# iMacsimus/Triangles-SDF-CPU-RayTracing

Measured on AMD Instinct MI355X. Metric: Mrays/sec + ms/frame at 1920x1080, bunny tris & SDF grid, 1/2/4/8 MI355X, higher is better.
Workload: dtype f32; 1 GPU; bunny: shipped stanford-bunny.obj (69,451 triangles), 1920x1080, primary rays (Normal shading, no plane) (BASELINE configs[1]); camera=orbit r=2.5 h=0.5 fovy 45, parallelism=1 GPU, 1 thread per pixel, frames_per_launch=16, streams=2

## Files before the change

### triangles-sdf-cpu-raytracing_amd/csrc/rt_device.hip

```cpp
#include <hip/hip_runtime.h>

#include <algorithm>
#include <atomic>
#include <cmath>
#include <cstdio>
#include <limits>
#include <map>
#include <mutex>
#include <string>
#include <type_traits>
#include <utility>

#include "../../include/rtamd.h"
#include "rt_dispatch.h"
#include "rt_error.h"
#include "rt_host.h"
#include "rt_queue.h"
#include "rt_ray_io.h"
#include "rt_scene.h"
#include "rt_shade.h"

using namespace rtd;
using namespace rti;

namespace {

#ifndef RT_PERSIST_BLOCK
#define RT_PERSIST_BLOCK 64
#endif
constexpr int kPBlock = RT_PERSIST_BLOCK;
static_assert(kPBlock % 64 == 0 && kPBlock >= 64 && kPBlock <= 1024, "persistent block: whole waves");
constexpr int kTile = 16;

template <class T>
__device__ __forceinline__ void fb_store(T *p, T v, bool peer) {
  if (peer) {
    __hip_atomic_store(p, v, __ATOMIC_RELAXED, __HIP_MEMORY_SCOPE_SYSTEM);
    return;
  }
  __hip_atomic_store(p, v, __ATOMIC_RELAXED, __HIP_MEMORY_SCOPE_AGENT);
}

#ifndef RT_PEER_RELEASE
#define RT_PEER_RELEASE 1
#endif
constexpr uint32_t kSysStoreFlags = RT_FLAG_TILE_NATURAL;
__device__ __forceinline__ void peer_release(uint32_t flags) {
#if RT_PEER_RELEASE
  if (flags & kSysStoreFlags) __builtin_amdgcn_fence(__ATOMIC_RELEASE, "");
#endif
}

__device__ __forceinline__ int image_row(int yl, const FrameArgs &fa) {
  if (fa.nranks <= 1) return yl;
  const uint32_t br = (uint32_t)fa.band_rows, k = (uint32_t)yl / br, r = (uint32_t)yl - k * br;
  return (int)((k * (uint32_t)fa.nranks + (uint32_t)fa.rank) * br + r);
}

template <int DIAG>
struct CntSel { using T = NoCnt; };
template <>
struct CntSel<1> { using T = LaneCnt; };
template <>
struct CntSel<2> { using T = LaneCnt; };

__device__ __forceinline__ void flush_counts(NoCnt &, unsigned long long *) {}
__device__ __forceinline__ void flush_counts(LaneCnt &c, unsigned long long *out) {
#pragma unroll
  for (int i = 0; i < C_ALL; ++i) {
    unsigned long long v = c.v[i];
#pragma unroll
    for (int off = 32; off > 0; off >>= 1) v += __shfl_xor(v, off, 64);
    if ((threadIdx.x & 63) == 0 && v) atomicAdd(out + i, v);
  }
}


#ifndef RT_DIAG_HOST_NOSTORE
#define RT_DIAG_HOST_NOSTORE 0
#endif

#ifndef RT_PAIR_FLUSH
#define RT_PAIR_FLUSH 1
#endif
constexpr int kPairWords = 2 * 8 * 16;

template <class S, int SLOTS, bool GENERAL, int DIAG, int B = kBlock, class CT>
__device__ __forceinline__ bool render_pixels(const S &sc, const PlaneDev &pl, const FrameArgs &fa,
                                              CT &cnt, uint32_t *stk, int xo, int yl,
                                              uint32_t *defer = nullptr) {
  const bool active = xo < fa.W && yl < fa.rows_local;
  constexpr bool kWaveCoop = DIAG == 0 && !GENERAL && S::kCoop;
  constexpr bool kWaveCount = DIAG == 1 && !GENERAL && S::kCoop;
  if (DIAG == 0 && !kWaveCoop && !active) return false;
  if (active || kWaveCoop || kWaveCount) {
    StackOf<S, B> st{stk + threadIdx.x};
    if constexpr (kWaveCoop) {
      const int yo = image_row(active ? yl : 0, fa);
      const uint32_t cx = fa.cull_x, cy = (uint32_t)fa.P.reserved;
      const uint32_t px = (uint32_t)xo >> 3, py = (uint32_t)yo >> 3;
      const bool inside = active && px >= (cx & 0xFFFFu) && px < (cx >> 16) && py >= (cy & 0xFFFFu) && py < (cy >> 16);
      if (__ballot(inside) == 0) {
        const bool natural = (fa.flags & (kSysStoreFlags | kFlagNatural)) != 0;
        const uint32_t idx = (uint32_t)(natural ? yo : yl) * (uint32_t)fa.W + (uint32_t)xo;
        if (defer) {
          defer[0] = 0u;
          defer[kPairWords] = __float_as_uint(kInf);
        } else if (RT_DIAG_HOST_NOSTORE != 0 && (fa.flags & kFlagHostFrame)) {
        } else if (active && (fa.flags & RT_FLAG_CLEAR) && !(fa.flags & RT_FLAG_HITS_ONLY)) {
          const bool sys = (fa.flags & (kSysStoreFlags | kFlagHostFrame)) != 0;
          fb_store(fa.color + idx, 0u, sys);
          fb_store(fa.t + idx, kInf, sys);
        }
        return false;
      }
      asm volatile("" : "+v"(xo), "+v"(yl));
    }
    const int yo = image_row(active ? yl : 0, fa);
    const int y = fa.H - yo - 1;
    const f3 o{fa.P.camera_pos[0], fa.P.camera_pos[1], fa.P.camera_pos[2]};
    f3 d;
    if (fa.flags & kFlagFastEye)
      d = eye_ray_fast(active ? xo : 0, y, fa.W, fa.H, fa.P.proj_inv, fa.P.view_inv);
    else
      d = eye_ray(active ? xo : 0, y, fa.W, fa.H, fa.P.proj_inv, fa.P.view_inv);
    const bool natural = (fa.flags & (kSysStoreFlags | kFlagNatural)) != 0;
    const bool sys = (fa.flags & (kSysStoreFlags | kFlagHostFrame)) != 0;
    const int yb = natural ? yo : yl;
    const uint32_t idx = active ? (uint32_t)yb * (uint32_t)fa.W + (uint32_t)xo : 0u;
    const bool clear = (fa.flags & RT_FLAG_CLEAR) != 0;
    const bool hits_only = (fa.flags & RT_FLAG_HITS_ONLY) != 0;
    const float tPrev = (clear || !active) ? kInf : fa.t[idx];
    const float tFarEff = std_min(100.0f, tPrev);
    bool hit;
    float t;
    f4 c;
    if (!GENERAL) {
      if (active) cnt.add(C_RAYS, 1);
      Hit h;
      if constexpr (kWaveCoop)
        h = sc.template primary<B>(o, d, 0.01f, tFarEff, active, stk);
      else if constexpr (kWaveCount)
        h = sc.template primary_counted<B>(o, d, 0.01f, tFarEff, active, stk, cnt);
      else
        h = sc.template intersect<B>(o, d, 0.01f, tFarEff, st, cnt);
      hit = h.hit;
      t = h.t;
      f3 n = h.n;
      if (dot(n, d) > 0) n = n * -1.0f;
      c = f4{(n.x + 1.0f) / 2.0f, (n.y + 1.0f) / 2.0f, (n.z + 1.0f) / 2.0f, (1.0f + 1.0f) / 2.0f};
    } else {
      c = shade_one<S, B>(sc, pl, fa.P, o, d, tFarEff, true, hit, t, st, nullptr, cnt);
    }
    const bool store = hit && !__builtin_isinf(t);
    if (defer) {
      defer[0] = store ? pack_rgba(c) : 0u;
      defer[kPairWords] = __float_as_uint(store ? t : kInf);
    } else if (RT_DIAG_HOST_NOSTORE == 1 && (fa.flags & kFlagHostFrame)) {
    } else if (RT_DIAG_HOST_NOSTORE == 2 && (fa.flags & kFlagHostFrame)) {
      if (active && store) fb_store(fa.color + idx, pack_rgba(c), sys);
    } else if (!active) {
    } else if (clear && !hits_only) {
      fb_store(fa.color + idx, store ? pack_rgba(c) : 0u, sys);
      fb_store(fa.t + idx, store ? t : kInf, sys);
    } else if (store) {
      fb_store(fa.color + idx, pack_rgba(c), sys);
      fb_store(fa.t + idx, t, sys);
    }
    return active && store;
  }
  return false;
}

typedef unsigned int u32x4 __attribute__((ext_vector_type(4)));
__device__ __forceinline__ void host_store16(uint32_t *p, u32x4 v) {
  asm volatile("global_store_dwordx4 %0, %1, off sc0 sc1" : : "v"(p), "v"(v) : "memory");
}

template <class S, int SLOTS, bool GENERAL, int DIAG, int BT = kBlock>
__device__ __forceinline__ void render_body(const S &sc, const PlaneDev &pl, const FrameArgs &fa,
                                            unsigned long long *counters, uint32_t *stk,
                                            uint32_t *hf = nullptr) {
  typename CntSel<DIAG>::T cnt{};
  unsigned long long t_start = 0;
  if (DIAG == 2) t_start = __builtin_amdgcn_s_memrealtime();
  const int lane = threadIdx.x & 63, wave = threadIdx.x >> 6;
  uint32_t bx = blockIdx.x, by = blockIdx.y;
  if (DIAG == 0 && fa.order) {
    const uint32_t tl = fa.order[blockIdx.y * gridDim.x + blockIdx.x];
    bx = tl % gridDim.x;
    by = tl / gridDim.x;
  }
  const uint64_t c0 = (DIAG == 0 && fa.cost) ? __builtin_amdgcn_s_memtime() : 0;
  const int xo = BT == 64 ? (int)bx * 8 + (lane & 7) : (int)bx * kTile + (wave & 1) * 8 + (lane & 7);
  const int yl = BT == 64 ? (int)by * 8 + (lane >> 3) : (int)by * kTile + (wave >> 1) * 8 + (lane >> 3);
  const int band = wave >> 1;
  const bool flush = RT_PAIR_FLUSH && DIAG == 0 && BT == kBlock && hf != nullptr &&
                     (fa.flags & kFlagHostFrame) && (fa.flags & RT_FLAG_CLEAR) && (fa.flags & RT_FLAG_HITS_ONLY) &&
                     (fa.W & 3) == 0 && (((uintptr_t)fa.color | (uintptr_t)fa.t) & 15u) == 0 &&
                     (int)bx * kTile + kTile <= fa.W && (int)by * kTile + band * 8 + 8 <= fa.rows_local;
  uint32_t *slot = flush ? hf + band * 128 + (lane >> 3) * 16 + (wave & 1) * 8 + (lane & 7) : nullptr;
  const bool stored = render_pixels<S, SLOTS, GENERAL, DIAG, BT>(sc, pl, fa, cnt, stk, xo, yl, slot);
  if (flush) {
    const uint32_t any = __ballot(stored) != 0 ? 1u : 0u;
    __builtin_amdgcn_fence(__ATOMIC_RELEASE, "workgroup");
    uint32_t old = 0;
    if (lane == 0) old = atomicAdd(hf + 2 * kPairWords + band, 1u | (any << 16));
    old = __builtin_amdgcn_readfirstlane(old);
    if ((old & 0xFFFFu) == 1u && (any | (old >> 16)) != 0u) {
      __builtin_amdgcn_fence(__ATOMIC_ACQUIRE, "workgroup");
      const int b = lane >> 5, r = (lane & 31) >> 2, ch = lane & 3;
      const u32x4 v = *reinterpret_cast<const u32x4 *>(hf + b * kPairWords + band * 128 + r * 16 + ch * 4);
      const int ylr = (int)by * kTile + band * 8 + r;
      const bool natural = (fa.flags & (kSysStoreFlags | kFlagNatural)) != 0;
      const uint32_t row = (uint32_t)(natural ? image_row(ylr, fa) : ylr);
      uint32_t *base = b ? reinterpret_cast<uint32_t *>(fa.t) : fa.color;
      host_store16(base + row * (uint32_t)fa.W + (uint32_t)bx * kTile + (uint32_t)ch * 4u, v);
    }
  }
  if constexpr (DIAG == 0) {
    if (fa.hit_box && !(fa.flags & kFlagRowSpan) && __ballot(stored)) {
      int32_t v[4] = {stored ? xo : INT32_MAX, stored ? -xo : INT32_MAX, stored ? yl : INT32_MAX,
                      stored ? -yl : INT32_MAX};
#pragma unroll
      for (int i = 0; i < 4; ++i)
#pragma unroll
        for (int off = 32; off > 0; off >>= 1) {
          const int32_t o = __shfl_xor(v[i], off, 64);
          v[i] = o < v[i] ? o : v[i];
        }
      if (lane == __ffsll((unsigned long long)__ballot(1)) - 1)
#pragma unroll
        for (int i = 0; i < 4; ++i)
          if (v[i] < __hip_atomic_load(fa.hit_box + i, __ATOMIC_RELAXED, __HIP_MEMORY_SCOPE_AGENT))
            atomicMin(fa.hit_box + i, v[i]);
    }
    if (fa.hit_box && (fa.flags & kFlagRowSpan) && __ballot(stored)) {
      int32_t lo = stored ? xo : INT32_MAX, nhi = stored ? -xo : INT32_MAX;
#pragma unroll
      for (int off = 1; off < 8; off <<= 1) {
        const int32_t a = __shfl_xor(lo, off, 64), b = __shfl_xor(nhi, off, 64);
        lo = a < lo ? a : lo;
        nhi = b < nhi ? b : nhi;
      }
      if ((lane & 7) == 0 && lo != INT32_MAX) {
        int32_t *sp = fa.hit_box + 2 * yl;
        if (lo < __hip_atomic_load(sp, __ATOMIC_RELAXED, __HIP_MEMORY_SCOPE_AGENT)) atomicMin(sp, lo);
        if (nhi < __hip_atomic_load(sp + 1, __ATOMIC_RELAXED, __HIP_MEMORY_SCOPE_AGENT)) atomicMin(sp + 1, nhi);
      }
    }
  }
  if constexpr (DIAG == 0) {
    if (fa.cost) {
      const uint64_t dt = __builtin_amdgcn_s_memtime() - c0;
      if (lane == __ffsll((unsigned long long)__ballot(1)) - 1)
        atomicMax(fa.cost + by * gridDim.x + bx, dt > 0xFFFFFFFFull ? 0xFFFFFFFFu : (uint32_t)dt);
    }
  }
  if constexpr (DIAG == 1) flush_counts(cnt, counters);
  if constexpr (DIAG == 2) {
    const unsigned long long t_end = __builtin_amdgcn_s_memrealtime();
    uint32_t units = 0;
#pragma unroll
    for (int i = 0; i < C_RAYS; ++i) units += cnt.v[i];
    uint32_t mx = units, sm = units;
#pragma unroll
    for (int off = 32; off > 0; off >>= 1) {
      const uint32_t om = __shfl_xor(mx, off, 64), os = __shfl_xor(sm, off, 64);
      mx = mx > om ? mx : om;
      sm += os;
    }
    uint32_t rest = units, u9 = 0;
    for (int r = 0; r < 9; ++r) {
      uint32_t m = rest;
#pragma unroll
      for (int off = 32; off > 0; off >>= 1) {
        const uint32_t om = __shfl_xor(m, off, 64);
        m = m > om ? m : om;
      }
      u9 = m;
      const uint64_t who = __ballot(rest == m);
      if ((threadIdx.x & 63) == (int)__builtin_ctzll(who)) rest = 0;
    }
    if ((threadIdx.x & 63) == 0) {
      const size_t w = ((size_t)blockIdx.y * gridDim.x + blockIdx.x) * (kBlock / 64) + (threadIdx.x >> 6);
      counters[4 * w] = t_start;
      counters[4 * w + 1] = t_end;
      counters[4 * w + 2] = ((unsigned long long)sm << 32) | mx;
      counters[4 * w + 3] = __builtin_amdgcn_s_getreg(0x1814) | ((unsigned long long)u9 << 8);
    }
  }
}

template <class S, int SLOTS, bool GENERAL, int DIAG>
constexpr int min_waves() {
  return (DIAG != 0 || SLOTS > 7) ? 1 : GENERAL ? RT_GENERAL_WAVES : S::kMinWaves;
}

#ifndef RT_FRAME_BLOCK
#define RT_FRAME_BLOCK 256
#endif
constexpr int kFBlock = RT_FRAME_BLOCK;
constexpr int kFTile = kFBlock == 64 ? 8 : kTile;
static_assert(kFBlock == 64 || kFBlock == kBlock, "one-frame workgroup: one wave or the 16x16 tile");
template <int DIAG>
constexpr int frame_block() { return DIAG == 0 ? kFBlock : kBlock; }
template <int DIAG>
constexpr int frame_tile() { return DIAG == 0 ? kFTile : kTile; }

#ifndef RT_FRAME_PRIO
#define RT_FRAME_PRIO 0
#endif
#ifndef RT_FRAME_COOP
#define RT_FRAME_COOP RT_COOP_RAYS
#endif
template <class S, int SLOTS, bool GENERAL, int DIAG>
__global__ __launch_bounds__(frame_block<DIAG>()) __attribute__((amdgpu_waves_per_eu(min_waves<S, SLOTS, GENERAL, DIAG>())))
void render_kernel(S sc_arg, PlaneDev pl, FrameArgs fa,
                                                        unsigned long long *counters) {
  __shared__ uint32_t stk[stack_words<S, SLOTS>() * frame_block<DIAG>()];
  constexpr bool kPair = RT_PAIR_FLUSH && DIAG == 0 && frame_block<DIAG>() == kBlock;
  __shared__ __attribute__((aligned(16))) uint32_t hf[kPair ? 2 * kPairWords + 4 : 4];
  S sc = sc_arg;
  if constexpr (S::kCoop && !GENERAL && DIAG == 0) {
    sc.prio_iters = RT_FRAME_PRIO;
    sc.coop_rays = RT_FRAME_COOP;
  }
  if (kPair && (fa.flags & kFlagHostFrame) && (fa.flags & RT_FLAG_CLEAR) && (fa.flags & RT_FLAG_HITS_ONLY)) {
    if (threadIdx.x < 2) hf[2 * kPairWords + threadIdx.x] = 0u;
    __syncthreads();
  }
  render_body<S, SLOTS, GENERAL, DIAG, frame_block<DIAG>()>(sc, pl, fa, counters, stk, kPair ? hf : nullptr);
  peer_release(fa.flags);
}

#ifndef RT_BATCH_BLOCK
#define RT_BATCH_BLOCK 64
#endif
constexpr int kBBlock = RT_BATCH_BLOCK;
#ifndef RT_BATCH_INTERLEAVE
#define RT_BATCH_INTERLEAVE 1
#endif
constexpr int kBTile = kBBlock == 64 ? 8 : kTile;
static_assert(kBBlock == 64 || kBBlock == kBlock, "batch workgroup: one wave or the 16x16 tile");

template <class S, int SLOTS, bool GENERAL>
__global__ __launch_bounds__(kBBlock) __attribute__((amdgpu_waves_per_eu(min_waves<S, SLOTS, GENERAL, 0>())))
void render_batch_kernel(S sc, PlaneDev pl, FrameBatch fb) {
  __shared__ uint32_t stk[stack_words<S, SLOTS>() * kBBlock];
  if constexpr (kBBlock == kBlock) {
    render_body<S, SLOTS, GENERAL, 0>(sc, pl, fb.f[blockIdx.z], nullptr, stk);
  } else {
    NoCnt cnt{};
    const int lane = threadIdx.x & 63;
#if RT_BATCH_INTERLEAVE
    const uint32_t n = gridDim.z, b = (blockIdx.z * gridDim.y + blockIdx.y) * gridDim.x + blockIdx.x;
    const uint32_t f = b % n, tl = fb.f[0].order ? fb.f[0].order[b / n] : b / n;
    const uint32_t tx = tl % gridDim.x, ty = tl / gridDim.x;
#else
    const uint32_t f = blockIdx.z, tl = blockIdx.y * gridDim.x + blockIdx.x, tx = blockIdx.x, ty = blockIdx.y;
#endif
    const uint64_t c0 = fb.f[0].cost ? __builtin_amdgcn_s_memtime() : 0;
    render_pixels<S, SLOTS, GENERAL, 0, kBBlock>(sc, pl, fb.f[f], cnt, stk, (int)tx * 8 + (lane & 7),
                                                 (int)ty * 8 + (lane >> 3));
    if (fb.f[0].cost && lane == 0) {
      const uint64_t dc = __builtin_amdgcn_s_memtime() - c0;
      atomicMax(fb.f[0].cost + tl, (uint32_t)(dc < 0xFFFFFFFFull ? dc : 0xFFFFFFFFull));
    }
  }
  peer_release(fb.f[0].flags);
}

struct PersistQ {
  uint32_t *heads;
  uint32_t items;
  uint32_t tiles_x, per_frame;
  uint32_t waves;
  uint32_t gx, gy;
  uint32_t stride;
  uint32_t nheads;
  uint32_t cpf, nper;
  unsigned long long *stamps;
  uint32_t ox, oy;
};
template <class S, bool GENERAL>
constexpr bool kQueueOrigin = S::kCoop && !GENERAL;
constexpr int kHeadStride = 1088;
constexpr int kHeadStrideMax = 4096;

__device__ __forceinline__ uint32_t q_claim(uint32_t *head) {
  uint32_t k = 0;
  if ((threadIdx.x & 63) == 0) k = __hip_atomic_fetch_add(head, 1u, __ATOMIC_RELAXED, __HIP_MEMORY_SCOPE_AGENT);
  return __builtin_amdgcn_readfirstlane(k);
}
#ifndef RT_QUEUE_HEADS
#define RT_QUEUE_HEADS 0
#endif
__device__ __forceinline__ uint32_t q_nheads(const PersistQ &q) { return RT_QUEUE_HEADS ? (uint32_t)RT_QUEUE_HEADS : q.nheads; }
__device__ __forceinline__ uint32_t q_home(uint32_t xcc, uint32_t nheads) {
  const uint32_t wave = __builtin_amdgcn_readfirstlane(threadIdx.x >> 6);
  return rtq::home(xcc, (blockIdx.x >> 3) + wave, nheads);
}
__device__ __forceinline__ uint32_t q_scan(const PersistQ &q, uint32_t nh, uint32_t own, int lane) {
  uint32_t v = 0xFFFFFFFFu;
  const bool mine = (uint32_t)lane < nh;
  if (mine) v = __hip_atomic_load(q.heads + (uint32_t)lane * q.stride, __ATOMIC_RELAXED, __HIP_MEMORY_SCOPE_AGENT);
  const uint32_t cap = q.cpf ? q.nper : rtq::cap(q.items, nh, (uint32_t)lane);
  const uint64_t left = __ballot(mine && v < cap);
  return left ? rtq::next(left, own, nh) : rtq::kNone;
}
__device__ __forceinline__ void q_leave(const PersistQ &q, uint32_t nh, int lane) {
  uint32_t *done = q.heads + nh * q.stride;
  uint32_t last = 0;
  if (lane == 0) last = __hip_atomic_fetch_add(done, 1u, __ATOMIC_RELAXED, __HIP_MEMORY_SCOPE_AGENT) == q.waves - 1;
  if (__builtin_amdgcn_readfirstlane(last)) {
    if ((uint32_t)lane < nh)
      __hip_atomic_store(q.heads + (uint32_t)lane * q.stride, 0u, __ATOMIC_RELAXED, __HIP_MEMORY_SCOPE_AGENT);
    if (lane == 0) __hip_atomic_store(done, 0u, __ATOMIC_RELAXED, __HIP_MEMORY_SCOPE_AGENT);
  }
}

template <class S, int SLOTS, bool GENERAL>
__global__ __launch_bounds__(kPBlock) __attribute__((amdgpu_waves_per_eu(min_waves<S, SLOTS, GENERAL, 0>())))
void render_persist_kernel(S sc_arg, PlaneDev pl, FrameBatch fb, PersistQ q) {
  __shared__ uint32_t stk[stack_words<S, SLOTS>() * kPBlock];
  S sc = sc_arg;
  if constexpr (S::kCoop && !GENERAL) sc.prio_iters = RT_HEAVY_PRIO;
  const int lane = threadIdx.x & 63;
  const uint32_t xcc = __builtin_amdgcn_s_getreg(0x1814) & 7;
#ifdef RT_PERSIST_STAMPS
  const unsigned long long t_start = __builtin_amdgcn_s_memrealtime();
  unsigned long long t_item = t_start, t_last = t_start, d_max = 0;
  uint32_t n_items = 0, last_item = 0, max_item = 0;
#endif
  uint32_t h = q_home(xcc, q_nheads(q));
  uint32_t k = q_claim(q.heads + h * q.stride);
  NoCnt cnt{};
  for (;;) {
    uint32_t item, f, r;
    bool drained, empty = false;
    if (q.cpf == 0) {
      item = k * q_nheads(q) + h;
      drained = item >= q.items;
      f = item / q.per_frame;
      r = item - f * q.per_frame;
    } else {
      drained = k >= q.nper;
      f = k / q.cpf;
      r = h * q.cpf + (k - f * q.cpf);
      empty = r >= q.per_frame;
      item = f * q.per_frame + r;
    }
    if (drained) {
      h = q_scan(q, q_nheads(q), h, lane);
      if (h == rtq::kNone) break;
      k = q_claim(q.heads + h * q.stride);
      continue;
    }
    const uint32_t knext = q_claim(q.heads + h * q.stride);
    if (empty) {
      k = knext;
      continue;
    }
    uint32_t ty = r / q.tiles_x, tx = r - ty * q.tiles_x;
    if constexpr (kQueueOrigin<S, GENERAL>) {
      tx += q.ox;
      ty += q.oy;
    }
#ifdef RT_PERSIST_STAMPS
    const unsigned long long t_begin = __builtin_amdgcn_s_memrealtime();
#endif
    for (uint32_t j = 0; j < q.gy; ++j)
      for (uint32_t i = 0; i < q.gx; ++i) {
        uint32_t fo = f;
        asm volatile("" : "+s"(fo));
        render_pixels<S, SLOTS, GENERAL, 0, kPBlock>(sc, pl, fb.f[fo], cnt, stk, (int)((tx * q.gx + i) * 8) + (lane & 7),
                                            (int)((ty * q.gy + j) * 8) + (lane >> 3));
      }
#ifdef RT_PERSIST_STAMPS
    ++n_items;
    t_item = __builtin_amdgcn_s_memrealtime();
    t_last = t_begin;
    last_item = item;
    if (t_item - t_begin > d_max) {
      d_max = t_item - t_begin;
      max_item = item;
    }
#endif
    k = knext;
  }
#ifdef RT_PERSIST_STAMPS
  if (q.stamps && lane == 0) {
    const size_t w = (size_t)blockIdx.x * (kPBlock / 64) + (threadIdx.x >> 6);
    unsigned long long *o = q.stamps + 8 * w;
    o[0] = t_start;
    o[1] = __builtin_amdgcn_s_memrealtime();
    o[2] = n_items | ((unsigned long long)xcc << 32);
    o[3] = t_item;
    o[4] = t_last;
    o[5] = last_item;
    o[6] = d_max;
    o[7] = max_item;
  }
#endif
  peer_release(fb.f[0].flags);
  q_leave(q, q_nheads(q), lane);
}

struct PumpFrame {
  float o[3];
  float proj_inv[16];
  float view_inv[16];
  uint32_t *color;
  float *t;
};

constexpr uint32_t kPumpHeads = rtq::kXcds;
struct ItemStream {
  uint32_t h, k;
};
__device__ __forceinline__ uint32_t take_item(const PersistQ &q, ItemStream &s, uint32_t xcc, int lane) {
  for (;;) {
    const uint32_t item = rtq::item(q.items, kPumpHeads, s.h, s.k);
    if (item != rtq::kNone) {
      s.k = q_claim(q.heads + s.h * q.stride);
      return item;
    }
    static_assert(kPumpHeads == 8 && rtq::cap(45, 8, 3) == (45 + 7 - 3) / 8 && rtq::next(0x21, 5, 8) == 0, "take_item's scan");
    uint32_t v = 0xFFFFFFFFu;
    if (lane < 8) v = __hip_atomic_load(q.heads + lane * q.stride, __ATOMIC_RELAXED, __HIP_MEMORY_SCOPE_AGENT);
    const uint64_t m = __ballot(lane < 8 && v < (q.items + 7u - (uint32_t)lane) / 8u) & 0xFFull;
    if (m == 0) return 0xFFFFFFFFu;
    const uint32_t rot = (uint32_t)(((m >> (xcc + 1)) | (m << (7 - xcc))) & 0xFFull);
    s.h = (xcc + 1 + (uint32_t)__builtin_ctz(rot)) & 7u;
    s.k = q_claim(q.heads + s.h * q.stride);
  }
}

struct OctP {
  using Ray = OctRay;
  static constexpr int kFields = kOctFields;
  static constexpr int kMinWaves = RT_OCT_WAVES;
  OctDev d;
  template <bool FAST>
  __device__ __forceinline__ int start(f3 o, f3 dir, f3 inv, float tf, Ray &R, float &t, f3 &n) const {
    NoCnt c;
    OctHitPt hp;
    const int s = oct_start<FAST>(d, o, dir, inv, 0.01f, tf, R, t, hp, c);
    if (s == RAY_HIT) n = oct_normal_at(d, hp, c);
    return s;
  }
  template <bool FAST>
  __device__ __forceinline__ int run(f3 o, f3 dir, f3 inv, float tf, LdsStack<kBlock, kOctFields> st, Ray &R, int limit,
                                     float &t, f3 &n) const {
    NoCnt c;
    OctHitPt hp;
    const int s = oct_run<kBlock, FAST, true, false>(d, o, dir, inv, 0.01f, tf, st, R, limit, t, hp, c);
    if (s == RAY_HIT) n = oct_normal_at(d, hp, c);
    return s;
  }
};

template <int kMode>
struct GridP {
  using Ray = GridRay;
  static constexpr int kFields = 1;
  static constexpr int kMinWaves = RT_GRID_WAVES;
  GridDev d;
  template <bool FAST>
  __device__ __forceinline__ int start(f3 o, f3 dir, f3 inv, float tf, Ray &R, float &, f3 &) const {
    return grid_start(o, dir, inv, 0.01f, tf, R);
  }
  template <bool FAST>
  __device__ __forceinline__ int run(f3 o, f3 dir, f3, float, LdsStack<kBlock, kFields>, Ray &R, int limit,
                                     float &t, f3 &n) const {
    NoCnt c;
    f3 hp;
    const int s = grid_run<kMode, true>(d, o, dir, R, limit, t, hp, c);
    if (s == RAY_HIT) n = grid_normal<kMode>(d, hp, c);
    return s;
  }
};

#ifndef RT_REFILL_MIN
#define RT_REFILL_MIN 16
#endif

#ifndef RT_PUMP_WAVES
#define RT_PUMP_WAVES 0
#endif
template <class P, int SLOTS>
__global__ __launch_bounds__(kBlock)
__attribute__((amdgpu_waves_per_eu(SLOTS > 7 ? 1 : (RT_PUMP_WAVES ? RT_PUMP_WAVES : P::kMinWaves))))
void render_pump_kernel(P sc, FrameBatch fb, PersistQ q, int32_t nframes, int32_t refill_min) {
  __shared__ uint32_t stk[SLOTS * P::kFields * kBlock];
  __shared__ PumpFrame frames[kMaxBatch];
  if ((int)threadIdx.x < nframes) {
    const FrameArgs &fa = fb.f[threadIdx.x];
    PumpFrame &pf = frames[threadIdx.x];
    for (int i = 0; i < 3; ++i) pf.o[i] = fa.P.camera_pos[i];
    for (int i = 0; i < 16; ++i) {
      pf.proj_inv[i] = fa.P.proj_inv[i];
      pf.view_inv[i] = fa.P.view_inv[i];
    }
    pf.color = fa.color;
    pf.t = fa.t;
  }
  __syncthreads();
  const FrameArgs &F = fb.f[0];
  const int lane = threadIdx.x & 63;
  const uint32_t xcc = __builtin_amdgcn_s_getreg(0x1814) & 7;
  const bool clear = (F.flags & RT_FLAG_CLEAR) != 0, hits_only = (F.flags & RT_FLAG_HITS_ONLY) != 0;
  const bool peer = (F.flags & kSysStoreFlags) != 0;
  const uint32_t isz = 64u * q.gx * q.gy;
  ItemStream is{xcc, 0u};
  is.k = q_claim(q.heads + is.h * q.stride);
  uint32_t cur = take_item(q, is, xcc, lane), off = 0;
  LdsStack<kBlock, P::kFields> st{stk + threadIdx.x};
  typename P::Ray R;
  bool live = false, fast = true;
  uint32_t f = 0;
  uint32_t idx = 0;
  f3 o{0.0f, 0.0f, 0.0f}, d{0.0f, 0.0f, 1.0f}, inv{kInf, kInf, 1.0f};
  float tfar = 100.0f;
  auto finish = [&](int status, float t, f3 n) {
    const bool hit = status == RAY_HIT;
    const bool store = hit && !__builtin_isinf(t);
    if (dot(n, d) > 0) n = n * -1.0f;
    const f4 c{(n.x + 1.0f) / 2.0f, (n.y + 1.0f) / 2.0f, (n.z + 1.0f) / 2.0f, (1.0f + 1.0f) / 2.0f};
    uint32_t *cp = frames[f].color + idx;
    float *tp = frames[f].t + idx;
    if (clear && !hits_only) {
      fb_store(cp, store ? pack_rgba(c) : 0u, peer);
      fb_store(tp, store ? t : kInf, peer);
    } else if (store) {
      fb_store(cp, pack_rgba(c), peer);
      fb_store(tp, t, peer);
    }
  };
  for (;;) {
    while (cur != 0xFFFFFFFFu) {
      const uint64_t dead = __ballot(!live);
      const uint32_t ndead = (uint32_t)__popcll(dead);
      if ((int)ndead < refill_min) break;
      const uint32_t rank = __builtin_amdgcn_mbcnt_hi((uint32_t)(dead >> 32),
                                                      __builtin_amdgcn_mbcnt_lo((uint32_t)dead, 0u));
      const uint32_t nxt = (off + ndead >= isz) ? take_item(q, is, xcc, lane) : 0xFFFFFFFFu;
      const uint32_t fc = cur / q.per_frame, rc = cur - fc * q.per_frame;
      const uint32_t tyc = rc / q.tiles_x, txc = rc - tyc * q.tiles_x;
      uint32_t fn = 0, txn = 0, tyn = 0;
      if (nxt != 0xFFFFFFFFu) {
        fn = nxt / q.per_frame;
        const uint32_t rn = nxt - fn * q.per_frame;
        tyn = rn / q.tiles_x;
        txn = rn - tyn * q.tiles_x;
      }
      bool got = false;
      uint32_t p = 0, tx = 0, ty = 0;
      if (!live) {
        if (off + rank < isz) { got = true; p = off + rank; f = fc; tx = txc; ty = tyc; }
        else if (nxt != 0xFFFFFFFFu) { got = true; p = off + rank - isz; f = fn; tx = txn; ty = tyn; }
      }
      off += ndead;
      if (off >= isz) { cur = nxt; off -= isz; }
      if (got) {
        const uint32_t tile = p >> 6;
        const uint32_t ti = q.gx == 1 ? 0u : (tile & 1u), tj = q.gx == 1 ? tile : (tile >> 1);
        const int x = (int)((tx * q.gx + ti) * 8 + (p & 7u));
        const int yl = (int)((ty * q.gy + tj) * 8 + ((p >> 3) & 7u));
        if (x < F.W && yl < F.rows_local) {
          const int yo = image_row(yl, F);
          const PumpFrame &pf = frames[f];
          idx = (uint32_t)(peer ? yo : yl) * (uint32_t)F.W + (uint32_t)x;
          o = f3{pf.o[0], pf.o[1], pf.o[2]};
          d = eye_ray(x, F.H - yo - 1, F.W, F.H, pf.proj_inv, pf.view_inv);
          inv = f3{1.0f / d.x, 1.0f / d.y, 1.0f / d.z};
          fast = __builtin_isfinite(inv.x) && __builtin_isfinite(inv.y) && __builtin_isfinite(inv.z);
          tfar = clear ? 100.0f : std_min(100.0f, pf.t[idx]);
          float t = kInf;
          f3 n{0.0f, 1.0f, 0.0f};
          const int s = fast ? sc.template start<true>(o, d, inv, tfar, R, t, n)
                             : sc.template start<false>(o, d, inv, tfar, R, t, n);
          if (s == RAY_PENDING) live = true;
          else finish(s, t, n);
        }
      }
    }
    if (__ballot(live) == 0) {
      if (cur == 0xFFFFFFFFu) break;
      continue;
    }
    const int limit = cur == 0xFFFFFFFFu ? 0 : 64 - refill_min;
    float t = kInf;
    f3 n{0.0f, 1.0f, 0.0f};
    int s = RAY_PENDING;
    if (__ballot(live && !fast) == 0) {
      if (live) s = sc.template run<true>(o, d, inv, tfar, st, R, limit, t, n);
    } else {
      if (live) s = sc.template run<false>(o, d, inv, tfar, st, R, limit, t, n);
    }
    if (live && s != RAY_PENDING) {
      finish(s, t, n);
      live = false;
    }
  }
  peer_release(F.flags);
  q_leave(q, kPumpHeads, lane);
}

__global__ void clear_kernel(uint32_t *c, float *t, int64_t n) {
  const int64_t i = ((int64_t)blockIdx.x * blockDim.x + threadIdx.x) * 4;
  if (i + 4 <= n) {
    *reinterpret_cast<uint4 *>(c + i) = make_uint4(0u, 0u, 0u, 0u);
    *reinterpret_cast<float4 *>(t + i) = make_float4(kInf, kInf, kInf, kInf);
  } else {
    for (int64_t j = i; j < n; ++j) {
      c[j] = 0u;
      t[j] = kInf;
    }
  }
}

struct ClearOutside {
  uint32_t *color[kMaxBatch];
  float *t[kMaxBatch];
  uint32_t W, H;
  uint32_t x0, x1, y0, y1;
};
__global__ __launch_bounds__(64) void clear_outside_kernel(ClearOutside a) {
  const uint32_t x = blockIdx.x * 64u + threadIdx.x, yb = blockIdx.y * 8u;
  if (x >= a.W) return;
  const bool in_x = x >= a.x0 && x < a.x1;
  if (in_x && yb >= a.y0 && yb + 8u <= a.y1) return;
  uint32_t *c = a.color[blockIdx.z];
  float *t = a.t[blockIdx.z];
#pragma unroll
  for (uint32_t j = 0; j < 8u; ++j) {
    const uint32_t y = yb + j;
    if (y >= a.H || (in_x && y >= a.y0 && y < a.y1)) continue;
    const uint32_t idx = y * a.W + x;
    fb_store(c + idx, 0u, false);
    fb_store(t + idx, kInf, false);
  }
}

constexpr int kCostClasses = 66;
__device__ __forceinline__ uint32_t cost_class(uint32_t c) {
  if (c == 0) return 0;
  const uint32_t e = 32u - (uint32_t)__clz(c);
  return 2 * e + (e >= 2 ? (c >> (e - 2)) & 1u : 0u);
}
__global__ __launch_bounds__(1024) void order_kernel(uint32_t *cost, uint32_t *order, uint32_t n) {
  __shared__ uint32_t hist[kCostClasses];
  for (uint32_t i = threadIdx.x; i < kCostClasses; i += blockDim.x) hist[i] = 0;
  __syncthreads();
  for (uint32_t i = threadIdx.x; i < n; i += blockDim.x) atomicAdd(&hist[cost_class(cost[i])], 1u);
  __syncthreads();
  if (threadIdx.x == 0) {
    uint32_t run = 0;
    for (int b = kCostClasses - 1; b >= 0; --b) {
      const uint32_t h = hist[b];
      hist[b] = run;
      run += h;
    }
  }
  __syncthreads();
  for (uint32_t i = threadIdx.x; i < n; i += blockDim.x) {
    order[atomicAdd(&hist[cost_class(cost[i])], 1u)] = i;
    cost[i] = 0;
  }
}

}

namespace rti {

int ensure_events(rt_scene *s) {
  if (int rc = s->fb.ev0.create_timing()) return rc;
  if (int rc = s->fb.ev1.create_timing()) return rc;
  return s->drop.ev_host.create(hipEventDisableTiming);
}

int ensure_fb(rt_scene *s, size_t px) {
  if (px <= s->fb.cap) return RT_OK;
  s->fb.cap = 0;
  if (int rc = s->fb.color.alloc(px)) return rc;
  if (int rc = s->fb.t.alloc(px)) return rc;
  s->fb.cap = px;
  return RT_OK;
}

}

namespace {

template <class S, int MAXD>
void launch_render_t(const S &sc, const PlaneDev &pl, const FrameArgs &fa, bool general,
                     hipStream_t stream, unsigned long long *counters, int diag) {
  const dim3 grid((fa.W + kTile - 1) / kTile, (fa.rows_local + kTile - 1) / kTile);
  const dim3 fgrid((fa.W + kFTile - 1) / kFTile, (fa.rows_local + kFTile - 1) / kFTile);
  if (diag == 1) {
    if (general)
      render_kernel<S, MAXD, true, 1><<<grid, kBlock, 0, stream>>>(sc, pl, fa, counters);
    else
      render_kernel<S, MAXD, false, 1><<<grid, kBlock, 0, stream>>>(sc, pl, fa, counters);
  } else if (diag == 2) {
    if (general)
      render_kernel<S, MAXD, true, 2><<<grid, kBlock, 0, stream>>>(sc, pl, fa, counters);
    else
      render_kernel<S, MAXD, false, 2><<<grid, kBlock, 0, stream>>>(sc, pl, fa, counters);
  } else {
    if (general)
      render_kernel<S, MAXD, true, 0><<<fgrid, kFBlock, 0, stream>>>(sc, pl, fa, nullptr);
    else
      render_kernel<S, MAXD, false, 0><<<fgrid, kFBlock, 0, stream>>>(sc, pl, fa, nullptr);
  }
}

#ifndef RT_SCHED_FRESH
#define RT_SCHED_FRESH 1
#endif
int schedule_begin(rt_scene *s, FrameArgs &fa, uint32_t gx, uint32_t gy, hipStream_t stream) {
  fa.order = nullptr;
  fa.cost = nullptr;
  const bool same_stream = stream == s->sched.last_stream;
  s->sched.last_stream = stream;
  if (!s->info.sched_on || !same_stream) return RT_OK;
  const uint32_t nb = gx * gy;
  if (!s->sched.os.s) {
    char label[64];
    std::snprintf(label, sizeof label, "scene %p schedule stream", (void *)s);
    if (int rc = s->sched.os.create(s->device, label)) return rc;
    for (rtmem::Event &e : s->sched.ord_ev)
      if (int rc = e.create(hipEventDisableTiming)) return rc;
    if (int rc = s->sched.frame_ev.create(hipEventDisableTiming)) return rc;
  }
  if (nb > s->sched.cap) {
    HIP_TRY(hipStreamSynchronize(s->sched.os.s));
    s->sched.cap = 0;
    s->sched.key[0] = s->sched.key[1] = 0;
    for (int b = 0; b < 2; ++b) {
      if (int rc = s->sched.cost[b].alloc(nb)) return rc;
      if (int rc = s->sched.order[b].alloc(nb)) return rc;
      HIP_TRY(hipMemsetAsync(s->sched.cost[b].p, 0, (size_t)nb * 4, stream));
    }
    s->sched.cap = nb;
  }
  const int p = s->sched.par;
  if (s->sched.rec[p]) {
    const hipError_t q = hipEventQuery(s->sched.ord_ev[p].e);
    if (q == hipErrorNotReady) {
      HIP_TRY(hipStreamWaitEvent(stream, s->sched.ord_ev[p].e, 0));
    } else if (q != hipSuccess) {
      HIP_TRY(q);
    }
  }
  const uint32_t key = (gx << 16) | gy;
  if (RT_SCHED_FRESH && s->sched.rec[p ^ 1] && s->sched.key[p ^ 1] == key &&
      hipEventQuery(s->sched.ord_ev[p ^ 1].e) == hipSuccess) {
    fa.order = s->sched.order[p ^ 1].p;
  } else if (s->sched.key[p] == key) {
    fa.order = s->sched.order[p].p;
  }
  fa.cost = s->sched.cost[p].p;
  return RT_OK;
}

int schedule_end(rt_scene *s, const FrameArgs &fa, uint32_t gx, uint32_t gy, hipStream_t stream) {
  if (!fa.cost) return RT_OK;
  const int p = s->sched.par;
  HIP_TRY(hipEventRecord(s->sched.frame_ev.e, stream));
  HIP_TRY(hipStreamWaitEvent(s->sched.os.s, s->sched.frame_ev.e, 0));
  order_kernel<<<1, 1024, 0, s->sched.os.s>>>(s->sched.cost[p].p, s->sched.order[p].p, gx * gy);
  HIP_TRY(hipGetLastError());
  HIP_TRY(hipEventRecord(s->sched.ord_ev[p].e, s->sched.os.s));
  s->sched.rec[p] = true;
  s->sched.key[p] = (gx << 16) | gy;
  s->sched.par = p ^ 1;
  return RT_OK;
}

}

namespace rti {

int launch_render(rt_scene *s, const FrameArgs &fa_in, hipStream_t stream, unsigned long long *counters, int diag,
                  bool sched) {
  FrameArgs fa = fa_in;
  const bool general = s->info.plane.on || fa.P.shading_mode != RT_SHADING_NORMAL;
  const uint32_t gx = (fa.W + kFTile - 1) / kFTile, gy = (fa.rows_local + kFTile - 1) / kFTile;
  fa.order = nullptr;
  fa.cost = nullptr;
  if (diag == 0 && sched) {
    const int rc = schedule_begin(s, fa, gx, gy, stream);
    if (rc) return rc;
  }
  if (!dispatch_scene(s, [&](const auto &sc, auto slots) {
        launch_render_t<std::decay_t<decltype(sc)>, decltype(slots)::value>(sc, s->info.plane, fa, general, stream,
                                                                            counters, diag);
      }))
    return set_err(RT_E_STATE, "scene has no geometry");
  HIP_TRY(hipGetLastError());
  if (diag == 0 && sched) return schedule_end(s, fa, gx, gy, stream);
  return RT_OK;
}

}

namespace {

constexpr size_t kQueueWords = (size_t)rtq::kMaxHeads * kHeadStride + 16;
constexpr size_t kQueueBytes = kQueueWords * sizeof(uint32_t);
static_assert((size_t)rtq::kXcds * kHeadStrideMax + 1 <= kQueueWords, "8 heads at the widest stride must fit");
std::mutex g_queue_mu;
std::map<std::pair<int, hipStream_t>, uint32_t *> g_queues;

int stream_queue(hipStream_t stream, uint32_t **out) {
  *out = nullptr;
  int dev = 0;
  HIP_TRY(hipGetDevice(&dev));
  std::lock_guard<std::mutex> lk(g_queue_mu);
  auto it = g_queues.find({dev, stream});
  if (it != g_queues.end()) {
    *out = it->second;
    return RT_OK;
  }
  void *p = nullptr;
  HIP_TRY(hipMallocAsync(&p, kQueueBytes, stream));
  const hipError_t e = hipMemsetAsync(p, 0, kQueueBytes, stream);
  if (e != hipSuccess) {
    HIP_NOTE(hipFreeAsync(p, stream));
    return set_err(RT_E_DEVICE, std::string("work-queue init: ") + hipGetErrorString(e));
  }
  g_queues[{dev, stream}] = (uint32_t *)p;
  *out = (uint32_t *)p;
  return RT_OK;
}

struct BandSched {
  uint32_t *cost = nullptr, *order = nullptr;
  uint32_t ntiles = 0;
  bool valid = false;
};
std::map<std::pair<int, hipStream_t>, BandSched> g_band_sched;

bool band_order_env() { return ab_on("RTAMD_BAND_ORDER"); }
std::atomic<bool> g_band_order{band_order_env()};
bool band_order_enabled() { return g_band_order.load(std::memory_order_relaxed); }

int band_sched(hipStream_t stream, uint32_t ntiles, BandSched **out) {
  *out = nullptr;
  int dev = 0;
  HIP_TRY(hipGetDevice(&dev));
  std::lock_guard<std::mutex> lk(g_queue_mu);
  BandSched &b = g_band_sched[{dev, stream}];
  if (b.ntiles != ntiles) {
    if (b.cost) HIP_NOTE(hipFreeAsync(b.cost, stream));
    if (b.order) HIP_NOTE(hipFreeAsync(b.order, stream));
    b = BandSched{};
    void *c = nullptr, *o = nullptr;
    HIP_TRY(hipMallocAsync(&c, (size_t)ntiles * 4, stream));
    HIP_TRY(hipMallocAsync(&o, (size_t)ntiles * 4, stream));
    HIP_TRY(hipMemsetAsync(c, 0, (size_t)ntiles * 4, stream));
    b.cost = (uint32_t *)c;
    b.order = (uint32_t *)o;
    b.ntiles = ntiles;
  }
  *out = &b;
  return RT_OK;
}

unsigned long long *g_persist_stamps = nullptr;
int64_t g_persist_stamps_cap = 0;

bool persist_enabled() {
  static const bool on = !ab_off("RTAMD_PERSIST");
  return on;
}

std::atomic<int64_t> g_band_queue_px{ab_int("RTAMD_BAND_PERSIST_PX", 1000000, INT64_MIN, INT64_MAX)};
bool band_takes_queue(const FrameArgs &f) {
  if (f.nranks <= 1) return true;
  static const int max_ranks = (int)ab_int("RTAMD_BAND_PERSIST", -1, 0, INT32_MAX);
  if (max_ranks >= 0) return f.nranks <= max_ranks;
  return (int64_t)f.rows_local * f.W >= g_band_queue_px.load(std::memory_order_relaxed);
}

int persist_group(int dflt) {
  static const int g = (int)ab_int("RTAMD_PERSIST_G", 0, 1, 4);
  return (g == 1 || g == 2 || g == 4) ? g : dflt;
}

template <class K>
int resident_blocks(K kernel, int &blocks, int &dev_cached, int block = kBlock) {
  int dev = 0;
  HIP_TRY(hipGetDevice(&dev));
  if (blocks == 0 || dev != dev_cached) {
    int per_cu = 0, cus = 0;
    HIP_TRY(hipOccupancyMaxActiveBlocksPerMultiprocessor(&per_cu, kernel, block, 0));
    HIP_TRY(hipDeviceGetAttribute(&cus, hipDeviceAttributeMultiprocessorCount, dev));
    static const int oversub = (int)ab_int("RTAMD_PERSIST_OVERSUB", 1, 1, 8);
    blocks = std::max(1, per_cu) * std::max(1, cus) * oversub;
    dev_cached = dev;
  }
  return RT_OK;
}

#ifndef RT_QUEUE_SUBHEADS
#define RT_QUEUE_SUBHEADS 2
#endif
static_assert(rtq::heads_ok(rtq::kXcds * RT_QUEUE_SUBHEADS), "RT_QUEUE_SUBHEADS: 1, 2, 4 or 8");
int queue_heads_env() {
  static const int h = [] {
    const long long v = ab_int("RTAMD_QHEADS", rtq::kXcds * RT_QUEUE_SUBHEADS, rtq::kXcds, rtq::kMaxHeads);
    return rtq::heads_ok((uint32_t)v) ? (int)v : (int)(rtq::kXcds * RT_QUEUE_SUBHEADS);
  }();
  return h;
}
std::atomic<int> g_queue_heads{queue_heads_env()};

bool queue_grid_env() {
  static const bool on = !ab_off("RTAMD_QGRID");
  return on;
}
std::atomic<bool> g_queue_grid{queue_grid_env()};
static_assert(rtq::kWhole == kCullWhole, "rtq::grid's whole-frame word is FrameArgs'");
namespace grid_check {
constexpr uint32_t cx[2] = {3u | (7u << 16), 0u}, cy[2] = {1u | (2u << 16), 0u};
constexpr rtq::Grid g = rtq::grid(cx, cy, 2, 250, 131, 2, 1);
static_assert(g.ox == 1 && g.oy == 1 && g.tiles_x == 3 && g.tiles_y == 1, "rtq::grid");
}

bool takes_queue_grid(const FrameBatch &fb, int n) {
  if (!g_queue_grid.load(std::memory_order_relaxed)) return false;
  for (int i = 0; i < n; ++i)
    if (fb.f[i].nranks != 1 || (fb.f[i].flags & (kSysStoreFlags | kFlagNatural | kFlagHostFrame)) != 0 ||
        fb.f[i].W != fb.f[0].W || fb.f[i].rows_local != fb.f[0].rows_local || fb.f[i].flags != fb.f[0].flags)
      return false;
  return true;
}

int make_queue(const FrameBatch &fb, int n, int group, int blocks, hipStream_t stream, PersistQ &q,
               uint32_t &grid, int block = kBlock, bool shrink = false) {
  uint32_t *heads = nullptr;
  if (const int rc = stream_queue(stream, &heads)) return rc;
  q.heads = heads;
  static const uint32_t stride = (uint32_t)ab_int("RTAMD_QSTRIDE", kHeadStride, 1, kHeadStrideMax);
  q.stride = stride;
  q.nheads = (uint32_t)g_queue_heads.load(std::memory_order_relaxed);
  if ((size_t)q.stride * q.nheads + 1 > kQueueWords)
    return set_err(RT_E_INVALID, "work queue: RTAMD_QSTRIDE x the head count does not fit the stream's head set");
  q.gx = group >= 2 ? 2 : 1;
  q.gy = group >= 4 ? 2 : 1;
  uint32_t cx[kMaxBatch], cy[kMaxBatch];
  for (int i = 0; i < n; ++i) {
    cx[i] = shrink ? fb.f[i].cull_x : rtq::kWhole;
    cy[i] = shrink ? (uint32_t)fb.f[i].P.reserved : rtq::kWhole;
  }
  const rtq::Grid g = rtq::grid(cx, cy, (uint32_t)n, (uint32_t)fb.f[0].W, (uint32_t)fb.f[0].rows_local, q.gx, q.gy);
  q.ox = g.ox;
  q.oy = g.oy;
  q.tiles_x = g.tiles_x;
  q.per_frame = g.tiles_x * g.tiles_y;
  q.items = q.per_frame * (uint32_t)n;
  q.cpf = q.nper = 0;
  const uint32_t wpb = (uint32_t)block / 64;
  grid = std::min<uint32_t>((uint32_t)blocks, (q.items + wpb - 1) / wpb);
  q.waves = grid * wpb;
  q.stamps = (g_persist_stamps && (int64_t)q.waves <= g_persist_stamps_cap) ? g_persist_stamps : nullptr;
  return RT_OK;
}

template <class S, int MAXD, bool GENERAL>
int launch_persist_t(rt_scene *s, const S &sc, const PlaneDev &pl, const FrameBatch &fb, int n, int group,
                     hipStream_t stream) {
  static int blocks = 0, dev_cached = -1;
  if (const int rc = resident_blocks(render_persist_kernel<S, MAXD, GENERAL>, blocks, dev_cached, kPBlock)) return rc;
  PersistQ q;
  uint32_t grid = 0;
  const bool shrink = kQueueOrigin<S, GENERAL> && takes_queue_grid(fb, n);
  if (const int rc = make_queue(fb, n, group, blocks, stream, q, grid, kPBlock, shrink)) return rc;
  const uint32_t W = (uint32_t)fb.f[0].W, H = (uint32_t)fb.f[0].rows_local;
  ClearOutside co;
  co.W = W;
  co.H = H;
  co.x0 = std::min(W, q.ox * q.gx * 8u);
  co.x1 = std::min(W, (q.ox + q.tiles_x) * q.gx * 8u);
  co.y0 = std::min(H, q.oy * q.gy * 8u);
  co.y1 = q.tiles_x ? std::min(H, (q.oy + q.per_frame / q.tiles_x) * q.gy * 8u) : co.y0;
  const bool whole = co.x0 == 0 && co.y0 == 0 && co.x1 == W && co.y1 == H;
  if (!whole && (fb.f[0].flags & RT_FLAG_CLEAR) && !(fb.f[0].flags & RT_FLAG_HITS_ONLY)) {
    for (int i = 0; i < kMaxBatch; ++i) {
      co.color[i] = i < n ? fb.f[i].color : nullptr;
      co.t[i] = i < n ? fb.f[i].t : nullptr;
    }
    clear_outside_kernel<<<dim3((W + 63u) / 64u, (H + 7u) / 8u, (uint32_t)n), 64, 0, stream>>>(co);
  }
  if (grid == 0) return RT_OK;
  render_persist_kernel<S, MAXD, GENERAL><<<grid, kPBlock, 0, stream>>>(sc, pl, fb, q);
  return RT_OK;
}

bool pump_env() {
  static const bool on = ab_on("RTAMD_PUMP");
  return on;
}
std::atomic<int> g_refill{(int)ab_int("RTAMD_REFILL", RT_REFILL_MIN, 1, 64)};
int refill_min() { return g_refill.load(std::memory_order_relaxed); }

template <class S>
struct PumpOf {
  static constexpr bool kHas = false;
};
template <bool PK>
struct PumpOf<OctS<PK>> {
  static constexpr bool kHas = true;
  using P = OctP;
  static P make(const OctS<PK> &s) { return P{s.d}; }
};
template <int kMode>
struct PumpOf<GridS<kMode>> {
  static constexpr bool kHas = true;
  using P = GridP<kMode>;
  static P make(const GridS<kMode> &s) { return P{s.d}; }
};
constexpr int kPumpGroup = 4;

template <class P, int MAXD>
int launch_pump_t(const P &sc, const FrameBatch &fb, int n, int group, hipStream_t stream) {
  static int blocks = 0, dev_cached = -1;
  if (const int rc = resident_blocks(render_pump_kernel<P, MAXD>, blocks, dev_cached)) return rc;
  PersistQ q;
  uint32_t grid = 0;
  if (const int rc = make_queue(fb, n, group, blocks, stream, q, grid)) return rc;
  render_pump_kernel<P, MAXD><<<grid, kBlock, 0, stream>>>(sc, fb, q, n, refill_min());
  return RT_OK;
}

template <class S, int MAXD>
int launch_batch_t(rt_scene *s, const S &sc, const PlaneDev &pl, const FrameBatch &fb, int n, bool general,
                   hipStream_t stream) {
  const int group = persist_group(S::kQueueGroup);
  if constexpr (PumpOf<S>::kHas) {
    if (!general && (pump_env() || (s && s->info.pump_on)) && persist_enabled() && band_takes_queue(fb.f[0]))
      return launch_pump_t<typename PumpOf<S>::P, MAXD>(PumpOf<S>::make(sc), fb, n,
                                                        persist_group(S::kQueueGroup ? S::kQueueGroup : kPumpGroup),
                                                        stream);
  }
  if (persist_enabled() && group > 0 && band_takes_queue(fb.f[0])) {
    return general ? launch_persist_t<S, MAXD, true>(s, sc, pl, fb, n, group, stream)
                   : launch_persist_t<S, MAXD, false>(s, sc, pl, fb, n, group, stream);
  }
  const dim3 grid((fb.f[0].W + kBTile - 1) / kBTile, (fb.f[0].rows_local + kBTile - 1) / kBTile, n);
  BandSched *bs = nullptr;
  if (kBBlock == 64 && RT_BATCH_INTERLEAVE && fb.f[0].nranks > 1 && band_order_enabled()) {
    if (const int rc = band_sched(stream, grid.x * grid.y, &bs)) return rc;
  }
  const FrameBatch *fbp = &fb;
  FrameBatch fbo;
  if (bs) {
    fbo = fb;
    fbo.f[0].order = bs->valid ? bs->order : nullptr;
    fbo.f[0].cost = bs->cost;
    fbp = &fbo;
  }
  if (general)
    render_batch_kernel<S, MAXD, true><<<grid, kBBlock, 0, stream>>>(sc, pl, *fbp);
  else
    render_batch_kernel<S, MAXD, false><<<grid, kBBlock, 0, stream>>>(sc, pl, *fbp);
  if (bs) {
    order_kernel<<<1, 64, 0, stream>>>(bs->cost, bs->order, bs->ntiles);
    HIP_TRY(hipGetLastError());
    bs->valid = true;
  }
  return RT_OK;
}

}

namespace rti {

int launch_batch(rt_scene *s, FrameBatch &fb, int n, hipStream_t stream) {
  const bool general = s->info.plane.on || fb.f[0].P.shading_mode != RT_SHADING_NORMAL;
  for (int i = 0; i < n; ++i) {
    if (general != (s->info.plane.on || fb.f[i].P.shading_mode != RT_SHADING_NORMAL))
      return set_err(RT_E_INVALID, "frames of one batch must share the shading path");
    fb.f[i].order = nullptr;
    fb.f[i].cost = nullptr;
  }
  int rc = RT_OK;
  if (!dispatch_scene(s, [&](const auto &sc, auto slots) {
        rc = launch_batch_t<std::decay_t<decltype(sc)>, decltype(slots)::value>(s, sc, s->info.plane, fb, n, general,
                                                                                stream);
      }))
    return set_err(RT_E_STATE, "scene has no geometry");
  if (rc) return rc;
  HIP_TRY(hipGetLastError());
  return RT_OK;
}

}

namespace {

bool fast_eye_enabled() {
  static const bool on = !ab_off("RTAMD_FAST_EYE");
  return on;
}

bool fast_eye_ok(const float *m, int32_t W, int32_t H) {
  if (W > 32768 || H > 32768) return false;
  for (int i = 0; i < 16; ++i) {
    const float a = std::fabs(m[i]);
    if (i >= 8 && i < 12) {
      if (!std::isfinite(m[i])) return false;
    } else if (!(m[i] == 0.0f || (a >= 0x1p-10f && a <= 0x1p10f))) {
      return false;
    }
  }
  const double wc = std::fabs((double)m[15]), wr = std::fabs((double)m[3]) + std::fabs((double)m[7]);
  if (!(wc - wr >= 0x1p-10)) return false;
  const double wmax = wc + wr;
  double lmin = 0.0;
  for (int i = 0; i < 3; ++i)
    lmin = std::max(lmin, (std::fabs((double)m[12 + i]) - std::fabs((double)m[i]) - std::fabs((double)m[4 + i])) / wmax);
  return lmin >= 0x1p-20;
}

bool tile_cull_env() {
  static const bool on = !ab_off("RTAMD_TILE_CULL");
  return on;
}
std::atomic<bool> g_tile_cull{tile_cull_env()};

bool cull_rect(const rt_render_params *p, int32_t W, int32_t H, const float box[6], const float *guard,
               int n_guard, int32_t out[4]) {
  if (W <= 0 || H <= 0 || W > 32768 || H > 32768) return false;
  const float *pi = p->proj_inv, *vi = p->view_inv;
  double o[3], M[3][3];
  for (int k = 0; k < 3; ++k) {
    o[k] = (double)p->camera_pos[k];
    if (!std::isfinite(o[k]) || !std::isfinite((double)box[k]) || !std::isfinite((double)box[3 + k])) return false;
    if (!(box[k] <= box[3 + k])) return false;
  }
  bool outside = false;
  for (int k = 0; k < 3; ++k) {
    if (o[k] < (double)box[k] || o[k] > (double)box[3 + k]) outside = true;
    if (o[k] == (double)box[k] || o[k] == (double)box[3 + k]) return false;
    for (int g = 0; g < n_guard; ++g)
      if (o[k] == (double)guard[6 * g + 2 * k] || o[k] == (double)guard[6 * g + 2 * k + 1]) return false;
  }
  if (!outside) return false;
  const double wc = (double)pi[15], wr = std::fabs((double)pi[3]) + std::fabs((double)pi[7]);
  if (!std::isfinite(wc) || !std::isfinite(wr) || !(std::fabs(wc) > wr * (1.0 + 0x1p-20))) return false;
  const double sgn = wc > 0 ? 1.0 : -1.0;
  const int cols[3] = {0, 1, 3};
  double scale = 0.0;
  for (int r = 0; r < 3; ++r)
    for (int c = 0; c < 3; ++c) {
      double a = 0.0;
      for (int j = 0; j < 3; ++j) a += (double)vi[j * 4 + r] * (double)pi[cols[c] * 4 + j];
      if (!std::isfinite(a)) return false;
      M[r][c] = a;
      scale = std::max(scale, std::fabs(a));
    }
  double C[3][3];
  for (int r = 0; r < 3; ++r)
    for (int c = 0; c < 3; ++c) {
      const int r1 = (r + 1) % 3, r2 = (r + 2) % 3, c1 = (c + 1) % 3, c2 = (c + 2) % 3;
      C[r][c] = M[r1][c1] * M[r2][c2] - M[r1][c2] * M[r2][c1];
    }
  const double det = M[0][0] * C[0][0] + M[0][1] * C[0][1] + M[0][2] * C[0][2];
  if (!std::isfinite(det) || !(std::fabs(det) > 1e-9 * scale * scale * scale)) return false;
  const double l0 = std::sqrt(M[0][0] * M[0][0] + M[1][0] * M[1][0] + M[2][0] * M[2][0]) * 2.0 / W;
  const double l1 = std::sqrt(M[0][1] * M[0][1] + M[1][1] * M[1][1] + M[2][1] * M[2][1]) * 2.0 / H;
  const double l2 = std::sqrt(M[0][2] * M[0][2] + M[1][2] * M[1][2] + M[2][2] * M[2][2]) +
                    std::sqrt(M[0][0] * M[0][0] + M[1][0] * M[1][0] + M[2][0] * M[2][0]) +
                    std::sqrt(M[0][1] * M[0][1] + M[1][1] * M[1][1] + M[2][1] * M[2][1]);
  if (!(l0 >= 0x1p-17 * l2) || !(l1 >= 0x1p-17 * l2)) return false;
  double lo[2] = {std::numeric_limits<double>::infinity(), std::numeric_limits<double>::infinity()};
  double hi[2] = {-lo[0], -lo[1]};
  int behind = 0;
  for (int i = 0; i < 8; ++i) {
    double v[3], c[3];
    for (int k = 0; k < 3; ++k) v[k] = (double)box[((i >> k) & 1) ? 3 + k : k] - o[k];
    for (int r = 0; r < 3; ++r) c[r] = (C[0][r] * v[0] + C[1][r] * v[1] + C[2][r] * v[2]) / det;
    const double z = sgn * c[2], zb = 1e-9 * (std::fabs(c[0]) + std::fabs(c[1]));
    if (!std::isfinite(z) || !std::isfinite(zb)) return false;
    if (z < -zb && z < 0.0) {
      ++behind;
      continue;
    }
    if (behind != 0 || !(z > zb) || !(z > 0.0)) return false;
    for (int a = 0; a < 2; ++a) {
      const double n = c[a] / c[2];
      if (!std::isfinite(n)) return false;
      lo[a] = std::min(lo[a], n);
      hi[a] = std::max(hi[a], n);
    }
  }
  if (behind == 8) {
    out[0] = out[1] = out[2] = out[3] = 0;
    return true;
  }
  if (behind != 0) return false;
  const double dim[2] = {(double)W, (double)H};
  int64_t p0[2], p1[2];
  for (int a = 0; a < 2; ++a) {
    const double f0 = std::floor((lo[a] + 1.0) * dim[a] * 0.5 - 0.5) - 2.0;
    const double f1 = std::ceil((hi[a] + 1.0) * dim[a] * 0.5 - 0.5) + 2.0;
    p0[a] = (int64_t)std::min(std::max(f0, 0.0), dim[a]);
    p1[a] = (int64_t)std::min(std::max(f1, -1.0), dim[a] - 1.0);
  }
  const int64_t r0 = (int64_t)H - 1 - p1[1], r1 = (int64_t)H - 1 - p0[1];
  if (p0[0] > p1[0] || r0 > r1) {
    out[0] = out[1] = out[2] = out[3] = 0;
    return true;
  }
  out[0] = (int32_t)(p0[0] >> 3);
  out[1] = (int32_t)(p1[0] >> 3) + 1;
  out[2] = (int32_t)(r0 >> 3);
  out[3] = (int32_t)(r1 >> 3) + 1;
  return true;
}

}

namespace rti {

int fill_frame(FrameArgs &fa, const rt_scene *s, const rt_render_params *p, uint32_t *c, float *t, int32_t W,
               int32_t H, uint32_t flags, const rt_tile *tile) {
  fa.P = *p;
  fa.cull_x = kCullWhole;
  fa.P.reserved = (int32_t)kCullWhole;
  if (g_tile_cull.load(std::memory_order_relaxed) && s && s->info.kind == RT_SCENE_MESH && !s->info.plane.on &&
      p->shading_mode == RT_SHADING_NORMAL && s->mesh.root != rtl::kInvalidChild && !(s->mesh.root & rtl::kLeafBit)) {
    int32_t r[4];
    if (cull_rect(p, W, H, s->mesh.root_box, s->mesh.root_child, 8, r)) {
      fa.cull_x = (uint32_t)r[0] | ((uint32_t)r[1] << 16);
      fa.P.reserved = (int32_t)((uint32_t)r[2] | ((uint32_t)r[3] << 16));
    }
  }
  fa.color = c;
  fa.t = t;
  fa.W = W;
  fa.H = H;
  fa.flags = flags;
  fa.band_rows = H;
  fa.rank = 0;
  fa.nranks = 1;
  fa.rows_local = H;
  fa.order = nullptr;
  fa.cost = nullptr;
  fa.hit_box = nullptr;
  if ((flags & RT_FLAG_HITS_ONLY) && !(flags & RT_FLAG_CLEAR))
    return set_err(RT_E_INVALID, "RT_FLAG_HITS_ONLY needs RT_FLAG_CLEAR (a cleared frame)");
  if (flags & ~(RT_FLAG_CLEAR | RT_FLAG_TILE_NATURAL | RT_FLAG_HITS_ONLY))
    return set_err(RT_E_INVALID, "unknown render flag");
  if (tile && tile->num_ranks > 1) {
    if (tile->band_rows <= 0 || tile->rank < 0 || tile->rank >= tile->num_ranks)
      return set_err(RT_E_INVALID, "bad tile");
    fa.band_rows = tile->band_rows;
    fa.rank = tile->rank;
    fa.nranks = tile->num_ranks;
    fa.rows_local = (int32_t)(rt_tile_pixels(W, H, tile) / W);
  }
  if (fast_eye_enabled() && fast_eye_ok(p->proj_inv, W, H)) fa.flags |= kFlagFastEye;
  return RT_OK;
}

}

extern "C" {

int rt_render_device(rt_scene *s, const rt_render_params *p, uint32_t *d_color, float *d_t, int32_t W,
                     int32_t H, uint32_t flags, const rt_tile *tile, void *stream) {
  if (!s) return set_err(RT_E_INVALID, "scene is NULL");
  int rc = no_instanced(s, "rt_render_device");
  if (rc) return rc;
  if ((rc = check_params(p, W, H))) return rc;
  if (!d_color || !d_t) return set_err(RT_E_INVALID, "NULL framebuffer");
  FrameArgs fa;
  if ((rc = fill_frame(fa, s, p, d_color, d_t, W, H, flags, tile))) return rc;
  if (fa.rows_local <= 0) return RT_OK;
  return launch_render(s, fa, (hipStream_t)stream);
}

int rt_render_device_frames(rt_scene *s, const rt_render_params *params, int32_t frames,
                            uint32_t *const *d_color, float *const *d_t, int32_t W, int32_t H,
                            uint32_t flags, const rt_tile *tile, void *stream) {
  if (!s || !params || !d_color || !d_t || frames < 0) return set_err(RT_E_INVALID, "bad arguments");
  if (int rc = no_instanced(s, "rt_render_device_frames")) return rc;
  if (frames == 1) return rt_render_device(s, params, d_color[0], d_t[0], W, H, flags, tile, stream);
  FrameBatch fb;
  for (int32_t f0 = 0; f0 < frames; f0 += kMaxBatch) {
    const int n = std::min<int32_t>(kMaxBatch, frames - f0);
    for (int i = 0; i < n; ++i) {
      int rc = check_params(params + f0 + i, W, H);
      if (rc) return rc;
      if (!d_color[f0 + i] || !d_t[f0 + i]) return set_err(RT_E_INVALID, "NULL framebuffer");
      if ((rc = fill_frame(fb.f[i], s, params + f0 + i, d_color[f0 + i], d_t[f0 + i], W, H, flags, tile)))
        return rc;
    }
    if (fb.f[0].rows_local <= 0) return RT_OK;
    const int rc = launch_batch(s, fb, n, (hipStream_t)stream);
    if (rc) return rc;
  }
  return RT_OK;
}

int rt_clear_device(uint32_t *d_color, float *d_t, int64_t n, void *stream) {
  if (!d_color || !d_t || n < 0) return set_err(RT_E_INVALID, "bad arguments");
  if (((uintptr_t)d_color | (uintptr_t)d_t) & 15) return set_err(RT_E_INVALID, "buffers must be 16-byte aligned");
  if (n == 0) return RT_OK;
  const int64_t lanes = (n + 3) / 4;
  clear_kernel<<<(unsigned)((lanes + 255) / 256), 256, 0, (hipStream_t)stream>>>(d_color, d_t, n);
  HIP_TRY(hipGetLastError());
  return RT_OK;
}

int rt_stream_prepare(void *stream) {
  uint32_t *heads = nullptr;
  return stream_queue((hipStream_t)stream, &heads);
}

int rt_stream_release(void *stream) {
  int dev = 0;
  HIP_TRY(hipGetDevice(&dev));
  uint32_t *p = nullptr;
  {
    std::lock_guard<std::mutex> lk(g_queue_mu);
    auto b = g_band_sched.find({dev, (hipStream_t)stream});
    if (b != g_band_sched.end()) {
      if (b->second.cost) HIP_NOTE(hipFreeAsync(b->second.cost, (hipStream_t)stream));
      if (b->second.order) HIP_NOTE(hipFreeAsync(b->second.order, (hipStream_t)stream));
      g_band_sched.erase(b);
    }
    auto it = g_queues.find({dev, (hipStream_t)stream});
    if (it == g_queues.end()) return RT_OK;
    p = it->second;
    g_queues.erase(it);
  }
  HIP_TRY(hipFreeAsync(p, (hipStream_t)stream));
  return RT_OK;
}

static int count_frames(rt_scene *s, const rt_render_params *params, int32_t frames, int32_t W, int32_t H,
                        uint32_t flags, const rt_tile *tile, unsigned long long (&h)[C_ALL]) {
  if (!s || !params || frames <= 0) return set_err(RT_E_INVALID, "bad arguments");
  int rc = no_instanced(s, "rt_count_work");
  if (rc) return rc;
  if ((rc = check_params(params, W, H))) return rc;
  const size_t px = (size_t)W * H;
  if ((rc = ensure_fb(s, px))) return rc;
  rtmem::DevArray<unsigned long long> d;
  if ((rc = d.alloc(C_ALL))) return rc;
  hipError_t e = hipMemset(d.p, 0, d.bytes());
  if (e == hipSuccess) HIP_NOTE(hipMemset(s->fb.t.p, 0x7f, px * 4));
  for (int32_t f = 0; f < frames && e == hipSuccess && rc == RT_OK; ++f) {
    FrameArgs fa;
    if (!(rc = check_params(params + f, W, H)) &&
        !(rc = fill_frame(fa, s, params + f, s->fb.color.p, s->fb.t.p, W, H, flags, tile)))
      rc = launch_render(s, fa, 0, d.p, 1);
  }
  if (e == hipSuccess && rc == RT_OK) e = hipMemcpy(h, d.p, sizeof(h), hipMemcpyDeviceToHost);
  if (rc) return rc;
  if (e != hipSuccess) return set_err(RT_E_DEVICE, std::string("rt_count_work: ") + hipGetErrorString(e));
  return RT_OK;
}

int rt_count_work(rt_scene *s, const rt_render_params *params, int32_t frames, int32_t W, int32_t H,
                  uint32_t flags, const rt_tile *tile, int64_t counters[9]) {
  if (!counters) return set_err(RT_E_INVALID, "bad arguments");
  unsigned long long h[C_ALL] = {};
  const int rc = count_frames(s, params, frames, W, H, flags, tile, h);
  if (rc) return rc;
  for (int i = 0; i < C_NUM; ++i) counters[i] = (int64_t)h[i];
  return RT_OK;
}

int rtx_count_share(rt_scene *s, const rt_render_params *params, int32_t frames, int32_t W, int32_t H,
                    uint32_t flags, int64_t out[2]) {
  if (!out) return set_err(RT_E_INVALID, "bad arguments");
  unsigned long long h[C_ALL] = {};
  const int rc = count_frames(s, params, frames, W, H, flags, nullptr, h);
  if (rc) return rc;
  out[0] = (int64_t)h[C_BVH_SHARED];
  out[1] = (int64_t)h[C_BVH_WAVE_EXP];
  return RT_OK;
}

int rtx_wave_stamps(rt_scene *s, const rt_render_params *params, int32_t W, int32_t H, uint32_t flags,
                    uint64_t *out, int64_t *nwaves) {
  if (!s || !params || !out || !nwaves) return set_err(RT_E_INVALID, "bad arguments");
  int rc = check_params(params, W, H);
  if (rc) return rc;
  const int64_t nb = (int64_t)((W + kTile - 1) / kTile) * ((H + kTile - 1) / kTile);
  const int64_t nw = nb * (kBlock / 64);
  if (*nwaves < nw) { *nwaves = nw; return set_err(RT_E_INVALID, "buffer too small"); }
  const size_t px = (size_t)W * H;
  if ((rc = ensure_fb(s, px))) return rc;
  rtmem::DevArray<unsigned long long> d;
  if ((rc = d.alloc((size_t)nw * 4))) return rc;
  FrameArgs fa;
  if (!(rc = fill_frame(fa, s, params, s->fb.color.p, s->fb.t.p, W, H, flags, nullptr)))
    rc = launch_render(s, fa, 0, d.p, 2);
  hipError_t e = rc ? hipSuccess : hipMemcpy(out, d.p, d.bytes(), hipMemcpyDeviceToHost);
  if (rc) return rc;
  if (e != hipSuccess) return set_err(RT_E_DEVICE, hipGetErrorString(e));
  *nwaves = nw;
  return RT_OK;
}

int rtx_set_band_queue_px(int64_t px) {
  g_band_queue_px.store(px < 0 ? (int64_t)1000000 : px);
  return RT_OK;
}

int rtx_fast_eye_ok(const float *proj_inv, int32_t W, int32_t H) {
  return proj_inv && fast_eye_ok(proj_inv, W, H) ? 1 : 0;
}

int rtx_cull_rect(const rt_render_params *p, int32_t W, int32_t H, const float box[6], int32_t out[4]) {
  return p && box && out && cull_rect(p, W, H, box, nullptr, 0, out) ? 1 : 0;
}

int rtx_set_tile_cull(int on) {
  g_tile_cull.store(on < 0 ? tile_cull_env() : (on != 0));
  return RT_OK;
}

int rtx_set_queue_heads(int heads) {
  if (heads >= 0 && !rtq::heads_ok((uint32_t)heads)) return set_err(RT_E_INVALID, "queue heads: 8, 16, 32 or 64");
  g_queue_heads.store(heads < 0 ? queue_heads_env() : heads);
  return RT_OK;
}

int rtx_queue_item(uint32_t items, uint32_t heads, uint32_t head, uint32_t k, uint32_t *item) {
  if (!item || !rtq::heads_ok(heads) || head >= heads) return set_err(RT_E_INVALID, "bad queue head");
  *item = rtq::item(items, heads, head, k);
  return RT_OK;
}
int64_t rtx_queue_cap(uint32_t items, uint32_t heads, uint32_t head) {
  if (!rtq::heads_ok(heads) || head >= heads) return -1;
  return (int64_t)rtq::cap(items, heads, head);
}

int rtx_queue_grid(const uint32_t *cull_x, const uint32_t *cull_y, int32_t frames, int32_t W, int32_t rows,
                   uint32_t gx, uint32_t gy, uint32_t out[4]) {
  if (!cull_x || !cull_y || !out || frames < 0 || W <= 0 || rows <= 0 || gx < 1 || gx > 2 || gy < 1 || gy > 2)
    return set_err(RT_E_INVALID, "bad queue grid");
  const rtq::Grid g = rtq::grid(cull_x, cull_y, (uint32_t)frames, (uint32_t)W, (uint32_t)rows, gx, gy);
  out[0] = g.ox;
  out[1] = g.oy;
  out[2] = g.tiles_x;
  out[3] = g.tiles_y;
  return RT_OK;
}

int rtx_set_queue_grid(int on) {
  g_queue_grid.store(on < 0 ? queue_grid_env() : (on != 0));
  return RT_OK;
}

int rtx_set_band_order(int on) {
  g_band_order.store(on < 0 ? band_order_env() : (on != 0));
  return RT_OK;
}

int rtx_set_persist_stamps(void *d_buf, int64_t cap_waves) {
  g_persist_stamps = (unsigned long long *)d_buf;
  g_persist_stamps_cap = d_buf ? cap_waves : 0;
  return RT_OK;
}

int rtx_set_coop(rt_scene *s, int on) {
  if (!s) return set_err(RT_E_INVALID, "scene is NULL");
  s->info.coop = on != 0;
  return RT_OK;
}


int rtx_set_refill(int32_t lanes) {
  g_refill.store((lanes >= 1 && lanes <= 64) ? lanes : RT_REFILL_MIN);
  return RT_OK;
}

int rtx_set_pump(rt_scene *s, int on) {
  if (!s) return set_err(RT_E_INVALID, "scene is NULL");
  s->info.pump_on = on != 0;
  return RT_OK;
}

int rtx_set_schedule(rt_scene *s, int on) {
  if (!s) return set_err(RT_E_INVALID, "scene is NULL");
  s->info.sched_on = on != 0;
  s->sched.key[0] = s->sched.key[1] = 0;
  return RT_OK;
}

int rt_bench_frames(rt_scene *s, const rt_render_params *params, int32_t frames, int32_t W, int32_t H,
                    uint32_t flags, float *mean_ms, float *total_ms) {
  if (!s || !params || frames <= 0) return set_err(RT_E_INVALID, "bad arguments");
  int rc = no_instanced(s, "rt_bench_frames");
  if (rc) return rc;
  if ((rc = check_params(params, W, H))) return rc;
  const size_t px = (size_t)W * H;
  if ((rc = ensure_fb(s, px)) || (rc = ensure_events(s))) return rc;
  HIP_TRY(hipMemset(s->fb.t.p, 0x7f, px * 4));
  HIP_TRY(hipDeviceSynchronize());
  HIP_TRY(hipEventRecord(s->fb.ev0.e, 0));
  for (int32_t f = 0; f < frames; ++f) {
    FrameArgs fa;
    if ((rc = check_params(params + f, W, H)) ||
        (rc = fill_frame(fa, s, params + f, s->fb.color.p, s->fb.t.p, W, H, flags, nullptr)) ||
        (rc = launch_render(s, fa, 0)))
      return rc;
  }
  HIP_TRY(hipEventRecord(s->fb.ev1.e, 0));
  HIP_TRY(hipEventSynchronize(s->fb.ev1.e));
  float ms = 0.0f;
  HIP_TRY(hipEventElapsedTime(&ms, s->fb.ev0.e, s->fb.ev1.e));
  if (total_ms) *total_ms = ms;
  if (mean_ms) *mean_ms = ms / (float)frames;
  return RT_OK;
}

}

namespace {

template <class S, int SLOTS>
__global__ __launch_bounds__(kBlock) void rays_kernel(S sc, PlaneDev pl, const float *o3,
                                                       const float *d3, int64_t n, float tn,
                                                       float tf, int32_t *hit, float *t,
                                                       float *nrm, int64_t *prim) {
  __shared__ uint32_t stk[stack_words<S, SLOTS>() * kBlock];
  const int64_t i = (int64_t)blockIdx.x * kBlock + threadIdx.x;
  if (i >= n) return;
  StackOf<S, kBlock> st{stk + threadIdx.x};
  const f3 o{o3[3 * i], o3[3 * i + 1], o3[3 * i + 2]};
  const f3 d{d3[3 * i], d3[3 * i + 1], d3[3 * i + 2]};
  NoCnt cnt;
  const SurfHit sh = union_intersect<S, kBlock>(sc, pl, o, d, tn, tf, st, cnt);
  hit[i] = sh.h.hit ? 1 : 0;
  t[i] = sh.h.t;
  nrm[3 * i] = sh.h.n.x;
  nrm[3 * i + 1] = sh.h.n.y;
  nrm[3 * i + 2] = sh.h.n.z;
  prim[i] = sh.h.hit ? sh.h.prim : -1;
}

constexpr int kRBlock = 64;
constexpr int64_t kMaxRayBlocks = (int64_t)(0xFFFFFFFFu / (uint32_t)kRBlock);

template <int B, bool NORMAL, class CT>
__device__ __forceinline__ Hit rays_closest(const MeshS &sc, f3 o, f3 d, float tn, float tf,
                                            LdsStack<B, MeshS::kFields> st, bool want_prim, CT &cnt) {
  float t;
  uint32_t k;
  Hit h = miss_hit();
  if (mesh_trace<B, false>(sc.d, o, d, tn, tf, st, t, k, cnt)) {
    h.hit = true;
    h.t = t;
    if constexpr (NORMAL) h.n = tri_normal(sc.d.tris, k);
    if (want_prim) h.prim = (int64_t)sc.d.tris[k].orig_id;
  }
  return h;
}
template <int B, bool NORMAL, int kMode, class CT>
__device__ __forceinline__ Hit rays_closest(const GridS<kMode> &sc, f3 o, f3 d, float tn, float tf,
                                            LdsStack<B, GridS<kMode>::kFields>, bool, CT &cnt) {
  Hit h = miss_hit();
  f3 p;
  uint32_t cell;
  if (grid_march<kMode>(sc.d, o, d, tn, tf, h.t, p, cell, cnt)) {
    h.hit = true;
    if constexpr (NORMAL) h.n = grid_normal<kMode>(sc.d, p, cnt);
    h.prim = (int64_t)cell;
  } else {
    h.t = kInf;
  }
  return h;
}
template <int B, bool NORMAL, bool PACK, class CT>
__device__ __forceinline__ Hit rays_closest(const OctS<PACK> &sc, f3 o, f3 d, float tn, float tf,
                                            LdsStack<B, kOctFields> st, bool, CT &cnt) {
  Hit h = miss_hit();
  uint32_t node;
  if (oct_trace<B, NORMAL, PACK>(sc.d, o, d, tn, tf, st, h.t, h.n, node, cnt)) {
    h.hit = true;
    h.prim = (int64_t)node;
  } else {
    h.t = kInf;
  }
  return h;
}

template <class S, int SLOTS, int MODE>
constexpr int trace_min_waves() {
  return (S::kCoop && SLOTS <= 7 && MODE != kRaysAny) ? S::kMinWaves : 1;
}
template <class S, int SLOTS, int MODE>
__global__ __launch_bounds__(kRBlock) __attribute__((amdgpu_waves_per_eu(trace_min_waves<S, SLOTS, MODE>())))
void trace_rays_kernel(S sc, PlaneDev pl, rt_ray_batch b) {
  __shared__ uint32_t stk[stack_words<S, SLOTS>() * kRBlock];
  const int64_t i = (int64_t)blockIdx.x * kRBlock + threadIdx.x;
  const bool active = i < b.n;
  StackOf<S, kRBlock> st{stk + threadIdx.x};
  f3 o{0.0f, 0.0f, 0.0f}, d{0.0f, 0.0f, 1.0f};
  float tn = b.tnear, tf = b.tfar;
  if (active) {
    o = f3{b.d_origin[3 * i], b.d_origin[3 * i + 1], b.d_origin[3 * i + 2]};
    d = f3{b.d_dir[3 * i], b.d_dir[3 * i + 1], b.d_dir[3 * i + 2]};
    if (b.d_tnear) tn = b.d_tnear[i];
    if (b.d_tfar) tf = b.d_tfar[i];
  }
  NoCnt cnt;
  if constexpr (MODE == kRaysAny) {
    if (active) b.d_hit[i] = union_occluded<S, kRBlock>(sc, pl, o, d, tn, tf, st, cnt) ? 1 : 0;
  } else {
    Hit h = miss_hit();
    bool traced = false;
    if constexpr (std::is_same_v<S, MeshS>) {
      if (!b.d_tnear) {
        float t;
        uint32_t k;
        if (mesh_primary_wave<kRBlock, MeshS::kFields>(sc.d, o, d, tn, tf, active, stk, t, k) && active) {
          h.hit = true;
          h.t = t;
          if constexpr (MODE == kRaysNormal) h.n = tri_normal(sc.d.tris, k);
          if (b.d_prim) h.prim = (int64_t)sc.d.tris[k].orig_id;
        }
        traced = true;
      }
    }
    if (!active) return;
    if (!traced) h = rays_closest<kRBlock, MODE == kRaysNormal>(sc, o, d, tn, tf, st, b.d_prim != nullptr, cnt);
    store_closest<MODE>(b, i, pl, RayIn{o, d, tn, tf}, h);
  }
}

template <class S, int MAXD>
void launch_rays_t(const S &sc, const PlaneDev &pl, const float *o, const float *d, int64_t n,
                   float tn, float tf, int32_t *hit, float *t, float *nrm, int64_t *prim) {
  const int64_t blocks = (n + kBlock - 1) / kBlock;
  rays_kernel<S, MAXD><<<(unsigned)blocks, kBlock>>>(sc, pl, o, d, n, tn, tf, hit, t, nrm, prim);
}

template <class S, int MAXD>
void launch_trace_t(const S &sc, const PlaneDev &pl, const rt_ray_batch &b, int mode, hipStream_t stream) {
  const unsigned blocks = (unsigned)((b.n + kRBlock - 1) / kRBlock);
  with_mode(mode, [&](auto m) {
    trace_rays_kernel<S, MAXD, decltype(m)::value><<<blocks, kRBlock, 0, stream>>>(sc, pl, b);
  });
}

int launch_trace(rt_scene *s, const rt_ray_batch &b, int mode, hipStream_t stream) {
  if (s->info.kind == RT_SCENE_INSTANCED) {
    if (int rc = rti::instanced_sync(s, stream)) return rc;
    const rti::InstArgs a{s->inst.recs.p, s->inst.tab.p, s->inst.n, s->info.maxd, s->inst.tlas.p, s->inst.tlas_leaves};
    if (s->inst.mixed.p) return rti::trace_mixed_launch(rti::MixedArgs{a, s->inst.mixed.p}, s->info.plane, b, mode, stream);
    return s->inst.tlas.p ? rti::trace_tlas_launch(a, s->info.plane, b, mode, stream)
                     : rti::trace_instances_launch(a, s->info.plane, b, mode, stream);
  }
  if (!dispatch_scene(s, [&](const auto &sc, auto slots) {
        launch_trace_t<std::decay_t<decltype(sc)>, decltype(slots)::value>(sc, s->info.plane, b, mode, stream);
      }))
    return set_err(RT_E_STATE, "scene has no geometry");
  HIP_TRY(hipGetLastError());
  return RT_OK;
}

}

extern "C" {

int rt_intersect_rays(rt_scene *s, const float *o, const float *d, int64_t n, float tnear, float tfar,
                      int32_t *hit, float *t, float *normal, int64_t *prim) {
  if (!s || !o || !d || !hit || !t || !normal || !prim) return set_err(RT_E_INVALID, "NULL argument");
  if (n <= 0) return RT_OK;
  const size_t m = (size_t)n;
  rtmem::DevArray<float> aO, aD, aT, aN;
  rtmem::DevArray<int32_t> aH;
  rtmem::DevArray<int64_t> aP;
  hipError_t e = hipSuccess;
  do {
    if ((e = aO.alloc_e(3 * m)) || (e = aD.alloc_e(3 * m)) || (e = aT.alloc_e(m)) || (e = aN.alloc_e(3 * m)) ||
        (e = aH.alloc_e(m)) || (e = aP.alloc_e(m)))
      break;
    float *const dO = aO.p, *const dD = aD.p, *const dT = aT.p, *const dN = aN.p;
    int32_t *const dH = aH.p;
    int64_t *const dP = aP.p;
    if ((e = rtdma::h2d(dO, o, n * 12, nullptr)) || (e = rtdma::h2d(dD, d, n * 12, nullptr))) break;
    if (s->info.kind == RT_SCENE_INSTANCED) {
      const rt_ray_batch b{n, dO, dD, nullptr, nullptr, tnear, tfar, dH, dT, dN, dP};
      if (const int rc = launch_trace(s, b, kRaysNormal, nullptr)) return rc;
    } else if (!dispatch_scene(s, [&](const auto &sc, auto slots) {
                 launch_rays_t<std::decay_t<decltype(sc)>, decltype(slots)::value>(sc, s->info.plane, dO, dD, n, tnear,
                                                                                   tfar, dH, dT, dN, dP);
               })) {
      return set_err(RT_E_STATE, "rt_intersect_rays: scene has no geometry");
    }
    if ((e = hipGetLastError())) break;
    if ((e = rtdma::d2h(hit, dH, n * 4, nullptr)) || (e = rtdma::d2h(t, dT, n * 4, nullptr)) ||
        (e = rtdma::d2h(normal, dN, n * 12, nullptr)) || (e = rtdma::d2h(prim, dP, n * 8, nullptr)))
      break;
  } while (0);
  if (e != hipSuccess) return set_err(RT_E_DEVICE, std::string("rt_intersect_rays: ") + hipGetErrorString(e));
  return RT_OK;
}

int rt_trace_rays_device(rt_scene *s, const rt_ray_batch *b, uint32_t flags, void *stream) {
  if (!s) return set_err(RT_E_INVALID, "scene is NULL");
  if (!b) return set_err(RT_E_INVALID, "ray batch is NULL");
  if (flags & ~RT_RAYS_ANY_HIT) return set_err(RT_E_INVALID, "unknown ray flag");
  if (b->n < 0) return set_err(RT_E_INVALID, "negative ray count");
  if (!b->d_origin || !b->d_dir) return set_err(RT_E_INVALID, "NULL ray origins or directions");
  if (!b->d_hit && !b->d_t && !b->d_normal && !b->d_prim) return set_err(RT_E_INVALID, "no output buffer");
  const bool any = (flags & RT_RAYS_ANY_HIT) != 0;
  if (any && (!b->d_hit || b->d_t || b->d_normal || b->d_prim))
    return set_err(RT_E_INVALID, "RT_RAYS_ANY_HIT writes d_hit only: d_t, d_normal and d_prim must be NULL");
  if (b->n / kRBlock + (b->n % kRBlock != 0) > kMaxRayBlocks)
    return set_err(RT_E_INVALID, "ray count exceeds one launch (" + std::to_string(kMaxRayBlocks * kRBlock) +
                                     " rays): split the batch");
  if (b->n == 0) return RT_OK;
  return launch_trace(s, *b, any ? kRaysAny : b->d_normal ? kRaysNormal : kRaysClosest, (hipStream_t)stream);
}

}
```

### triangles-sdf-cpu-raytracing_amd/csrc/rt_host.cpp

```cpp
#include "rt_host.h"

#include <algorithm>
#include <cmath>
#include <cstdio>
#include <cstdlib>
#include <cstring>
#include <limits>
#include <unordered_map>
#include <utility>
#include <vector>
#ifdef _OPENMP
#include <immintrin.h>
#include <omp.h>
#endif

namespace rth {

static const float kInf = std::numeric_limits<float>::infinity();

static bool read_file(const char *path, std::vector<char> &buf, std::string &err) {
  FILE *f = std::fopen(path, "rb");
  if (!f) { err = std::string("cannot open ") + path; return false; }
  std::fseek(f, 0, SEEK_END);
  long n = std::ftell(f);
// ... 291 lines not shown
      if (start < nearest && nearest < end) res.divider = nearest;
      else if (start < other && other < end) res.divider = other;
    }
    return res;
  }
  std::vector<Box> &rightB_for(int axis) { return rightB[axis]; }

  static constexpr size_t kAxesTaskMin = 1024;

  Div try_divide(size_t start, size_t end) {
    if (end - start <= 8 * 3) return Div{};
    std::copy(cur.begin() + start / 3, cur.begin() + end / 3, scrY.begin() + start / 3);
    std::copy(cur.begin() + start / 3, cur.begin() + end / 3, scrZ.begin() + start / 3);
    const float curSAH = static_cast<float>(end - start) / 3.0f;
    Div dx, dy, dz;
    if (end - start >= 3 * kAxesTaskMin) {
#pragma omp task shared(dy)
      dy = try_axis(scrY, start, end, 1);
#pragma omp task shared(dz)
      dz = try_axis(scrZ, start, end, 2);
      dx = try_axis(cur, start, end, 0);
#pragma omp taskwait
    } else {
      dx = try_axis(cur, start, end, 0);
      dy = try_axis(scrY, start, end, 1);
      dz = try_axis(scrZ, start, end, 2);
    }
    const float m = std::min({curSAH, dx.sah, dy.sah, dz.sah});
    if (dx.sah == m) return dx;
    if (dy.sah == m) {
      std::copy(scrY.begin() + start / 3, scrY.begin() + end / 3, cur.begin() + start / 3);
      return dy;
    }
    if (dz.sah == m) {
      std::copy(scrZ.begin() + start / 3, scrZ.begin() + end / 3, cur.begin() + start / 3);
      return dz;
    }
    return Div{};
  }

  int32_t alloc_node() {
    int32_t id;
#pragma omp critical(rt_bvh_nodes)
    {
      id = (int32_t)nodes.size();
      nodes.emplace_back();
    }
    return id;
  }

  void create(int32_t self, size_t start, size_t end) {
    size_t dividers[20] = {};
    size_t nd = 0;
    std::pair<size_t, size_t> q[40];
    int qf = 0, qr = -1, qc = 0;
    auto enq = [&](size_t a, size_t b) {
      if (qc == 40) return;
      qr = (qr + 1) % 40;
      q[qr] = {a, b};
      ++qc;
    };
    enq(start, end);
    while (qc) {
      auto c = q[qf];
      qf = (qf + 1) % 40;
      --qc;
      if (nd == 7) break;
      Div r = try_divide(c.first, c.second);
      if (r.divided) {
        dividers[nd++] = r.divider;
        enq(c.first, r.divider);
        enq(r.divider, c.second);
      }
    }
    HNode node;
    if (nd == 0) {
      if (end - start > 24) {
        dividers[nd++] = ((start / 3 + end / 3) / 2) * 3;
      } else {
        node.leaf = true;
        node.start = (uint32_t)start;
        node.count = (uint32_t)(end - start);
#pragma omp critical(rt_bvh_nodes)
        nodes[self] = node;
        return;
      }
    }
    std::sort(dividers, dividers + nd);
    node.nchild = (uint32_t)(nd + 1);
    size_t lo[8], hi[8];
    for (size_t c = 0; c <= nd; ++c) {
      lo[c] = (c == 0) ? start : dividers[c - 1];
      hi[c] = (c == nd) ? end : dividers[c];
      Box b = empty_box();
      for (size_t t = lo[c] / 3; t < hi[c] / 3; ++t) grow(b, triBox[cur[t]]);
      node.box[c] = b;
      node.child[c] = alloc_node();
    }
#pragma omp critical(rt_bvh_nodes)
    nodes[self] = node;
    for (size_t c = 0; c <= nd; ++c) {
      const int32_t ch = node.child[c];
      const size_t a = lo[c], b = hi[c];
      if (b - a > 3 * 2048) {
#pragma omp task firstprivate(ch, a, b)
        create(ch, a, b);
      } else {
        create(ch, a, b);
      }
    }
#pragma omp taskwait
  }
};

}

bool build_bvh8(const float *vpos4, int64_t nverts, const uint32_t *idx, int64_t nidx, BVHGpu &out,
                std::string &err, unsigned want) {
  if (nidx < 0 || nidx % 3 != 0) { err = "index count must be a multiple of 3"; return false; }
  const size_t ntri = (size_t)nidx / 3;
  for (int64_t i = 0; i < nidx; ++i)
    if ((int64_t)idx[i] >= nverts) { err = "vertex index out of range"; return false; }
  if (ntri > rtl::kMaxLeafFirstTri) { err = "too many triangles"; return false; }
  out = BVHGpu();
  if (ntri == 0) { out.root_word = rtl::kInvalidChild; return true; }

  Builder B;
  B.triBox.resize(ntri);
  for (int a = 0; a < 3; ++a) B.key[a].resize(ntri);
  for (size_t t = 0; t < ntri; ++t) {
    Box b = empty_box();
    for (int k = 0; k < 3; ++k) {
      const float *v = vpos4 + 4 * (size_t)idx[3 * t + k];
      const float w = v[3];
      Box p{{v[0] / w, v[1] / w, v[2] / w}, {v[0] / w, v[1] / w, v[2] / w}};
      grow(b, p);
    }
    B.triBox[t] = b;
    for (int a = 0; a < 3; ++a) B.key[a][t] = b.mx[a];
  }
  B.cur.resize(ntri);
  for (size_t t = 0; t < ntri; ++t) B.cur[t] = (uint32_t)t;
  B.scrY.resize(ntri);
  B.scrZ.resize(ntri);
  for (int a = 0; a < 3; ++a) B.rightB[a].resize(ntri);
  B.nodes.reserve(ntri + 16);
  B.nodes.emplace_back();
#pragma omp parallel
  {
#pragma omp single
    B.create(0, 0, (size_t)nidx);
  }

  bvh_layout(vpos4, idx, nidx, B.nodes, B.cur, out, want, true);
  return true;
}

void bvh_layout(const float *vpos4, const uint32_t *idx, int64_t nidx, HostNodes H,
                const std::vector<uint32_t> &cur, BVHGpu &out, unsigned want, bool host_tris) {
  (void)nidx;
  out.host_nodes = (int64_t)H.size();
  if (want & kBvhPerm) out.perm_tri = cur;
  if (want & kBvhCanon) {
    out.canon.reserve(H.size() * 52);
    std::vector<int32_t> st{0};
    while (!st.empty()) {
      int32_t id = st.back();
      st.pop_back();
      const HNode &n = H[id];
      uint32_t rec[52] = {};
      rec[0] = n.leaf;
      rec[1] = n.leaf ? n.count : n.nchild;
      rec[2] = n.leaf ? n.start : 0;
      if (!n.leaf) {
        float bx[48];
        for (int c = 0; c < 8; ++c) {
          const bool v = (uint32_t)c < n.nchild;
          bx[0 * 8 + c] = v ? n.box[c].mn[0] : kInf;
          bx[1 * 8 + c] = v ? n.box[c].mn[1] : kInf;
          bx[2 * 8 + c] = v ? n.box[c].mn[2] : kInf;
          bx[3 * 8 + c] = v ? n.box[c].mx[0] : kInf;
          bx[4 * 8 + c] = v ? n.box[c].mx[1] : kInf;
          bx[5 * 8 + c] = v ? n.box[c].mx[2] : kInf;
        }
        std::memcpy(rec + 4, bx, 192);
        for (int c = (int)n.nchild - 1; c >= 0; --c) st.push_back(n.child[c]);
      }
      out.canon.insert(out.canon.end(), rec, rec + 52);
    }
  }

  std::vector<std::pair<uint32_t, uint32_t>> leaf_fill;
  std::vector<uint32_t> leaf_cnt;
  uint32_t next_slot = 0;
  auto leaf_word = [&](const HNode &n) -> uint32_t {
    const uint32_t first = next_slot, nt = n.count / 3;
    if (nt == 0) return rtl::kInvalidChild;
    next_slot += nt;
    leaf_fill.push_back({first, n.start / 3});
    leaf_cnt.push_back(nt);
    return rtl::kLeafBit | (first << 3) | (nt - 1);
  };
  auto fill_tris = [&]() {
    out.n_tris = next_slot;
    if (!(want & kBvhTris)) return;
    if (!host_tris) {
      out.leaf_tab.resize(3 * leaf_fill.size());
      for (size_t l = 0; l < leaf_fill.size(); ++l) {
        out.leaf_tab[3 * l] = leaf_fill[l].first;
        out.leaf_tab[3 * l + 1] = leaf_fill[l].second;
        out.leaf_tab[3 * l + 2] = leaf_cnt[l];
      }
      return;
    }
    out.tris.resize(next_slot);
#pragma omp parallel for schedule(dynamic, 256)
    for (int64_t l = 0; l < (int64_t)leaf_fill.size(); ++l) {
      for (uint32_t k = 0; k < leaf_cnt[l]; ++k) {
        const uint32_t slot = leaf_fill[l].second + k;
        const uint32_t *tv = idx + 3 * (size_t)cur[slot];
        float v[3][3];
        for (int j = 0; j < 3; ++j) {
          const float *p = vpos4 + 4 * (size_t)tv[j];
          const float w = p[3];
          v[j][0] = p[0] / w; v[j][1] = p[1] / w; v[j][2] = p[2] / w;
        }
        rtl::GTri &g = out.tris[leaf_fill[l].first + k];
        g.v0x = v[0][0]; g.v0y = v[0][1]; g.v0z = v[0][2];
        g.orig_id = cur[slot];
        g.e1x = v[1][0] - v[0][0]; g.e1y = v[1][1] - v[0][1]; g.e1z = v[1][2] - v[0][2];
        g.e2x = v[2][0] - v[0][0]; g.e2y = v[2][1] - v[0][1]; g.e2z = v[2][2] - v[0][2];
        g.pad1 = g.pad2 = 0.0f;
      }
    }
  };

  if (H[0].leaf) {
    out.root_word = leaf_word(H[0]);
    fill_tris();
    out.max_depth = 0;
    out.host_inner = 0;
    return;
  }
  std::vector<int32_t> order{0};
  std::vector<int32_t> depth_of{1};
  std::vector<int32_t> gpu_id(H.size(), -1);
  gpu_id[0] = 0;
  for (size_t i = 0; i < order.size(); ++i) {
    const HNode &n = H[order[i]];
    for (uint32_t c = 0; c < n.nchild; ++c) {
      const int32_t ch = n.child[c];
      if (!H[ch].leaf) {
        gpu_id[ch] = (int32_t)order.size();
        order.push_back(ch);
        depth_of.push_back(depth_of[i] + 1);
      }
    }
  }
  out.host_inner = (int64_t)order.size();
  out.nodes.resize(order.size());
  for (size_t i = 0; i < order.size(); ++i) {
    const HNode &n = H[order[i]];
    rtl::GNode &g = out.nodes[i];
    out.max_depth = std::max(out.max_depth, depth_of[i]);
    for (int c = 0; c < 8; ++c) {
      if ((uint32_t)c < n.nchild) {
        for (int k = 0; k < 3; ++k) { g.box[c][2 * k] = n.box[c].mn[k]; g.box[c][2 * k + 1] = n.box[c].mx[k]; }
        const HNode &ch = H[n.child[c]];
        g.child[c] = ch.leaf ? leaf_word(ch) : (uint32_t)gpu_id[n.child[c]];
      } else {
        for (int k = 0; k < 6; ++k) g.box[c][k] = kInf;
        g.child[c] = rtl::kInvalidChild;
      }
    }
  }
  out.root_word = 0;
  {
    const HNode &r = H[0];
    Box u = empty_box();
    for (uint32_t c = 0; c < r.nchild; ++c) grow(u, r.box[c]);
    for (int k = 0; k < 3; ++k) { out.root_box[k] = u.mn[k]; out.root_box[3 + k] = u.mx[k]; }
  }
  fill_tris();
}

std::vector<uint32_t> bvh_level_first(const std::vector<rtl::GNode> &nodes) {
  std::vector<uint32_t> first;
  if (nodes.empty()) return first;
  uint32_t lo = 0, hi = 1;
  for (;;) {
    first.push_back(lo);
    uint32_t last = 0;
    for (uint32_t i = lo; i < hi; ++i)
      for (uint32_t w : nodes[i].child)
        if (!(w & rtl::kLeafBit)) last = std::max(last, w);
    if (last < hi || last >= nodes.size()) break;
    lo = hi;
    hi = last + 1;
  }
  first.push_back((uint32_t)nodes.size());
  return first;
}

void refit_bvh8(BVHGpu &b, const float *vpos4, const uint32_t *idx) {
  auto leaf_box = [&](uint32_t word) {
    const uint32_t first = (word & ~rtl::kLeafBit) >> 3, nt = (word & 7u) + 1u;
    Box box = empty_box();
    for (uint32_t k = 0; k < nt; ++k) {
      rtl::GTri &g = b.tris[first + k];
      const uint32_t *tv = idx + 3 * (size_t)g.orig_id;
      float v[3][3];
      for (int j = 0; j < 3; ++j) {
        const float *p = vpos4 + 4 * (size_t)tv[j];
        const float w = p[3];
        v[j][0] = p[0] / w; v[j][1] = p[1] / w; v[j][2] = p[2] / w;
        grow(box, Box{{v[j][0], v[j][1], v[j][2]}, {v[j][0], v[j][1], v[j][2]}});
      }
      g.v0x = v[0][0]; g.v0y = v[0][1]; g.v0z = v[0][2];
      g.e1x = v[1][0] - v[0][0]; g.e1y = v[1][1] - v[0][1]; g.e1z = v[1][2] - v[0][2];
      g.e2x = v[2][0] - v[0][0]; g.e2y = v[2][1] - v[0][1]; g.e2z = v[2][2] - v[0][2];
      g.pad1 = g.pad2 = 0.0f;
    }
    return box;
  };
  auto node_box = [&](const rtl::GNode &n) {
    Box u = empty_box();
    for (int c = 0; c < 8; ++c)
      if (n.child[c] != rtl::kInvalidChild)
        grow(u, Box{{n.box[c][0], n.box[c][2], n.box[c][4]}, {n.box[c][1], n.box[c][3], n.box[c][5]}});
    return u;
  };
  if (b.nodes.empty()) {
    if (b.root_word != rtl::kInvalidChild) leaf_box(b.root_word);
    return;
  }
  for (size_t i = b.nodes.size(); i-- > 0;) {
    rtl::GNode &n = b.nodes[i];
    for (int c = 0; c < 8; ++c) {
      const uint32_t w = n.child[c];
      if (w == rtl::kInvalidChild) continue;
      const Box box = (w & rtl::kLeafBit) ? leaf_box(w) : node_box(b.nodes[w]);
      for (int k = 0; k < 3; ++k) { n.box[c][2 * k] = box.mn[k]; n.box[c][2 * k + 1] = box.mx[k]; }
    }
  }
  const Box u = node_box(b.nodes[0]);
  for (int k = 0; k < 3; ++k) { b.root_box[k] = u.mn[k]; b.root_box[3 + k] = u.mx[k]; }
}

bool flatten_octree(const uint8_t *nodes36, int64_t count, OctGpu &out, std::string &err) {
  out = OctGpu();
  if (count <= 0) { err = "empty octree"; return false; }
  out.child.resize((size_t)count);
  out.vals.resize((size_t)count);
  for (int64_t i = 0; i < count; ++i) {
    float v[8];
    uint32_t off;
    std::memcpy(v, nodes36 + 36 * i, 32);
    std::memcpy(&off, nodes36 + 36 * i + 32, 4);
    std::memcpy(out.vals[(size_t)i].v, v, 32);
    if (off == 0) {
      bool all10 = true, all0 = true, allAbove = true;
      for (int k = 0; k < 8; ++k) {
        all10 = all10 && (v[k] > 10.0f);
        all0 = all0 && (v[k] == 0.0f);
        allAbove = allAbove && (v[k] >= 1e-4f);
      }
      out.child[(size_t)i] = rtl::OctWord{(all10 || all0 || allAbove) ? rtl::kOctNeverHits : 0u, 0u};
    } else {
      if ((int64_t)off + 7 >= count || off == rtl::kOctNeverHits) { err = "octree child offset out of range"; return false; }
      out.child[(size_t)i] = rtl::OctWord{off, 0u};
    }
  }
  constexpr int8_t kUnseen = -1, kOpen = -2;
  std::vector<int8_t> can((size_t)count, kUnseen);
  std::vector<int8_t> height((size_t)count, 0);
  std::vector<std::pair<uint32_t, bool>> post{{0u, false}};
  while (!post.empty()) {
    auto [n, expanded] = post.back();
    post.pop_back();
    const uint32_t c = out.child[n].child;
    if (!expanded) {
      if (can[n] >= 0) continue;
      if (can[n] == kOpen) { err = "octree is cyclic"; return false; }
      if (c == 0 || c == rtl::kOctNeverHits) {
        can[n] = c == 0 ? 1 : 0;
        continue;
      }
      can[n] = kOpen;
      post.push_back({n, true});
      for (int k = 0; k < 8; ++k)
        if (can[c + k] < 0) post.push_back({c + (uint32_t)k, false});
      continue;
    }
    uint32_t m = 0;
    int h = 0;
    for (int k = 0; k < 8; ++k) {
      if (can[c + k] > 0) m |= 1u << k;
      if (out.child[c + k].child == 0) m |= 1u << (8 + k);
      h = std::max(h, (int)height[c + k]);
    }
    if (h + 1 > 24) { err = "octree is deeper than 24 levels"; return false; }
    height[n] = (int8_t)(h + 1);
    out.child[n].masks = m;
    can[n] = (m & 0xFFu) ? 1 : 0;
  }
  out.max_depth = height[0];
  return true;
}

namespace {
struct V3 { float x, y, z; };
static inline V3 sub(V3 a, V3 b) { return {a.x - b.x, a.y - b.y, a.z - b.z}; }
static inline float dot3(V3 a, V3 b) { return a.x * b.x + a.y * b.y + a.z * b.z; }
static inline V3 crs(V3 a, V3 b) { return {a.y * b.z - a.z * b.y, a.z * b.x - a.x * b.z, a.x * b.y - a.y * b.x}; }
static inline V3 nrm(V3 a) { float l = std::sqrt(dot3(a, a)); return {a.x / l, a.y / l, a.z / l}; }
struct M4 { float m[4][4]; float &at(int r, int c) { return m[c][r]; } };
static M4 look_at(V3 eye, V3 center, V3 up) {
  V3 z = nrm(sub(eye, center));
  V3 x = nrm(crs(up, z));
  V3 y = nrm(crs(z, x));
  M4 M{};
  M.at(0, 0) = x.x; M.at(0, 1) = x.y; M.at(0, 2) = x.z; M.at(0, 3) = -dot3(x, eye);
  M.at(1, 0) = y.x; M.at(1, 1) = y.y; M.at(1, 2) = y.z; M.at(1, 3) = -dot3(y, eye);
  M.at(2, 0) = z.x; M.at(2, 1) = z.y; M.at(2, 2) = z.z; M.at(2, 3) = -dot3(z, eye);
  M.at(3, 3) = 1.0f;
  return M;
}
static void invert(M4 &A, float out[16]) {
  double a[4][8];
  for (int r = 0; r < 4; ++r)
    for (int c = 0; c < 4; ++c) { a[r][c] = A.at(r, c); a[r][c + 4] = (r == c) ? 1.0 : 0.0; }
  for (int c = 0; c < 4; ++c) {
    int p = c;
    for (int r = c + 1; r < 4; ++r) if (std::fabs(a[r][c]) > std::fabs(a[p][c])) p = r;
    if (p != c) for (int k = 0; k < 8; ++k) std::swap(a[p][k], a[c][k]);
    const double piv = a[c][c];
    for (int k = 0; k < 8; ++k) a[c][k] /= piv;
    for (int r = 0; r < 4; ++r) {
      if (r == c) continue;
      const double f = a[r][c];
      if (f == 0.0) continue;
      for (int k = 0; k < 8; ++k) a[r][k] -= f * a[c][k];
    }
  }
  for (int r = 0; r < 4; ++r)
    for (int c = 0; c < 4; ++c) out[c * 4 + r] = (float)a[r][c + 4];
}
struct Q { float x, y, z, w; };
static inline Q qmul(Q a, Q b) {
  return {a.w * b.x + a.x * b.w + a.y * b.z - a.z * b.y, a.w * b.y - a.x * b.z + a.y * b.w + a.z * b.x,
          a.w * b.z + a.x * b.y - a.y * b.x + a.z * b.w, a.w * b.w - a.x * b.x - a.y * b.y - a.z * b.z};
}
}

namespace {
Q orientation_of(V3 P, V3 T, V3 U) {
  M4 m = look_at(P, T, U);
  Q q;
  if (m.at(2, 2) < 0) {
    if (m.at(0, 0) > m.at(1, 1)) {
      float t = 1 + m.at(0, 0) - m.at(1, 1) - m.at(2, 2);
      q = {t, m.at(0, 1) + m.at(1, 0), m.at(2, 0) + m.at(0, 2), m.at(1, 2) - m.at(2, 1)};
    } else {
      float t = 1 - m.at(0, 0) + m.at(1, 1) - m.at(2, 2);
      q = {m.at(0, 1) + m.at(1, 0), t, m.at(1, 2) + m.at(2, 1), m.at(2, 0) - m.at(0, 2)};
    }
  } else {
    if (m.at(0, 0) < -m.at(1, 1)) {
      float t = 1 - m.at(0, 0) - m.at(1, 1) + m.at(2, 2);
      q = {m.at(2, 0) + m.at(0, 2), m.at(1, 2) + m.at(2, 1), t, m.at(0, 1) - m.at(1, 0)};
    } else {
      float t = 1 + m.at(0, 0) + m.at(1, 1) + m.at(2, 2);
      q = {m.at(1, 2) - m.at(2, 1), m.at(2, 0) - m.at(0, 2), m.at(0, 1) - m.at(1, 0), t};
    }
  }
  return q;
}
V3 rotate_vector(V3 v, Q q) {
  const Q p{v.x, v.y, v.z, 0.0f}, c{-q.x, -q.y, -q.z, q.w};
  const Q r = qmul(qmul(q, p), c);
  return {r.x, r.y, r.z};
}
Q angle_axis(float angle, V3 axis) {
  const V3 n = nrm(axis);
  const float half = angle * 0.5f;
  Q q;
  q.w = std::cos(half);
  q.x = n.x * std::sin(half);
  q.y = n.y * std::sin(half);
  q.z = n.z * std::sin(half);
  return q;
}
V3 v3(const float *p) { return {p[0], p[1], p[2]}; }
void put(float *o, V3 v) { o[0] = v.x; o[1] = v.y; o[2] = v.z; }
Q q_of(const CamState &c) { return {c.q[0], c.q[1], c.q[2], c.q[3]}; }
void set_q(CamState &c, Q q) { c.q[0] = q.x; c.q[1] = q.y; c.q[2] = q.z; c.q[3] = q.w; }
V3 cam_up_v(const CamState &c) { return nrm(rotate_vector({0.0f, 1.0f, 0.0f}, q_of(c))); }
V3 cam_right_v(const CamState &c) { return nrm(rotate_vector({1.0f, 0.0f, 0.0f}, q_of(c))); }
V3 cam_forward_v(const CamState &c) { return nrm(sub(v3(c.target), v3(c.pos))); }
float len3(V3 a) { return std::sqrt(dot3(a, a)); }
}

void cam_init(CamState &c, const float pos[3], const float target[3], const float up[3]) {
  c = CamState{};
  put(c.pos, v3(pos));
  put(c.target, v3(target));
  set_q(c, orientation_of(v3(pos), v3(target), v3(up)));
  c.sens = 0.01f;
}

void cam_rotate(CamState &c, float dx, float dy) {
  const float pitch = dy * c.sens, yaw = dx * c.sens;
  const Q q_yaw = angle_axis(yaw, cam_up_v(c));
  const Q q_pitch = angle_axis(pitch, cam_right_v(c));
  const Q r = qmul(qmul(q_pitch, q_yaw), q_of(c));
  const float n = std::sqrt(r.x * r.x + r.y * r.y + r.z * r.z + r.w * r.w);
  set_q(c, Q{r.x / n, r.y / n, r.z / n, r.w / n});
  const V3 f = nrm(rotate_vector({0.0f, 0.0f, -1.0f}, q_of(c)));
  const V3 T = v3(c.target);
  const float dist = len3(sub(T, v3(c.pos)));
  put(c.pos, sub(T, V3{f.x * dist, f.y * dist, f.z * dist}));
  if (c.lock) set_q(c, orientation_of(v3(c.pos), T, v3(c.locked)));
}

void cam_reset_position(CamState &c, const float pos[3]) {
  const V3 up = cam_up_v(c);
  put(c.pos, v3(pos));
  set_q(c, orientation_of(v3(c.pos), v3(c.target), up));
}

void cam_reset_target(CamState &c, const float target[3]) {
  const V3 up = cam_up_v(c);
  put(c.target, v3(target));
  set_q(c, orientation_of(v3(c.pos), v3(c.target), up));
}

void cam_set_lock_up(CamState &c, bool on) {
  if (!c.lock && on) put(c.locked, cam_up_v(c));
  c.lock = on ? 1 : 0;
}

void cam_zoom(CamState &c, float wheel) {
  const float dist = len3(sub(v3(c.target), v3(c.pos)));
  const float r = wheel * dist / 25.0f;
  const V3 f = cam_forward_v(c);
  const V3 P = v3(c.pos);
  const float np[3] = {P.x + f.x * r, P.y + f.y * r, P.z + f.z * r};
  cam_reset_position(c, np);
}

void cam_basis(const CamState &c, float up[3], float right[3], float forward[3]) {
  if (up) put(up, cam_up_v(c));
  if (right) put(right, cam_right_v(c));
  if (forward) put(forward, cam_forward_v(c));
}

void cam_view_inverse(const CamState &c, float view_inv[16]) {
  M4 view = look_at(v3(c.pos), v3(c.target), cam_up_v(c));
  invert(view, view_inv);
}

bool save_obj(const char *path, const float *vpos4, int64_t nverts, const uint32_t *idx, int64_t nidx,
              const float *vnorm4, const float *vtex2, std::string &err) {
  if (!path || (!vpos4 && nverts) || (!idx && nidx) || nidx % 3 != 0) { err = "bad arguments"; return false; }
  FILE *f = std::fopen(path, "wb");
  if (!f) { err = std::string("cannot create ") + path; return false; }
  auto num = [](float x) { return std::to_string(x); };
  std::string v, tc, n, fc;
  for (int64_t i = 0; i < nverts; ++i) {
    const float *p = vpos4 + 4 * i;
    v += "v " + num(p[0]) + " " + num(p[1]) + " " + num(p[2]) + "\n";
    const float nx = vnorm4 ? vnorm4[4 * i] : 0.0f, ny = vnorm4 ? vnorm4[4 * i + 1] : 0.0f,
                nz = vnorm4 ? vnorm4[4 * i + 2] : 1.0f;
    n += "vn " + num(nx) + " " + num(ny) + " " + num(nz) + "\n";
    tc += "vt " + num(vtex2 ? vtex2[2 * i] : 0.0f) + " " + num(vtex2 ? vtex2[2 * i + 1] : 0.0f) + "\n";
  }
  for (int64_t t = 0; t < nidx / 3; ++t) {
    fc += "f";
    for (int k = 0; k < 3; ++k) {
      const std::string q = std::to_string(idx[3 * t + k] + 1);
      fc += " " + q + "/" + q + "/" + q;
    }
    fc += "\n";
  }
  const std::string all = "# obj file created by custom obj loader\no MainModel\n" + v + tc + n + "s off\n" + fc;
  const size_t wrote = std::fwrite(all.data(), 1, all.size(), f);
  std::fclose(f);
  if (wrote != all.size()) { err = "short write"; return false; }
  return true;
}

namespace {
uint32_t crc32(const uint8_t *p, size_t n, uint32_t c = 0xFFFFFFFFu) {
  static uint32_t table[256];
  static bool init = false;
  if (!init) {
    for (uint32_t i = 0; i < 256; ++i) {
      uint32_t v = i;
      for (int k = 0; k < 8; ++k) v = (v & 1) ? 0xEDB88320u ^ (v >> 1) : v >> 1;
      table[i] = v;
    }
    init = true;
  }
  for (size_t i = 0; i < n; ++i) c = table[(c ^ p[i]) & 0xFF] ^ (c >> 8);
  return c;
}
// ... 150 lines not shown
```

### triangles-sdf-cpu-raytracing_amd/csrc/rt_host.h

```cpp
#pragma once
#include <stdint.h>

#include <cstdlib>
#include <string>
#include <utility>
#include <vector>

#include "rt_layout.h"

#ifndef RT_AB_ENV
#define RT_AB_ENV 0
#endif
inline const char *ab_env(const char *name) {
#if RT_AB_ENV
  return std::getenv(name);
#else
  (void)name;
  return nullptr;
#endif
}
inline bool ab_on(const char *name) {
  const char *e = ab_env(name);
  return e && e[0] == '1';
}
inline bool ab_off(const char *name) {
  const char *e = ab_env(name);
  return e && e[0] == '0';
}
inline long long ab_int(const char *name, long long dflt, long long lo, long long hi) {
  const char *e = ab_env(name);
  const long long v = e ? std::atoll(e) : dflt;
  return v >= lo && v <= hi ? v : dflt;
}

namespace rth {

struct Mesh {
  std::vector<float> vpos4;
  std::vector<uint32_t> idx;
};

bool load_obj(const char *path, bool scale, Mesh &out, std::string &err);
bool load_grid(const char *path, uint32_t size[3], std::vector<float> &values, std::string &err);
bool load_octree(const char *path, std::vector<uint8_t> &nodes36, std::string &err);

enum : unsigned {
  kBvhCanon = 1,
  kBvhPerm = 2,
  kBvhTris = 4,
  kBvhDeviceTris = 8,
  kBvhAll = kBvhCanon | kBvhPerm | kBvhTris,
};
struct DevBuffer {
  void *p = nullptr;
  size_t bytes = 0;
  void (*release)(void *) = nullptr;
  DevBuffer() = default;
  DevBuffer(const DevBuffer &) = delete;
  DevBuffer &operator=(const DevBuffer &) = delete;
  DevBuffer(DevBuffer &&o) noexcept { swap(o); }
  DevBuffer &operator=(DevBuffer &&o) noexcept {
    DevBuffer t(std::move(o));
    swap(t);
    return *this;
  }
  ~DevBuffer() {
    if (p && release) release(p);
  }
  void swap(DevBuffer &o) noexcept {
    std::swap(p, o.p);
    std::swap(bytes, o.bytes);
    std::swap(release, o.release);
  }
  void *take() {
    void *q = p;
    p = nullptr;
    return q;
  }
};
struct BVHGpu {
  std::vector<rtl::GNode> nodes;
  std::vector<rtl::GTri> tris;
  DevBuffer dev_tris;
  uint32_t n_tris = 0;
  uint32_t root_word = rtl::kInvalidChild;
  float root_box[6] = {0, 0, 0, 0, 0, 0};
  int32_t max_depth = 0;
  int64_t host_nodes = 0, host_inner = 0;
  std::vector<uint32_t> canon;
  std::vector<uint32_t> perm_tri;
  std::vector<uint32_t> leaf_tab;
};
bool build_bvh8(const float *vpos4, int64_t nverts, const uint32_t *idx, int64_t nidx, BVHGpu &out,
                std::string &err, unsigned want = kBvhAll);

struct BvhBox {
  float mn[3], mx[3];
};
struct BvhHostNode {
  bool leaf = false;
  uint32_t start = 0, count = 0;
  uint32_t nchild = 0;
  int32_t child[8] = {-1, -1, -1, -1, -1, -1, -1, -1};
  BvhBox box[8];
};
void host_introsort(uint32_t *ids, size_t n, const float *K, int64_t depth_limit);
struct HostNodes {
  const BvhHostNode *p;
  size_t n;
  HostNodes(const std::vector<BvhHostNode> &v) : p(v.data()), n(v.size()) {}
  HostNodes(const BvhHostNode *ptr, size_t count) : p(ptr), n(count) {}
  size_t size() const { return n; }
  const BvhHostNode &operator[](size_t i) const { return p[i]; }
};
void bvh_layout(const float *vpos4, const uint32_t *idx, int64_t nidx, HostNodes H,
                const std::vector<uint32_t> &cur, BVHGpu &out, unsigned want, bool host_tris);
std::vector<uint32_t> bvh_level_first(const std::vector<rtl::GNode> &nodes);
void refit_bvh8(BVHGpu &b, const float *vpos4, const uint32_t *idx);
bool build_bvh8_gpu(const float *vpos4, int64_t nverts, const uint32_t *idx, int64_t nidx, BVHGpu &out,
                    std::string &err, unsigned want = kBvhAll);

struct OctGpu {
  std::vector<rtl::OctWord> child;
  std::vector<rtl::OctVals> vals;
  int32_t max_depth = 0;
};
bool flatten_octree(const uint8_t *nodes36, int64_t count, OctGpu &out, std::string &err);

constexpr int kSdfFeatures = 7;
struct SdfMeshHost {
  BVHGpu bvh;
  std::vector<float> tri;
  std::vector<float> pn;
};
struct SdfTopo {
  std::vector<uint32_t> weld;
  std::vector<uint32_t> tri_edge;
  std::vector<uint32_t> v_off;
  std::vector<uint32_t> v_inc;
  std::vector<uint32_t> e_off;
  std::vector<uint32_t> e_inc;
  uint32_t n_wverts = 0, n_wedges = 0;
};
bool prep_sdf_mesh(const float *vpos4, int64_t nverts, const uint32_t *idx, int64_t nidx,
                   SdfMeshHost &out, std::string &err, SdfTopo *topo = nullptr);
void refit_sdf_mesh(SdfMeshHost &m, const SdfTopo &topo, const uint32_t *idx, int64_t nidx, const float *new_vpos4);

bool subdivide_mesh(const float *vpos4, int64_t nverts, const uint32_t *idx, int64_t nidx, int levels,
                    Mesh &out, std::string &err);

using SdfQuery = bool (*)(void *ctx, const float *p3, int64_t n, float *out, std::string &err);
bool build_sdf_octree(SdfQuery query, void *ctx, int depth, std::vector<uint8_t> &nodes36,
                      std::string &err);

struct CamState {
  float pos[3], target[3], q[4];
  float sens;
  int32_t lock;
  float locked[3];
};
void cam_init(CamState &c, const float pos[3], const float target[3], const float up[3]);
void cam_rotate(CamState &c, float dx, float dy);
void cam_reset_position(CamState &c, const float pos[3]);
void cam_reset_target(CamState &c, const float target[3]);
void cam_set_lock_up(CamState &c, bool on);
void cam_zoom(CamState &c, float wheel);
void cam_basis(const CamState &c, float up[3], float right[3], float forward[3]);
void cam_view_inverse(const CamState &c, float view_inv[16]);

bool save_obj(const char *path, const float *vpos4, int64_t nverts, const uint32_t *idx, int64_t nidx,
              const float *vnorm4, const float *vtex2, std::string &err);

bool write_png(const char *path, const uint32_t *rgba, int32_t W, int32_t H, std::string &err);

void camera_matrices(const float pos[3], const float target[3], const float up[3], float fovy,
                     float aspect, float znear, float zfar, float view_inv[16], float proj_inv[16]);

void copy_rect(uint32_t *dc, float *dt, const uint32_t *sc, const float *st, int64_t W, int32_t x0, int32_t x1,
               int32_t y0, int32_t y1, int threads);
void copy_spans(uint32_t *dc, float *dt, uint32_t *sc, float *st, int64_t W, int32_t H, const int32_t *span,
                int threads, bool clear_src = false);
void clear_frame(uint32_t *c, float *t, int64_t n, int threads);

}
```

### triangles-sdf-cpu-raytracing_amd/csrc/rt_scene.h

```cpp
#pragma once
#include <hip/hip_runtime.h>
#include <stdint.h>

#include <vector>

#include "../../include/rtamd.h"
#include "rt_error.h"
#include "rt_frame.h"
#include "rt_instances.h"
#include "rt_layout.h"
#include "rt_mem.h"
#include "rt_scenes.h"

namespace rts {

struct Common {
  int kind = 0;
  int32_t maxd = 1;
  rtd::PlaneDev plane{};
  uint64_t version = 0;
  int64_t dev_bytes = 0;
  bool sched_on = true;
  bool coop = true;
  bool pump_on = false;
};

struct MeshDesc {
  uint32_t root = rtl::kInvalidChild;
  float root_box[6] = {0, 0, 0, 0, 0, 0};
  float root_child[48] = {};
  int64_t host_nodes = 0, host_inner = 0;
  uint32_t n_inner = 0;
  float dmax2 = 0.0f;
  int32_t depth = 0;
  uint32_t n_tris = 0;
  uint32_t root_nchild = 0;
};

struct GridDesc {
  uint32_t size[3] = {0, 0, 0};
  bool bricked = false;
};

struct OctDesc {
  int32_t depth = 0;
};

struct Geometry {
  rtmem::DevArray<rtl::GNode> nodes;
  rtmem::DevArray<rtl::GTri> tris;
  rtmem::DevArray<float> vals;
  rtmem::DevArray<rtl::OctWord> child;
  rtmem::DevArray<rtl::OctVals> ovals;
};

struct Dynamic {
  bool on = false;
  int64_t nverts = 0;
  rtmem::DevArray<uint32_t> idx;
  rtmem::DevArray<float> vstage;
  rtmem::DevArray<uint32_t> edge;
  rtmem::Pinned<uint32_t> h_refit;
  std::vector<uint32_t> level_first;
  int64_t bytes = 0;
};

struct OctDynamic {
  bool on = false;
  uint32_t max_nodes = 0;
  rtmem::DevArray<uint32_t> status;
  rtmem::DevArray<rtl::OctWord> s_child;
  rtmem::DevArray<rtl::OctVals> s_vals;
  rtmem::DevArray<uint64_t> cells;
  rtmem::DevArray<uint32_t> flag, bsum, lvl;
  rtmem::DevArray<float> top;
  int64_t bytes = 0;
};

struct Instanced {
  rtmem::DevArray<rti::InstRec> recs;
  rtmem::DevArray<rtd::MeshDev> tab;
  int32_t n = 0;
  std::vector<rt_scene *> blas;
  std::vector<uint64_t> blas_seen;
  rtmem::DevArray<rti::BlasRec> mixed;
  rtmem::DevArray<rtt::TNode> tlas;
  rtmem::DevArray<float> xform;
  int32_t tlas_leaves = 0;
};

struct Frame {
  rtmem::DevArray<uint32_t> color;
  rtmem::DevArray<float> t;
  size_t cap = 0;
  rtmem::Event ev0, ev1;
};

struct Schedule {
  rtmem::DevArray<uint32_t> cost[2], order[2];
  uint32_t key[2] = {0, 0};
  bool rec[2] = {false, false};
  int par = 0;
  uint32_t cap = 0;
  hipStream_t last_stream = nullptr;
  rtmem::Stream os;
  rtmem::Event ord_ev[2], frame_ev;
};

struct Dropin {
  rtmem::Stream xs[2];
  rtmem::Event xev;
  rtmem::Event ev_host;
  rtmem::DevArray<int32_t> hit_box;
  rtmem::Pinned<int32_t> h_hit_box;
  rtmem::DevArray<int32_t> row_span;
  rtmem::Pinned<int32_t> h_row_span;
  int32_t span_cap = 0;
  rtdma::HostStage stage{hipHostMallocDefault};
};

}

struct rt_scene {
  int device = 0;
  rts::Common info;
  rts::MeshDesc mesh;
  rts::GridDesc grid;
  rts::OctDesc oct;
  rts::Geometry geo;
  rts::Dynamic dyn;
  rts::OctDynamic octdyn;
  rts::Instanced inst;
  rts::Frame fb;
  rts::Schedule sched;
  rts::Dropin drop;
};

namespace rti {

rtd::MeshDev mesh_dev(const rt_scene *s);
rtd::GridDev grid_dev(const rt_scene *s);
int grid_mode(const rt_scene *s, const rtd::GridDev &gd);
int no_instanced(const rt_scene *s, const char *who);
rti::TlasArgs tlas_args(const rt_scene *s);
int instanced_sync(rt_scene *s, hipStream_t stream);

int ensure_fb(rt_scene *s, size_t px);
int ensure_events(rt_scene *s);
int fill_frame(FrameArgs &fa, const rt_scene *s, const rt_render_params *p, uint32_t *c, float *t, int32_t W,
               int32_t H, uint32_t flags, const rt_tile *tile);
int launch_render(rt_scene *s, const FrameArgs &fa, hipStream_t stream, unsigned long long *counters = nullptr,
                  int diag = 0, bool sched = true);
int launch_batch(rt_scene *s, FrameBatch &fb, int n, hipStream_t stream);


}
```

### triangles-sdf-cpu-raytracing_amd/csrc/rt_scene.hip

```cpp
#include <hip/hip_runtime.h>

#include <algorithm>
#include <cmath>
#include <cstdio>
#include <cstring>
#include <limits>
#include <string>
#include <vector>

#include "../../include/rtamd.h"
#include "rt_dispatch.h"
#include "rt_error.h"
#include "rt_host.h"
#include "rt_refit.h"
#include "rt_scene.h"
#include "rt_sdf_octree.h"
#include "rt_shade.h"

using namespace rtd;
using namespace rti;

namespace {

uint64_t grid_bricked_samples(const uint32_t size[3]) {
  return (uint64_t)grid_bricks(size[0]) * grid_bricks(size[1]) * grid_bricks(size[2]) * 64u;
}

uint64_t grid_samples(const rt_scene *s) {
  return s->grid.bricked ? grid_bricked_samples(s->grid.size) : (uint64_t)s->grid.size[0] * s->grid.size[1] * s->grid.size[2];
}

int g_grid_force = 0;

}

namespace rti {

GridDev grid_dev(const rt_scene *s) {
  const uint64_t n = grid_samples(s);
  const uint32_t bytes = 4 * n < (1ull << 32) ? (uint32_t)(4 * n) : 0u;
  if (!s->grid.bricked) return GridDev{s->geo.vals.p, s->grid.size[0], s->grid.size[1], s->grid.size[2], s->grid.size[2],
                                       s->grid.size[1] * s->grid.size[2], bytes};
  const uint32_t ys = grid_bricks(s->grid.size[2]) * 64u;
  return GridDev{s->geo.vals.p, s->grid.size[0], s->grid.size[1], s->grid.size[2], ys, grid_bricks(s->grid.size[1]) * ys, bytes};
}

int grid_mode(const rt_scene *s, const GridDev &gd) {
  const bool buf = gd.bytes != 0 && gd.xs < (1u << 24) && gd.ys < (1u << 24) && !(g_grid_force & 2);
  return (buf ? kGridBuf : 0) | (s->grid.bricked ? kGridBricked : 0);
}

}

namespace {

__global__ __launch_bounds__(256) void brick_kernel(const float *__restrict__ src, float *__restrict__ dst,
                                                    uint32_t sx, uint32_t sy, uint32_t sz, uint64_t n) {
  const uint64_t i = (uint64_t)blockIdx.x * 256 + threadIdx.x;
  if (i >= n) return;
  const uint32_t nby = grid_bricks(sy), nbz = grid_bricks(sz);
  const uint32_t l = (uint32_t)(i & 63u);
  const uint64_t b = i >> 6;
  const uint32_t bz = (uint32_t)(b % nbz), by = (uint32_t)((b / nbz) % nby), bx = (uint32_t)(b / nbz / nby);
  const uint32_t x = bx * 4 + (l >> 4), y = by * 4 + ((l >> 2) & 3u), z = bz * 4 + (l & 3u);
  dst[i] = (x < sx && y < sy && z < sz) ? src[((uint64_t)x * sy + y) * sz + z] : 0.0f;
}

__global__ __launch_bounds__(256) void grid_copy_kernel(const float *__restrict__ src, float *__restrict__ dst, uint64_t n) {
  const uint64_t i = (uint64_t)blockIdx.x * 256 + threadIdx.x;
  if (i < n) dst[i] = src[i];
}

}

namespace rti {

MeshDev mesh_dev(const rt_scene *s) {
  MeshDev m{s->geo.nodes.p, s->geo.tris.p, s->mesh.root, {}, s->info.coop, s->mesh.dmax2};
  for (int k = 0; k < 6; ++k) m.rbox[k] = s->mesh.root_box[k];
  return m;
}

int no_instanced(const rt_scene *s, const char *who) {
  if (s && s->info.kind == RT_SCENE_INSTANCED)
    return set_err(RT_E_STATE, std::string(who) + ": not available for an instanced scene");
  return RT_OK;
}

int instanced_sync(rt_scene *s, hipStream_t stream) {
  for (size_t j = 0; j < s->inst.blas.size(); ++j) {
    if (s->inst.blas[j]->info.version == s->inst.blas_seen[j]) continue;
    rtd::MeshDev *entry = s->inst.mixed.p ? &(s->inst.mixed.p + j)->mesh : s->inst.tab.p + j;
    if (int rc = rti::blas_entry_launch(entry, mesh_dev(s->inst.blas[j]), stream)) return rc;
    s->inst.blas_seen[j] = s->inst.blas[j]->info.version;
    if (!s->inst.tlas.p) continue;
    const rti::TlasArgs t = rti::tlas_args(s);
    if (int rc = s->inst.mixed.p ? rti::mixed_boxes_launch(t, s->inst.mixed.p, 0, s->inst.n, nullptr, (int32_t)j, stream)
                            : rti::tlas_boxes_launch(t, 0, s->inst.n, nullptr, (int32_t)j, stream))
      return rc;
    if (int rc = rti::tlas_refit_launch(t, stream)) return rc;
  }
  return RT_OK;
}

rti::TlasArgs tlas_args(const rt_scene *s) {
  return rti::TlasArgs{s->inst.tlas.p, s->inst.tlas_leaves, s->inst.n, s->inst.recs.p, s->inst.xform.p, s->inst.tab.p};
}

}

namespace {

int pick_maxd(int depth, int32_t &maxd) {
  const int need = depth > 1 ? depth - 1 : 1;
  const int options[] = {4, 7, 15, 31};
  for (int m : options)
    if (need <= m) { maxd = m; return RT_OK; }
  return set_err(RT_E_INVALID, "tree deeper than 32 levels");
}

}

namespace {
int g_bvh_mode = RT_BVH_AUTO;
constexpr int64_t kBvhDeviceMinTris = 32768;

thread_local int t_bvh_last = 0;

int build_bvh(const float *vpos4, int64_t nverts, const uint32_t *idx, int64_t nidx, rth::BVHGpu &b,
              unsigned want) {
  std::string err;
  int ndev = 0;
  const bool dev = g_bvh_mode == RT_BVH_DEVICE ||
                   (g_bvh_mode == RT_BVH_AUTO && nidx / 3 >= kBvhDeviceMinTris &&
                    hipGetDeviceCount(&ndev) == hipSuccess && ndev > 0);
  bool fell_back = false;
  if (dev) {
    if (rth::build_bvh8_gpu(vpos4, nverts, idx, nidx, b, err, want)) {
      t_bvh_last = 2;
      return RT_OK;
    }
    if (err.rfind("GPU BVH builder bound", 0) == 0) return set_err(RT_E_DEVICE, err);
    const bool device_failure = err.rfind("GPU BVH build:", 0) == 0;
    if (!device_failure) return set_err(RT_E_INVALID, err);
    if (g_bvh_mode == RT_BVH_DEVICE) return set_err(RT_E_DEVICE, err);
    if (const hipError_t e = hipDeviceSynchronize(); e != hipSuccess)
      return set_err(RT_E_DEVICE, err + "; device unusable afterwards: " + hipGetErrorString(e));
    (void)hipGetLastError();
    std::fprintf(stderr, "rtamd: %s; building the BVH on the host instead\n", err.c_str());
    fell_back = true;
    err.clear();
  }
  if (!rth::build_bvh8(vpos4, nverts, idx, nidx, b, err, want)) return set_err(RT_E_INVALID, err);
  t_bvh_last = fell_back ? 3 : 1;
  return RT_OK;
}

int new_scene(rt_scene **out) {
  if (!out) return set_err(RT_E_INVALID, "out is NULL");
  int dev = 0;
  HIP_TRY(hipGetDevice(&dev));
  rt_scene *s = new rt_scene();
  s->device = dev;
  s->info.plane.on = 0;
  s->info.plane.n = f3{0.0f, 1.0f, 0.0f};
  *out = s;
  return RT_OK;
}

}

extern "C" {

int rt_set_bvh_builder(int mode) {
  if (mode < RT_BVH_AUTO || mode > RT_BVH_DEVICE) return set_err(RT_E_INVALID, "bad BVH builder mode");
  g_bvh_mode = mode;
  return RT_OK;
}

int rt_bvh_export(const float *vpos4, int64_t nverts, const uint32_t *idx, int64_t nidx,
                  uint32_t *canon, int64_t *nnodes, uint32_t *perm_tri, int32_t *max_depth) {
  if (!vpos4 || !idx || !nnodes || nverts <= 0 || nidx <= 0) return set_err(RT_E_INVALID, "bad mesh");
  rth::BVHGpu b;
  const unsigned want = (canon ? rth::kBvhCanon : 0u) | (perm_tri ? rth::kBvhPerm : 0u);
  if (int rc = build_bvh(vpos4, nverts, idx, nidx, b, want)) return rc;
  const int64_t n = canon ? (int64_t)b.canon.size() / 52 : b.host_nodes;
  if (canon) {
    if (*nnodes < n) return set_err(RT_E_INVALID, "buffer too small");
    std::memcpy(canon, b.canon.data(), b.canon.size() * 4);
  }
  if (perm_tri) std::memcpy(perm_tri, b.perm_tri.data(), b.perm_tri.size() * 4);
  if (max_depth) *max_depth = b.max_depth;
  *nnodes = n;
  return RT_OK;
}

__global__ void tri_edge_bound_kernel(const rtl::GTri *__restrict__ tris, uint32_t n, uint32_t *out) {
  const uint32_t i = blockIdx.x * blockDim.x + threadIdx.x;
  float m = 0.0f;
  if (i < n) {
    const float4 *q = reinterpret_cast<const float4 *>(tris + i);
    const float4 b = q[1], c = q[2];
    const float v = __builtin_sqrtf(b.x * b.x + b.y * b.y + b.z * b.z) *
                    __builtin_sqrtf(c.x * c.x + c.y * c.y + c.z * c.z);
    m = __builtin_isnan(v) ? kInf : v;
  }
  for (int off = 32; off > 0; off >>= 1) m = __builtin_fmaxf(m, __shfl_xor(m, off, 64));
  if ((threadIdx.x & 63) == 0 && m > 0.0f) atomicMax(out, __float_as_uint(m));
}

float dmax2_of(uint32_t edge_bits) {
  float M;
  std::memcpy(&M, &edge_bits, 4);
  if (M == 0.0f) return std::numeric_limits<float>::max();
  if (!std::isfinite(M)) return 0.0f;
  const double r = std::ldexp(1.0, 124) / (2.0 * (double)M * (1.0 + 1e-6));
  const double r2 = r * r;
  return r2 >= (double)std::numeric_limits<float>::max() ? std::numeric_limits<float>::max()
                                                          : std::nextafter((float)r2, 0.0f);
}
int mesh_dmax2(rt_scene *s, uint32_t n_tris) {
  s->mesh.dmax2 = 0.0f;
  if (n_tris == 0) return RT_OK;
  rtmem::DevArray<uint32_t> d;
  uint32_t h = 0;
  if (int rc = d.alloc(1)) return rc;
  hipError_t e = hipMemset(d.p, 0, 4);
  if (e == hipSuccess) {
    tri_edge_bound_kernel<<<(n_tris + 255) / 256, 256>>>(s->geo.tris.p, n_tris, d.p);
    e = hipGetLastError();
  }
  if (e == hipSuccess) e = hipMemcpy(&h, d.p, 4, hipMemcpyDeviceToHost);
  if (e != hipSuccess) return set_err(RT_E_DEVICE, std::string("triangle edge bound: ") + hipGetErrorString(e));
  s->mesh.dmax2 = dmax2_of(h);
  return RT_OK;
}

int rt_scene_create_mesh(const float *vpos4, int64_t nverts, const uint32_t *idx, int64_t nidx,
                         rt_scene **out) {
  return rt_scene_create_mesh_ex(vpos4, nverts, idx, nidx, 0u, out);
}

int rt_scene_create_mesh_ex(const float *vpos4, int64_t nverts, const uint32_t *idx, int64_t nidx,
                            uint32_t flags, rt_scene **out) {
  if (!vpos4 || !idx || nverts <= 0 || nidx <= 0) return set_err(RT_E_INVALID, "empty mesh");
  if (flags & ~RT_MESH_DYNAMIC) return set_err(RT_E_INVALID, "rt_scene_create_mesh_ex: unknown flags");
  rth::BVHGpu b;
  if (int rc = build_bvh(vpos4, nverts, idx, nidx, b, rth::kBvhTris | rth::kBvhDeviceTris)) return rc;
  int32_t maxd = 8;
  int rc = pick_maxd(b.max_depth, maxd);
  if (rc) return rc;
  rt_scene *s;
  if ((rc = new_scene(&s))) return rc;
  s->info.kind = RT_SCENE_MESH;
  s->info.maxd = maxd;
  s->mesh.root = b.root_word;
  std::memcpy(s->mesh.root_box, b.root_box, sizeof(s->mesh.root_box));
  if (!(b.root_word & rtl::kLeafBit) && b.root_word < b.nodes.size())
    std::memcpy(s->mesh.root_child, b.nodes[b.root_word].box, sizeof(s->mesh.root_child));
  s->mesh.host_nodes = b.host_nodes;
  s->mesh.host_inner = b.host_inner;
  s->mesh.depth = b.max_depth;
  s->mesh.n_inner = (uint32_t)b.nodes.size();
  if (b.dev_tris.p) {
    s->info.dev_bytes += (int64_t)b.dev_tris.bytes;
    s->geo.tris.adopt(b.dev_tris);
  }
  if ((rc = s->geo.nodes.upload(b.nodes.data(), b.nodes.size(), s->info.dev_bytes)) ||
      (!s->geo.tris.p && (rc = s->geo.tris.upload_padded(b.tris.data(), b.tris.size(), 8, s->info.dev_bytes))) ||
      (rc = mesh_dmax2(s, b.n_tris))) {
    rt_scene_destroy(s);
    return rc;
  }
  s->mesh.n_tris = b.n_tris;
  if (!b.nodes.empty())
    for (uint32_t w : b.nodes[0].child) s->mesh.root_nchild += w != rtl::kInvalidChild;
  if (flags & RT_MESH_DYNAMIC) {
    const int64_t before = s->info.dev_bytes;
    s->dyn.nverts = nverts;
    s->dyn.level_first = rth::bvh_level_first(b.nodes);
    if ((rc = s->dyn.idx.upload(idx, (size_t)nidx, s->info.dev_bytes)) ||
        (rc = s->dyn.vstage.upload(nullptr, 4 * (size_t)nverts, s->info.dev_bytes)) ||
        (rc = s->dyn.edge.upload(nullptr, 1, s->info.dev_bytes)) ||
        (rc = s->dyn.h_refit.alloc(64, hipHostMallocDefault))) {
      rt_scene_destroy(s);
      return rc;
    }
    s->dyn.bytes = s->info.dev_bytes - before;
    s->dyn.on = true;
  }
  *out = s;
  return RT_OK;
}

static int update_vertices_device(rt_scene *s, const float *d_vpos4, hipStream_t st) {
  const rti::RefitArgs a{s->geo.nodes.p, s->geo.tris.p, s->mesh.root, d_vpos4, s->dyn.idx.p, s->dyn.level_first.data(),
                         s->dyn.level_first.empty() ? 0 : (int32_t)s->dyn.level_first.size() - 1};
  if (int rc = rti::refit_launch(a, st)) return rc;
  const bool inner = a.levels > 0;
  HIP_TRY(hipMemsetAsync(s->dyn.edge.p, 0, 4, st));
  if (s->mesh.n_tris) {
    tri_edge_bound_kernel<<<(s->mesh.n_tris + 255) / 256, 256, 0, st>>>(s->geo.tris.p, s->mesh.n_tris, s->dyn.edge.p);
    HIP_TRY(hipGetLastError());
  }
  if (inner) HIP_TRY(hipMemcpyAsync(s->dyn.h_refit.h, s->geo.nodes.p[0].box, 192, hipMemcpyDeviceToHost, st));
  HIP_TRY(hipMemcpyAsync(s->dyn.h_refit.h + 48, s->dyn.edge.p, 4, hipMemcpyDeviceToHost, st));
  HIP_TRY(hipStreamSynchronize(st));
  if (inner) {
    std::memcpy(s->mesh.root_child, s->dyn.h_refit.h, 192);
    const float inf = std::numeric_limits<float>::infinity();
    float mn[3] = {inf, inf, inf}, mx[3] = {-inf, -inf, -inf};
    for (uint32_t c = 0; c < s->mesh.root_nchild; ++c) {
      for (int k = 0; k < 3; ++k) {
        mn[k] = std::min(mn[k], s->mesh.root_child[6 * c + 2 * k]);
        mx[k] = std::max(mx[k], s->mesh.root_child[6 * c + 2 * k + 1]);
      }
    }
    for (int k = 0; k < 3; ++k) { s->mesh.root_box[k] = mn[k]; s->mesh.root_box[3 + k] = mx[k]; }
  }
  s->mesh.dmax2 = s->mesh.n_tris ? dmax2_of(s->dyn.h_refit.h[48]) : 0.0f;
  ++s->info.version;
  return RT_OK;
}

int rt_scene_create_grid(const uint32_t size[3], const float *values, rt_scene **out) {
  if (!size || !values) return set_err(RT_E_INVALID, "NULL argument");
  const uint64_t n = (uint64_t)size[0] * size[1] * size[2];
  if (size[0] < 1 || size[1] < 1 || size[2] < 1 || n > (1ull << 32))
    return set_err(RT_E_INVALID, "bad grid size");
  rt_scene *s;
  int rc = new_scene(&s);
  if (rc) return rc;
  s->info.kind = RT_SCENE_GRID;
  s->grid.size[0] = size[0]; s->grid.size[1] = size[1]; s->grid.size[2] = size[2];
  if ((uint64_t)n * 4 <= kGridLinearMaxBytes && !(g_grid_force & 1)) {
    if ((rc = s->geo.vals.upload(values, (size_t)n, s->info.dev_bytes))) {
      rt_scene_destroy(s);
      return rc;
    }
    *out = s;
    return RT_OK;
  }
  const uint64_t nb = grid_bricked_samples(size);
  if (nb >= (1ull << 32)) {
    rt_scene_destroy(s);
    return set_err(RT_E_INVALID, "bad grid size");
  }
  s->grid.bricked = true;
  rtmem::DevArray<float> ref;
  int64_t staged = 0;
  if ((rc = ref.upload(values, (size_t)n, staged)) ||
      (rc = s->geo.vals.upload(nullptr, (size_t)nb, s->info.dev_bytes))) {
    rt_scene_destroy(s);
    return rc;
  }
  brick_kernel<<<(unsigned)((nb + 255) / 256), 256>>>(ref.p, s->geo.vals.p, size[0], size[1], size[2], nb);
  const hipError_t e1 = hipGetLastError(), e2 = hipDeviceSynchronize();
  if (e1 != hipSuccess || e2 != hipSuccess) {
    rt_scene_destroy(s);
    return set_err(RT_E_DEVICE, std::string("grid bricking: ") + hipGetErrorString(e1 != hipSuccess ? e1 : e2));
  }
  *out = s;
  return RT_OK;
}

int rt_scene_create_octree(const void *nodes36, int64_t count, rt_scene **out) {
  if (!nodes36 || count <= 0) return set_err(RT_E_INVALID, "empty octree");
  rth::OctGpu g;
  std::string err;
  if (!rth::flatten_octree((const uint8_t *)nodes36, count, g, err)) return set_err(RT_E_INVALID, err);
  int32_t maxd = 8;
  int rc = pick_maxd(g.max_depth, maxd);
  if (rc) return rc;
  rt_scene *s;
  if ((rc = new_scene(&s))) return rc;
  s->info.kind = RT_SCENE_OCTREE;
  s->info.maxd = maxd;
  s->oct.depth = g.max_depth;
  if ((rc = s->geo.child.upload(g.child.data(), g.child.size(), s->info.dev_bytes)) ||
      (rc = s->geo.ovals.upload(g.vals.data(), g.vals.size(), s->info.dev_bytes))) {
    rt_scene_destroy(s);
    return rc;
  }
  *out = s;
  return RT_OK;
}

int rt_scene_update_grid_device(rt_scene *s, const float *d_values, void *stream) {
  if (!s) return set_err(RT_E_INVALID, "rt_scene_update_grid_device: scene is NULL");
  if (!d_values) return set_err(RT_E_INVALID, "rt_scene_update_grid_device: values are NULL");
  if (s->info.kind != RT_SCENE_GRID) return set_err(RT_E_STATE, "rt_scene_update_grid_device: not a grid scene");
  int dev = 0;
  HIP_TRY(hipGetDevice(&dev));
  if (s->device != dev)
    return set_err(RT_E_INVALID, "rt_scene_update_grid_device: the scene lives on device " + std::to_string(s->device) +
                                     ", the current one is " + std::to_string(dev));
  const hipStream_t st = (hipStream_t)stream;
  const uint64_t n = grid_samples(s);
  const unsigned blocks = (unsigned)((n + 255) / 256);
  if (s->grid.bricked)
    brick_kernel<<<blocks, 256, 0, st>>>(d_values, s->geo.vals.p, s->grid.size[0], s->grid.size[1], s->grid.size[2], n);
  else
    grid_copy_kernel<<<blocks, 256, 0, st>>>(d_values, s->geo.vals.p, n);
  HIP_TRY(hipGetLastError());
  return RT_OK;
}

int rt_scene_create_octree_dynamic(int32_t depth, int64_t max_nodes, rt_scene **out) {
  if (!out) return set_err(RT_E_INVALID, "rt_scene_create_octree_dynamic: out is NULL");
  if (depth < 0 || depth > 12) return set_err(RT_E_INVALID, "rt_scene_create_octree_dynamic: depth must be in [0, 12]");
  if (max_nodes < 1 || max_nodes > 0xFFFFFFFFll)
    return set_err(RT_E_INVALID, "rt_scene_create_octree_dynamic: max_nodes must be in [1, 2^32 - 1]");
  int32_t maxd = 8;
  int rc = pick_maxd(depth, maxd);
  if (rc) return rc;
  rt_scene *s;
  if ((rc = new_scene(&s))) return rc;
  s->info.kind = RT_SCENE_OCTREE;
  s->info.maxd = maxd;
  s->oct.depth = depth;
  rts::OctDynamic &od = s->octdyn;
  od.on = true;
  od.max_nodes = (uint32_t)max_nodes;
  const size_t C = (size_t)max_nodes;
  rtl::OctWord w0{rtl::kOctNeverHits, 0u};
  rtl::OctVals v0;
  std::fill(v0.v, v0.v + 8, 1000.0f);
  const uint32_t st0[2] = {1u, 0u};
  hipError_t e = hipSuccess;
  auto put = [&](void *d, const void *h, size_t bytes) {
    if (rc == RT_OK && e == hipSuccess) e = rtdma::h2d(d, h, bytes, nullptr);
  };
  if ((rc = s->geo.child.alloc(C)) == RT_OK && (rc = s->geo.ovals.alloc(C)) == RT_OK) {
    s->info.dev_bytes += (int64_t)(s->geo.child.bytes() + s->geo.ovals.bytes());
    put(s->geo.child.p, &w0, sizeof w0);
    put(s->geo.ovals.p, &v0, sizeof v0);
  }
  if (rc == RT_OK) rc = od.status.alloc(2);
  put(od.status.p, st0, sizeof st0);
  if (rc == RT_OK) rc = od.s_child.alloc(C);
  if (rc == RT_OK) rc = od.s_vals.alloc(C);
  if (rc == RT_OK) rc = od.cells.alloc(C);
  if (rc == RT_OK) rc = od.flag.alloc(rtsdf::oct_flag_count(od.max_nodes));
  if (rc == RT_OK) rc = od.bsum.alloc(rtsdf::oct_bsum_count(od.max_nodes));
  if (rc == RT_OK) rc = od.lvl.alloc(rtsdf::kOctLvlWords);
  if (rc == RT_OK) rc = od.top.alloc(std::max<size_t>(rtsdf::oct_top_first(rtsdf::oct_top_levels(depth)), 1));
  if (rc == RT_OK && e != hipSuccess)
    rc = set_err(RT_E_DEVICE, rterr::hip_fail("rt_scene_create_octree_dynamic: upload of the initial tree", e));
  if (rc != RT_OK) {
    rt_scene_destroy(s);
    return rc;
  }
  od.bytes = (int64_t)(od.status.bytes() + od.s_child.bytes() + od.s_vals.bytes() + od.cells.bytes() + od.flag.bytes() +
                       od.bsum.bytes() + od.lvl.bytes() + od.top.bytes());
  s->info.dev_bytes += od.bytes;
  *out = s;
  return RT_OK;
}

static int octree_check(const rt_scene *s, const char *who) {
  if (!s) return set_err(RT_E_INVALID, std::string(who) + ": scene is NULL");
  if (s->info.kind != RT_SCENE_OCTREE) return set_err(RT_E_STATE, std::string(who) + ": not an octree scene");
  return RT_OK;
}
static int octree_status(rt_scene *s, const char *who, uint32_t st[2]) {
  if (int rc = octree_check(s, who)) return rc;
  HIP_TRY(hipSetDevice(s->device));
  HIP_TRY(hipDeviceSynchronize());
  st[0] = (uint32_t)s->geo.child.n;
  st[1] = 0u;
  if (s->octdyn.on) HIP_TRY(rtdma::d2h(st, s->octdyn.status.p, 8, nullptr));
  return RT_OK;
}

static int octree_download(rt_scene *s, const char *who, uint32_t st[2], std::vector<rtl::OctWord> &w,
                           std::vector<rtl::OctVals> *v) {
  if (int rc = octree_check(s, who)) return rc;
  int prev = 0;
  HIP_TRY(hipGetDevice(&prev));
  int rc = octree_status(s, who, st);
  if (rc == RT_OK) {
    w.resize(st[0]);
    hipError_t e = rtdma::d2h(w.data(), s->geo.child.p, (size_t)st[0] * sizeof(rtl::OctWord), nullptr);
    if (e == hipSuccess && v) {
      v->resize(st[0]);
      e = rtdma::d2h(v->data(), s->geo.ovals.p, (size_t)st[0] * sizeof(rtl::OctVals), nullptr);
    }
    if (e != hipSuccess) rc = set_err(RT_E_DEVICE, rterr::hip_fail(who, e));
  }
  HIP_NOTE(hipSetDevice(prev));
  return rc;
}

int rt_scene_octree_status(rt_scene *s, int64_t *count, int32_t *overflow) {
  if (int rc = octree_check(s, "rt_scene_octree_status")) return rc;
  int prev = 0;
  HIP_TRY(hipGetDevice(&prev));
  uint32_t st[2];
  const int rc = octree_status(s, "rt_scene_octree_status", st);
  HIP_NOTE(hipSetDevice(prev));
  if (rc) return rc;
  if (count) *count = (int64_t)st[0];
  if (overflow) *overflow = (int32_t)st[1];
  return RT_OK;
}

int rt_scene_get_octree(rt_scene *s, int64_t *count, void *nodes36) {
  if (!count) return set_err(RT_E_INVALID, "rt_scene_get_octree: count is NULL");
  if (int rc = octree_check(s, "rt_scene_get_octree")) return rc;
  uint32_t st[2];
  if (!nodes36) {
    int prev = 0;
    HIP_TRY(hipGetDevice(&prev));
    const int rc = octree_status(s, "rt_scene_get_octree", st);
    HIP_NOTE(hipSetDevice(prev));
    if (rc == RT_OK) *count = (int64_t)st[0];
    return rc;
  }
  std::vector<rtl::OctWord> w;
  std::vector<rtl::OctVals> v;
  if (int rc = octree_download(s, "rt_scene_get_octree", st, w, &v)) return rc;
  if (*count < (int64_t)st[0]) return set_err(RT_E_INVALID, "rt_scene_get_octree: node buffer too small");
  uint8_t *o = static_cast<uint8_t *>(nodes36);
  for (size_t i = 0; i < w.size(); ++i) {
    const uint32_t off = w[i].child == rtl::kOctNeverHits ? 0u : w[i].child;
    std::memcpy(o + 36 * i, v[i].v, 32);
    std::memcpy(o + 36 * i + 32, &off, 4);
  }
  *count = (int64_t)st[0];
  return RT_OK;
}

int rt_scene_replicate(const rt_scene *src, int device, rt_scene **out) {
  if (!src || !out) return set_err(RT_E_INVALID, "bad arguments");
  if (int rc = no_instanced(src, "rt_scene_replicate")) return rc;
  *out = nullptr;
  int ndev = 0;
  HIP_TRY(hipGetDeviceCount(&ndev));
  if (device < 0 || device >= ndev) return set_err(RT_E_INVALID, "rt_scene_replicate: no such device");
  int prev = 0;
  HIP_TRY(hipGetDevice(&prev));
  HIP_TRY(hipSetDevice(device));
  rt_scene *s = new rt_scene();
  s->device = device;
  s->info = src->info;
  s->mesh = src->mesh;
  s->grid = src->grid;
  s->oct = src->oct;
  s->info.dev_bytes = src->info.dev_bytes - src->dyn.bytes - src->octdyn.bytes;
  hipError_t e = hipSuccess;
  const char *step = "";
  auto copy = [&](auto &to, const auto &from) {
    if (!from.p || e != hipSuccess) return;
    if ((e = to.alloc_e(from.n)) != hipSuccess) { step = "hipMalloc"; return; }
    if ((e = hipMemcpyPeer(to.p, device, from.p, src->device, from.bytes())) != hipSuccess) step = "hipMemcpyPeer";
  };
  copy(s->geo.nodes, src->geo.nodes);
  copy(s->geo.tris, src->geo.tris);
  copy(s->geo.vals, src->geo.vals);
  copy(s->geo.child, src->geo.child);
  copy(s->geo.ovals, src->geo.ovals);
  HIP_NOTE(hipSetDevice(prev));
  if (e != hipSuccess) {
    rt_scene_destroy(s);
    return set_err(RT_E_DEVICE, std::string("rt_scene_replicate: ") + step + ": " + hipGetErrorString(e));
  }
// ... 417 lines not shown
```

### triangles-sdf-cpu-raytracing_amd/rtamd/_lib.py

```python
from __future__ import annotations

import ctypes as C
import os
import subprocess

PKG_ROOT = os.path.dirname(os.path.dirname(os.path.abspath(__file__)))
LIB_PATH = os.environ.get("RTAMD_LIB") or os.path.join(PKG_ROOT, "lib", "librtamd.so")

RT_OK = 0
RT_FLAG_CLEAR = 1
RT_FLAG_TILE_NATURAL = 2
RT_FLAG_HITS_ONLY = 4
RT_RAYS_ANY_HIT = 1
RT_SHADE_CLEAR = 1
RT_POINTS_UNSIGNED = 1
RT_MESH_DYNAMIC = 1
RT_IPC_HANDLE_BYTES = 64
RT_SCENE_MESH, RT_SCENE_GRID, RT_SCENE_OCTREE, RT_SCENE_INSTANCED = 1, 2, 3, 4
RT_INSTANCE_DISABLED = 1
RT_INSTANCED_TLAS = 1

_lib = None


class RtError(RuntimeError):
    pass


class RenderParams(C.Structure):
    _fields_ = [
        ("camera_pos", C.c_float * 3),
        ("view_inv", C.c_float * 16),
        ("proj_inv", C.c_float * 16),
        ("light_pos", C.c_float * 3),
        ("shading_mode", C.c_int32),
        ("enable_shadows", C.c_int32),
        ("enable_reflections", C.c_int32),
        ("reserved", C.c_int32),
    ]


class Tile(C.Structure):
    _fields_ = [("band_rows", C.c_int32), ("rank", C.c_int32), ("num_ranks", C.c_int32),
                ("reserved", C.c_int32)]


class CameraState(C.Structure):
    _fields_ = [("position", C.c_float * 3), ("target", C.c_float * 3), ("orientation", C.c_float * 4),
                ("sensitivity", C.c_float), ("lock_up", C.c_int32), ("locked_up", C.c_float * 3)]


class RayBatch(C.Structure):
    _fields_ = [("n", C.c_int64), ("d_origin", C.c_void_p), ("d_dir", C.c_void_p), ("d_tnear", C.c_void_p),
                ("d_tfar", C.c_void_p), ("tnear", C.c_float), ("tfar", C.c_float), ("d_hit", C.c_void_p),
                ("d_t", C.c_void_p), ("d_normal", C.c_void_p), ("d_prim", C.c_void_p)]


class PointBatch(C.Structure):
    _fields_ = [("n", C.c_int64), ("d_point", C.c_void_p), ("d_radius", C.c_void_p), ("radius", C.c_float),
                ("d_dist", C.c_void_p), ("d_closest", C.c_void_p), ("d_prim", C.c_void_p),
                ("d_feature", C.c_void_p)]


class Instance(C.Structure):
    _fields_ = [("blas", C.c_int32), ("flags", C.c_uint32), ("xform", C.c_float * 12)]


_SIGS = {
    "rt_last_error": (C.c_char_p, []),
    "rt_abi_version": (C.c_int, []),
    "rt_build_id": (C.c_char_p, []),
    "rt_device_count": (C.c_int, []),
    "rt_set_device": (C.c_int, [C.c_int]),
    "rt_load_obj": (C.c_int, [C.c_char_p, C.c_int, C.c_void_p, C.POINTER(C.c_int64), C.c_void_p,
                              C.POINTER(C.c_int64)]),
    "rt_load_grid": (C.c_int, [C.c_char_p, C.c_void_p, C.c_void_p]),
    "rt_load_octree": (C.c_int, [C.c_char_p, C.POINTER(C.c_int64), C.c_void_p]),
    "rt_camera": (C.c_int, [C.c_void_p, C.c_void_p, C.c_void_p, C.c_float, C.c_float, C.c_float,
                            C.c_float, C.c_void_p, C.c_void_p]),
    "rt_bvh_export": (C.c_int, [C.c_void_p, C.c_int64, C.c_void_p, C.c_int64, C.c_void_p,
                                C.POINTER(C.c_int64), C.c_void_p, C.POINTER(C.c_int32)]),
    "rt_set_bvh_builder": (C.c_int, [C.c_int]),
    "rt_scene_create_mesh": (C.c_int, [C.c_void_p, C.c_int64, C.c_void_p, C.c_int64,
                                       C.POINTER(C.c_void_p)]),
    "rt_scene_create_mesh_ex": (C.c_int, [C.c_void_p, C.c_int64, C.c_void_p, C.c_int64, C.c_uint32,
                                          C.POINTER(C.c_void_p)]),
    "rt_scene_update_vertices": (C.c_int, [C.c_void_p, C.c_void_p, C.c_int64]),
    "rt_scene_update_vertices_device": (C.c_int, [C.c_void_p, C.c_void_p, C.c_int64, C.c_void_p]),
    "rt_affine_inverse": (C.c_int, [C.c_void_p, C.c_void_p]),
    "rt_scene_create_instanced": (C.c_int, [C.POINTER(C.c_void_p), C.c_int32, C.POINTER(Instance), C.c_int32,
                                            C.POINTER(C.c_void_p)]),
    "rt_scene_create_instanced_ex": (C.c_int, [C.POINTER(C.c_void_p), C.c_int32, C.POINTER(Instance), C.c_int32,
                                               C.c_uint32, C.POINTER(C.c_void_p)]),
    "rt_scene_create_instanced_any": (C.c_int, [C.POINTER(C.c_void_p), C.c_int32, C.POINTER(Instance), C.c_int32,
                                                C.c_uint32, C.POINTER(C.c_void_p)]),
    "rt_instance_world_box": (C.c_int, [C.c_void_p, C.c_void_p, C.c_void_p]),
    "rt_scene_get_tlas": (C.c_int, [C.c_void_p, C.c_void_p, C.c_void_p, C.POINTER(C.c_int32)]),
    "rt_scene_update_instances": (C.c_int, [C.c_void_p, C.c_int32, C.c_int32, C.POINTER(Instance)]),
    "rt_scene_update_instances_device": (C.c_int, [C.c_void_p, C.c_int32, C.c_int32, C.c_void_p, C.c_void_p]),
    "rt_scene_get_instances": (C.c_int, [C.c_void_p, C.c_int32, C.c_int32, C.POINTER(Instance), C.c_void_p,
                                         C.c_void_p]),
    "rt_scene_create_grid": (C.c_int, [C.c_void_p, C.c_void_p, C.POINTER(C.c_void_p)]),
    "rt_scene_create_octree": (C.c_int, [C.c_void_p, C.c_int64, C.POINTER(C.c_void_p)]),
    "rt_scene_set_plane": (C.c_int, [C.c_void_p, C.c_int, C.c_void_p, C.c_float]),
    "rt_scene_kind": (C.c_int, [C.c_void_p]),
    "rt_scene_device_bytes": (C.c_int64, [C.c_void_p]),
    "rt_scene_bvh_stats": (C.c_int, [C.c_void_p, C.POINTER(C.c_int64), C.POINTER(C.c_int64),
                                     C.POINTER(C.c_int32)]),
    "rt_scene_destroy": (C.c_int, [C.c_void_p]),
    "rt_scene_replicate": (C.c_int, [C.c_void_p, C.c_int, C.POINTER(C.c_void_p)]),
    "rt_scene_device": (C.c_int, [C.c_void_p]),
    "rt_scene_get_plane": (C.c_int, [C.c_void_p, C.POINTER(C.c_int), C.c_void_p, C.POINTER(C.c_float)]),
    "rt_multi_create": (C.c_int, [C.c_void_p, C.c_void_p, C.c_int32, C.c_int32, C.POINTER(C.c_void_p)]),
    "rt_multi_info": (C.c_int, [C.c_void_p, C.POINTER(C.c_int32), C.POINTER(C.c_int32), C.POINTER(C.c_int32)]),
    "rt_multi_render": (C.c_int, [C.c_void_p, C.c_void_p, C.c_void_p, C.c_void_p, C.c_int32, C.c_int32,
                                  C.c_uint32, C.POINTER(C.c_float)]),
    "rt_multi_render_device_frames": (C.c_int, [C.c_void_p, C.c_void_p, C.c_int32, C.c_void_p, C.c_void_p,
                                                C.c_int32, C.c_int32, C.c_uint32, C.c_void_p]),
    "rt_multi_rccl_version": (C.c_int, [C.POINTER(C.c_int32)]),
    "rt_multi_destroy": (C.c_int, [C.c_void_p]),
    "rt_render": (C.c_int, [C.c_void_p, C.c_void_p, C.c_void_p, C.c_void_p, C.c_int32, C.c_int32,
                            C.c_uint32, C.POINTER(C.c_float)]),
    "rt_host_pin": (C.c_int, [C.c_void_p, C.c_int64]),
    "rt_host_unpin": (C.c_int, [C.c_void_p]),
    "rt_render_device": (C.c_int, [C.c_void_p, C.c_void_p, C.c_void_p, C.c_void_p, C.c_int32,
                                   C.c_int32, C.c_uint32, C.c_void_p, C.c_void_p]),
    "rt_untile_device": (C.c_int, [C.c_void_p, C.c_void_p, C.c_int64, C.c_void_p, C.c_void_p,
                                   C.c_int32, C.c_int32, C.c_void_p, C.c_void_p]),
    "rt_tile_pixels": (C.c_int64, [C.c_int32, C.c_int32, C.c_void_p]),
    "rt_render_device_frames": (C.c_int, [C.c_void_p, C.c_void_p, C.c_int32, C.c_void_p, C.c_void_p,
                                          C.c_int32, C.c_int32, C.c_uint32, C.c_void_p, C.c_void_p]),
    "rt_clear_device": (C.c_int, [C.c_void_p, C.c_void_p, C.c_int64, C.c_void_p]),
    "rt_stream_prepare": (C.c_int, [C.c_void_p]),
    "rt_stream_release": (C.c_int, [C.c_void_p]),
    "rt_exchange_alloc": (C.c_int, [C.c_int64, C.POINTER(C.c_void_p)]),
    "rt_exchange_free": (C.c_int, [C.c_void_p]),
    "rt_ipc_get_handle": (C.c_int, [C.c_void_p, C.c_void_p]),
    "rt_ipc_open": (C.c_int, [C.c_void_p, C.POINTER(C.c_void_p)]),
    "rt_ipc_close": (C.c_int, [C.c_void_p]),
    "rt_intersect_rays": (C.c_int, [C.c_void_p, C.c_void_p, C.c_void_p, C.c_int64, C.c_float,
                                    C.c_float, C.c_void_p, C.c_void_p, C.c_void_p, C.c_void_p]),
    "rt_trace_rays_device": (C.c_int, [C.c_void_p, C.POINTER(RayBatch), C.c_uint32, C.c_void_p]),
    "rt_eye_rays_device": (C.c_int, [C.c_void_p, C.c_int32, C.c_int32, C.c_void_p, C.c_void_p, C.c_void_p]),
    "rt_shade_rays_device": (C.c_int, [C.c_void_p, C.POINTER(RayBatch), C.c_void_p, C.c_void_p, C.c_uint32,
                                       C.c_void_p]),
    "rt_count_work": (C.c_int, [C.c_void_p, C.c_void_p, C.c_int32, C.c_int32, C.c_int32,
                                C.c_uint32, C.c_void_p, C.c_void_p]),
    "rt_bench_frames": (C.c_int, [C.c_void_p, C.c_void_p, C.c_int32, C.c_int32, C.c_int32,
                                  C.c_uint32, C.POINTER(C.c_float), C.POINTER(C.c_float)]),
    "rt_sdf_mesh_create": (C.c_int, [C.c_void_p, C.c_int64, C.c_void_p, C.c_int64,
                                     C.POINTER(C.c_void_p)]),
    "rt_sdf_mesh_points": (C.c_int, [C.c_void_p, C.c_void_p, C.c_int64, C.c_void_p]),
    "rt_sdf_mesh_grid": (C.c_int, [C.c_void_p, C.c_void_p, C.c_void_p]),
    "rt_sdf_mesh_points_device": (C.c_int, [C.c_void_p, C.POINTER(PointBatch), C.c_uint32, C.c_void_p]),
    "rt_sdf_mesh_grid_device": (C.c_int, [C.c_void_p, C.c_void_p, C.c_void_p, C.c_void_p]),
    "rt_sdf_mesh_device": (C.c_int, [C.c_void_p]),
    "rt_sdf_mesh_octree": (C.c_int, [C.c_void_p, C.c_int32, C.POINTER(C.c_int64), C.c_void_p]),
    "rt_sdf_mesh_destroy": (C.c_int, [C.c_void_p]),
    "rt_sdf_mesh_create_ex": (C.c_int, [C.c_void_p, C.c_int64, C.c_void_p, C.c_int64, C.c_uint32,
                                        C.POINTER(C.c_void_p)]),
    "rt_sdf_mesh_update_vertices": (C.c_int, [C.c_void_p, C.c_void_p, C.c_int64]),
    "rt_sdf_mesh_update_vertices_device": (C.c_int, [C.c_void_p, C.c_void_p, C.c_int64, C.c_void_p]),
    "rt_sdf_mesh_get_pseudonormals": (C.c_int, [C.c_void_p, C.c_void_p, C.c_int64]),
    "rt_sdf_mesh_device_bytes": (C.c_int64, [C.c_void_p]),
    "rt_scene_update_grid_device": (C.c_int, [C.c_void_p, C.c_void_p, C.c_void_p]),
    "rt_scene_create_octree_dynamic": (C.c_int, [C.c_int32, C.c_int64, C.POINTER(C.c_void_p)]),
    "rt_sdf_mesh_octree_device": (C.c_int, [C.c_void_p, C.c_void_p, C.c_void_p]),
    "rt_scene_octree_status": (C.c_int, [C.c_void_p, C.POINTER(C.c_int64), C.POINTER(C.c_int32)]),
    "rt_scene_get_octree": (C.c_int, [C.c_void_p, C.POINTER(C.c_int64), C.c_void_p]),
    "rt_mesh_subdivide": (C.c_int, [C.c_void_p, C.c_int64, C.c_void_p, C.c_int64, C.c_int32, C.c_void_p,
                                    C.POINTER(C.c_int64), C.c_void_p, C.POINTER(C.c_int64)]),
    "rt_camera_init": (C.c_int, [C.c_void_p, C.c_void_p, C.c_void_p, C.POINTER(CameraState)]),
    "rt_camera_rotate": (C.c_int, [C.POINTER(CameraState), C.c_float, C.c_float]),
    "rt_camera_reset_position": (C.c_int, [C.POINTER(CameraState), C.c_void_p]),
    "rt_camera_reset_target": (C.c_int, [C.POINTER(CameraState), C.c_void_p]),
    "rt_camera_set_lock_up": (C.c_int, [C.POINTER(CameraState), C.c_int]),
    "rt_camera_zoom": (C.c_int, [C.POINTER(CameraState), C.c_float]),
    "rt_camera_basis": (C.c_int, [C.POINTER(CameraState), C.c_void_p, C.c_void_p, C.c_void_p]),
    "rt_camera_view_inverse": (C.c_int, [C.POINTER(CameraState), C.c_void_p]),
    "rt_write_png": (C.c_int, [C.c_char_p, C.c_void_p, C.c_int32, C.c_int32]),
    "rt_save_obj": (C.c_int, [C.c_char_p, C.c_void_p, C.c_int64, C.c_void_p, C.c_int64, C.c_void_p,
                              C.c_void_p]),
}

EXPORTED = tuple(_SIGS)

_XSIGS = {
    "rtx_set_tile_cull": (C.c_int, [C.c_int]),
    "rtx_cull_rect": (C.c_int, [C.c_void_p, C.c_int32, C.c_int32, C.c_void_p, C.c_void_p]),
    "rtx_set_queue_grid": (C.c_int, [C.c_int]),
    "rtx_queue_grid": (C.c_int, [C.c_void_p, C.c_void_p, C.c_int32, C.c_int32, C.c_int32, C.c_uint32, C.c_uint32,
                                 C.c_void_p]),
    "rtx_scene_mesh_download": (C.c_int, [C.c_void_p, C.c_void_p, C.POINTER(C.c_int64), C.c_void_p,
                                          C.POINTER(C.c_int64)]),
    "rtx_scene_mesh_constants": (C.c_int, [C.c_void_p, C.c_void_p, C.c_void_p, C.POINTER(C.c_float)]),
    "rtx_bvh_refit_host": (C.c_int, [C.c_void_p, C.c_int64, C.c_void_p, C.c_int64, C.c_void_p, C.c_void_p,
                                     C.POINTER(C.c_int64), C.c_void_p, C.POINTER(C.c_int64)]),
    "rtx_count_share": (C.c_int, [C.c_void_p, C.c_void_p, C.c_int32, C.c_int32, C.c_int32, C.c_uint32,
                                  C.c_void_p]),
    "rtx_dispatch_probe": (C.c_int, [C.c_int, C.c_int, C.c_int, C.c_void_p]),
    "rtx_octree_flatten": (C.c_int, [C.c_void_p, C.c_int64, C.POINTER(C.c_int32), C.POINTER(C.c_int32), C.c_void_p]),
    "rtx_set_tlas_uniform_min": (C.c_int, [C.c_int]),
    "rtx_set_tlas_count": (C.c_int, [C.c_void_p]),
    "rtx_tlas_box_pass": (C.c_int, [C.c_void_p, C.c_void_p, C.c_void_p, C.c_float, C.c_float]),
    "rtx_tlas_build_host": (C.c_int, [C.c_void_p, C.c_int32, C.c_void_p]),
    "rtx_tlas_candidates": (C.c_int, [C.c_void_p, C.c_int32, C.c_void_p, C.c_void_p, C.c_float, C.c_void_p, C.c_int32,
                                      C.c_void_p, C.c_int32]),
    "rtx_set_points_lds_pad": (C.c_int, [C.c_int32]),
    "rtx_sdf_mesh_lds_bytes": (C.c_int64, [C.c_void_p]),
    "rtx_sdf_mesh_download": (C.c_int, [C.c_void_p, C.c_void_p, C.POINTER(C.c_int64), C.c_void_p,
                                        C.POINTER(C.c_int64)]),
    "rtx_sdf_mesh_refit_host": (C.c_int, [C.c_void_p, C.c_int64, C.c_void_p, C.c_int64, C.c_void_p, C.c_void_p,
                                          C.POINTER(C.c_int64), C.c_void_p, C.POINTER(C.c_int64), C.c_void_p]),
    "rtx_live_resources": (C.c_int, [C.POINTER(C.c_int64)]),
    "rtx_scene_octree_words": (C.c_int, [C.c_void_p, C.c_void_p, C.c_int64]),
}


def source_build_id() -> str:
    import glob
    import hashlib
    srcs = sorted(os.path.relpath(p, PKG_ROOT) for ext in ("cpp", "h", "hip")
                  for p in glob.glob(os.path.join(PKG_ROOT, "csrc", f"*.{ext}")))
    h = hashlib.sha256()
    for rel in srcs + [os.path.join("..", "include", "rtamd.h"), "Makefile"]:
        with open(os.path.join(PKG_ROOT, rel), "rb") as f:
            h.update(f.read())
    return h.hexdigest()[:16]


def build(force: bool = False) -> str:
    if os.environ.get("RTAMD_LIB"):
        return LIB_PATH
    subprocess.run(["make", "-C", PKG_ROOT, "-s"] + (["-B"] if force else []), check=True)
    return LIB_PATH


def _share_torch_runtime() -> None:
    if os.environ.get("RTAMD_NO_TORCH"):
        return
    try:
        import torch
    except Exception:
        pass


def lib():
    global _lib
    if _lib is None:
        _share_torch_runtime()
        if not os.path.exists(LIB_PATH):
            raise RtError(f"librtamd.so not built ({LIB_PATH}); run build() / make -C {PKG_ROOT}")
        L = C.CDLL(LIB_PATH)
        for name, (res, args) in _SIGS.items():
            fn = getattr(L, name)
            fn.restype = res
            fn.argtypes = args
        for name, (res, args) in _XSIGS.items():
            fn = getattr(L, name, None)
            if fn is not None:
                fn.restype = res
                fn.argtypes = args
        _lib = L
    return _lib


def check(rc: int) -> None:
    if rc != RT_OK:
        msg = lib().rt_last_error()
        raise RtError(f"rtamd error {rc}: {msg.decode() if msg else ''}")
```

Baseline: 43820 Mrays/s.

## Cull empty tiles per row using projected BVH frontier spans

Takes a shallow frontier of BVH child boxes (depth 2, up to 512), projects them each frame in a small GPU kernel, and builds a per-tile-row x-span table. The persistent renderer then replaces the single screen rectangle cull with the per-row span, so waves whose 8x8 tiles fall outside the silhouette only clear and skip traversal. This adds a tiny extra kernel launch per batch, per-stream span buffers, and a table load per tile, in exchange for skipping more empty rays around the bunny.

```diff
diff --git a/triangles-sdf-cpu-raytracing_amd/csrc/rt_cull.h b/triangles-sdf-cpu-raytracing_amd/csrc/rt_cull.h
--- /dev/null
+++ b/triangles-sdf-cpu-raytracing_amd/csrc/rt_cull.h
@@ -0,0 +1,162 @@
+#pragma once
+#include <stdint.h>
+
+#include "../../include/rtamd.h"
+
+#if defined(__HIPCC__) || defined(__CUDACC__)
+#define RTC_HD __host__ __device__ inline
+#else
+#define RTC_HD inline
+#endif
+
+namespace rtc {
+
+constexpr int kFrontierCap = 512;
+constexpr int kFrontierDepth = 2;
+
+RTC_HD double dmin(double a, double b) { return b < a ? b : a; }
+RTC_HD double dmax(double a, double b) { return a < b ? b : a; }
+
+struct Cam {
+  double o[3];
+  double C[3][3];
+  double det, sgn;
+};
+
+RTC_HD bool cull_cam(const rt_render_params *p, int32_t W, int32_t H, Cam &cam) {
+  if (W <= 0 || H <= 0 || W > 32768 || H > 32768) return false;
+  const float *pi = p->proj_inv, *vi = p->view_inv;
+  double M[3][3];
+  for (int k = 0; k < 3; ++k) {
+    cam.o[k] = (double)p->camera_pos[k];
+    if (!__builtin_isfinite(cam.o[k])) return false;
+  }
+  const double wc = (double)pi[15], wr = __builtin_fabs((double)pi[3]) + __builtin_fabs((double)pi[7]);
+  if (!__builtin_isfinite(wc) || !__builtin_isfinite(wr) || !(__builtin_fabs(wc) > wr * (1.0 + 0x1p-20))) return false;
+  cam.sgn = wc > 0 ? 1.0 : -1.0;
+  const int cols[3] = {0, 1, 3};
+  double scale = 0.0;
+  for (int r = 0; r < 3; ++r)
+    for (int c = 0; c < 3; ++c) {
+      double a = 0.0;
+      for (int j = 0; j < 3; ++j) a += (double)vi[j * 4 + r] * (double)pi[cols[c] * 4 + j];
+      if (!__builtin_isfinite(a)) return false;
+      M[r][c] = a;
+      scale = dmax(scale, __builtin_fabs(a));
+    }
+  for (int r = 0; r < 3; ++r)
+    for (int c = 0; c < 3; ++c) {
+      const int r1 = (r + 1) % 3, r2 = (r + 2) % 3, c1 = (c + 1) % 3, c2 = (c + 2) % 3;
+      cam.C[r][c] = M[r1][c1] * M[r2][c2] - M[r1][c2] * M[r2][c1];
+    }
+  cam.det = M[0][0] * cam.C[0][0] + M[0][1] * cam.C[0][1] + M[0][2] * cam.C[0][2];
+  if (!__builtin_isfinite(cam.det) || !(__builtin_fabs(cam.det) > 1e-9 * scale * scale * scale)) return false;
+  const double n0 = __builtin_sqrt(M[0][0] * M[0][0] + M[1][0] * M[1][0] + M[2][0] * M[2][0]);
+  const double n1 = __builtin_sqrt(M[0][1] * M[0][1] + M[1][1] * M[1][1] + M[2][1] * M[2][1]);
+  const double l0 = n0 * 2.0 / W;
+  const double l1 = n1 * 2.0 / H;
+  const double l2 = __builtin_sqrt(M[0][2] * M[0][2] + M[1][2] * M[1][2] + M[2][2] * M[2][2]) + n0 + n1;
+  if (!(l0 >= 0x1p-17 * l2) || !(l1 >= 0x1p-17 * l2)) return false;
+  return true;
+}
+
+RTC_HD bool cull_box(const Cam &cam, int32_t W, int32_t H, const float lo[3], const float hi[3], int32_t out[4],
+                     double (*pix)[2] = nullptr) {
+  for (int k = 0; k < 3; ++k) {
+    if (!__builtin_isfinite((double)lo[k]) || !__builtin_isfinite((double)hi[k])) return false;
+    if (!(lo[k] <= hi[k])) return false;
+    if (cam.o[k] == (double)lo[k] || cam.o[k] == (double)hi[k]) return false;
+  }
+  const double inf = __builtin_inf();
+  double nlo[2] = {inf, inf};
+  double nhi[2] = {-inf, -inf};
+  int behind = 0;
+  for (int i = 0; i < 8; ++i) {
+    double v[3], c[3];
+    for (int k = 0; k < 3; ++k) v[k] = (double)(((i >> k) & 1) ? hi[k] : lo[k]) - cam.o[k];
+    for (int r = 0; r < 3; ++r)
+      c[r] = (cam.C[0][r] * v[0] + cam.C[1][r] * v[1] + cam.C[2][r] * v[2]) / cam.det;
+    const double z = cam.sgn * c[2], zb = 1e-9 * (__builtin_fabs(c[0]) + __builtin_fabs(c[1]));
+    if (!__builtin_isfinite(z) || !__builtin_isfinite(zb)) return false;
+    if (z < -zb && z < 0.0) {
+      ++behind;
+      continue;
+    }
+    if (behind != 0 || !(z > zb) || !(z > 0.0)) return false;
+    for (int a = 0; a < 2; ++a) {
+      const double n = c[a] / c[2];
+      if (!__builtin_isfinite(n)) return false;
+      nlo[a] = dmin(nlo[a], n);
+      nhi[a] = dmax(nhi[a], n);
+      if (pix) pix[i][a] = (n + 1.0) * (a == 0 ? (double)W : (double)H) * 0.5 - 0.5;
+    }
+  }
+  if (behind == 8) {
+    out[0] = out[1] = out[2] = out[3] = 0;
+    return true;
+  }
+  if (behind != 0) return false;
+  const double dim[2] = {(double)W, (double)H};
+  int64_t p0[2], p1[2];
+  for (int a = 0; a < 2; ++a) {
+    const double f0 = __builtin_floor((nlo[a] + 1.0) * dim[a] * 0.5 - 0.5) - 2.0;
+    const double f1 = __builtin_ceil((nhi[a] + 1.0) * dim[a] * 0.5 - 0.5) + 2.0;
+    p0[a] = (int64_t)dmin(dmax(f0, 0.0), dim[a]);
+    p1[a] = (int64_t)dmin(dmax(f1, -1.0), dim[a] - 1.0);
+  }
+  const int64_t r0 = (int64_t)H - 1 - p1[1], r1 = (int64_t)H - 1 - p0[1];
+  if (p0[0] > p1[0] || r0 > r1) {
+    out[0] = out[1] = out[2] = out[3] = 0;
+    return true;
+  }
+  out[0] = (int32_t)(p0[0] >> 3);
+  out[1] = (int32_t)(p1[0] >> 3) + 1;
+  out[2] = (int32_t)(r0 >> 3);
+  out[3] = (int32_t)(r1 >> 3) + 1;
+  return true;
+}
+
+RTC_HD void row_span(const double pix[8][2], int32_t W, int32_t H, const int32_t rect[4], uint32_t r, uint32_t &x0,
+                     uint32_t &x1) {
+  x0 = x1 = 0u;
+  const int64_t i1 = (int64_t)8 * r + 7 < (int64_t)H - 1 ? (int64_t)8 * r + 7 : (int64_t)H - 1;
+  const double a = (double)((int64_t)H - 1 - i1) - 2.0, b = (double)((int64_t)H - 1 - (int64_t)8 * r) + 2.0;
+  const double inf = __builtin_inf();
+  double xlo = inf, xhi = -inf;
+#pragma unroll 1
+  for (int i = 0; i < 8; ++i) {
+    if (pix[i][1] >= a && pix[i][1] <= b) {
+      xlo = dmin(xlo, pix[i][0]);
+      xhi = dmax(xhi, pix[i][0]);
+    }
+#pragma unroll 1
+    for (int j = i + 1; j < 8; ++j) {
+      const double dy = pix[j][1] - pix[i][1], dx = pix[j][0] - pix[i][0];
+      for (int e = 0; e < 2; ++e) {
+        const double c = e ? b : a;
+        if ((pix[i][1] < c && pix[j][1] > c) || (pix[i][1] > c && pix[j][1] < c)) {
+          const double x = pix[i][0] + (c - pix[i][1]) / dy * dx;
+          xlo = dmin(xlo, x);
+          xhi = dmax(xhi, x);
+        }
+      }
+    }
+  }
+  if (!(xlo <= xhi)) return;
+  const double f0 = __builtin_floor(xlo) - 2.0, f1 = __builtin_ceil(xhi) + 2.0;
+  const int64_t p0 = (int64_t)dmin(dmax(f0, 0.0), (double)W), p1 = (int64_t)dmin(dmax(f1, -1.0), (double)W - 1.0);
+  if (p0 > p1) return;
+  const uint32_t t0 = (uint32_t)(p0 >> 3), t1 = (uint32_t)(p1 >> 3) + 1u;
+  x0 = t0 > (uint32_t)rect[0] ? t0 : (uint32_t)rect[0];
+  x1 = t1 < (uint32_t)rect[1] ? t1 : (uint32_t)rect[1];
+}
+
+RTC_HD uint32_t span_word(uint32_t lo, uint32_t hi, bool whole, uint32_t cx, uint32_t cy, uint32_t r) {
+  if (cx == 0xFFFF0000u || cy == 0xFFFF0000u) return 0xFFFF0000u;
+  if (r < (cy & 0xFFFFu) || r >= (cy >> 16)) return 0u;
+  if (whole) return cx;
+  const uint32_t a = lo > (cx & 0xFFFFu) ? lo : (cx & 0xFFFFu), b = hi < (cx >> 16) ? hi : (cx >> 16);
+  return a < b ? a | (b << 16) : 0u;
+}
+
+}
diff --git a/triangles-sdf-cpu-raytracing_amd/csrc/rt_device.hip b/triangles-sdf-cpu-raytracing_amd/csrc/rt_device.hip
--- a/triangles-sdf-cpu-raytracing_amd/csrc/rt_device.hip
+++ b/triangles-sdf-cpu-raytracing_amd/csrc/rt_device.hip
@@ -10,8 +10,10 @@
 #include <string>
 #include <type_traits>
 #include <utility>
+#include <vector>
 
 #include "../../include/rtamd.h"
+#include "rt_cull.h"
 #include "rt_dispatch.h"
 #include "rt_error.h"
 #include "rt_host.h"
@@ -85,10 +87,10 @@
 #endif
 constexpr int kPairWords = 2 * 8 * 16;
 
-template <class S, int SLOTS, bool GENERAL, int DIAG, int B = kBlock, class CT>
+template <class S, int SLOTS, bool GENERAL, int DIAG, int B = kBlock, bool SPANS = false, class CT>
 __device__ __forceinline__ bool render_pixels(const S &sc, const PlaneDev &pl, const FrameArgs &fa,
                                               CT &cnt, uint32_t *stk, int xo, int yl,
-                                              uint32_t *defer = nullptr) {
+                                              uint32_t *defer = nullptr, const uint32_t *spans = nullptr) {
   const bool active = xo < fa.W && yl < fa.rows_local;
   constexpr bool kWaveCoop = DIAG == 0 && !GENERAL && S::kCoop;
   constexpr bool kWaveCount = DIAG == 1 && !GENERAL && S::kCoop;
@@ -97,8 +99,12 @@
     StackOf<S, B> st{stk + threadIdx.x};
     if constexpr (kWaveCoop) {
       const int yo = image_row(active ? yl : 0, fa);
-      const uint32_t cx = fa.cull_x, cy = (uint32_t)fa.P.reserved;
+      uint32_t cx = fa.cull_x;
+      const uint32_t cy = (uint32_t)fa.P.reserved;
       const uint32_t px = (uint32_t)xo >> 3, py = (uint32_t)yo >> 3;
+      if constexpr (SPANS) {
+        if (spans) cx = spans[py];
+      }
       const bool inside = active && px >= (cx & 0xFFFFu) && px < (cx >> 16) && py >= (cy & 0xFFFFu) && py < (cy >> 16);
       if (__ballot(inside) == 0) {
         const bool natural = (fa.flags & (kSysStoreFlags | kFlagNatural)) != 0;
@@ -422,7 +428,7 @@
 
 template <class S, int SLOTS, bool GENERAL>
 __global__ __launch_bounds__(kPBlock) __attribute__((amdgpu_waves_per_eu(min_waves<S, SLOTS, GENERAL, 0>())))
-void render_persist_kernel(S sc_arg, PlaneDev pl, FrameBatch fb, PersistQ q) {
+void render_persist_kernel(S sc_arg, PlaneDev pl, FrameBatch fb, PersistQ q, const uint32_t *spans) {
   __shared__ uint32_t stk[stack_words<S, SLOTS>() * kPBlock];
   S sc = sc_arg;
   if constexpr (S::kCoop && !GENERAL) sc.prio_iters = RT_HEAVY_PRIO;
@@ -474,8 +480,15 @@
       for (uint32_t i = 0; i < q.gx; ++i) {
         uint32_t fo = f;
         asm volatile("" : "+s"(fo));
-        render_pixels<S, SLOTS, GENERAL, 0, kPBlock>(sc, pl, fb.f[fo], cnt, stk, (int)((tx * q.gx + i) * 8) + (lane & 7),
-                                            (int)((ty * q.gy + j) * 8) + (lane >> 3));
+        if constexpr (kQueueOrigin<S, GENERAL>) {
+          const uint32_t *sp = spans ? spans + fo * (((uint32_t)fb.f[fo].H + 7u) >> 3) : nullptr;
+          render_pixels<S, SLOTS, GENERAL, 0, kPBlock, true>(sc, pl, fb.f[fo], cnt, stk,
+                                                             (int)((tx * q.gx + i) * 8) + (lane & 7),
+                                                             (int)((ty * q.gy + j) * 8) + (lane >> 3), nullptr, sp);
+        } else {
+          render_pixels<S, SLOTS, GENERAL, 0, kPBlock>(sc, pl, fb.f[fo], cnt, stk, (int)((tx * q.gx + i) * 8) + (lane & 7),
+                                                       (int)((ty * q.gy + j) * 8) + (lane >> 3));
+        }
       }
 #ifdef RT_PERSIST_STAMPS
     ++n_items;
@@ -744,6 +757,60 @@
   }
 }
 
+struct SpanArgs {
+  rt_render_params P[kMaxBatch];
+  uint32_t cx[kMaxBatch], cy[kMaxBatch];
+  const rtl::GNode *nodes;
+  const uint32_t *frontier;
+  uint32_t n;
+  int32_t W, H;
+  uint32_t rows;
+  uint32_t *table;
+};
+static_assert(sizeof(SpanArgs) + 256 <= 4096, "SpanArgs exceeds the 4 KiB kernel-argument budget");
+constexpr int kSpanBlock = 256;
+__global__ __launch_bounds__(kSpanBlock) void cull_spans_kernel(SpanArgs a) {
+  extern __shared__ uint32_t span_lds[];
+  uint32_t *lo = span_lds, *hi = span_lds + a.rows, *whole = span_lds + 2 * a.rows;
+  const uint32_t f = blockIdx.x;
+  for (uint32_t r = threadIdx.x; r < a.rows; r += blockDim.x) {
+    lo[r] = 0xFFFFu;
+    hi[r] = 0u;
+  }
+  if (threadIdx.x == 0) *whole = 0u;
+  __syncthreads();
+  const uint32_t cx = a.cx[f], cy = a.cy[f];
+  if (cx != kCullWhole && cy != kCullWhole) {
+    rtc::Cam cam;
+    if (!rtc::cull_cam(&a.P[f], a.W, a.H, cam)) {
+      if (threadIdx.x == 0) atomicOr(whole, 1u);
+    } else {
+      for (uint32_t i = threadIdx.x; i < a.n; i += blockDim.x) {
+        const uint32_t e = a.frontier[i];
+        const float *b = a.nodes[e >> 3].box[e & 7u];
+        const float blo[3] = {b[0], b[2], b[4]}, bhi[3] = {b[1], b[3], b[5]};
+        int32_t r[4];
+        double pix[8][2];
+        if (!rtc::cull_box(cam, a.W, a.H, blo, bhi, r, pix)) {
+          atomicOr(whole, 1u);
+          continue;
+        }
+        for (uint32_t y = (uint32_t)r[2]; y < (uint32_t)r[3] && y < a.rows; ++y) {
+          uint32_t x0, x1;
+          rtc::row_span(pix, a.W, a.H, r, y, x0, x1);
+          if (x0 >= x1) continue;
+          atomicMin(&lo[y], x0);
+          atomicMax(&hi[y], x1);
+        }
+      }
+    }
+  }
+  __syncthreads();
+  const bool wf = *whole != 0u;
+  for (uint32_t r = threadIdx.x; r < a.rows; r += blockDim.x)
+    a.table[(size_t)f * a.rows + r] = rtc::span_word(lo[r], hi[r], wf, cx, cy, r);
+}
+
 constexpr int kCostClasses = 66;
 __device__ __forceinline__ uint32_t cost_class(uint32_t c) {
   if (c == 0) return 0;
@@ -912,28 +979,64 @@
 constexpr size_t kQueueWords = (size_t)rtq::kMaxHeads * kHeadStride + 16;
 constexpr size_t kQueueBytes = kQueueWords * sizeof(uint32_t);
 static_assert((size_t)rtq::kXcds * kHeadStrideMax + 1 <= kQueueWords, "8 heads at the widest stride must fit");
+constexpr size_t kSpanRows0 = 512;
+struct StreamQ {
+  uint32_t *heads = nullptr;
+  uint32_t *spans = nullptr;
+  size_t span_words = 0;
+};
 std::mutex g_queue_mu;
-std::map<std::pair<int, hipStream_t>, uint32_t *> g_queues;
+std::map<std::pair<int, hipStream_t>, StreamQ> g_queues;
+
+int stream_state(int dev, hipStream_t stream, StreamQ **out) {
+  auto it = g_queues.find({dev, stream});
+  if (it != g_queues.end()) {
+    *out = &it->second;
+    return RT_OK;
+  }
+  void *p = nullptr, *t = nullptr;
+  HIP_TRY(hipMallocAsync(&p, kQueueBytes, stream));
+  hipError_t e = hipMemsetAsync(p, 0, kQueueBytes, stream);
+  if (e == hipSuccess) e = hipMallocAsync(&t, kMaxBatch * kSpanRows0 * sizeof(uint32_t), stream);
+  if (e != hipSuccess) {
+    HIP_NOTE(hipFreeAsync(p, stream));
+    return set_err(RT_E_DEVICE, std::string("work-queue init: ") + hipGetErrorString(e));
+  }
+  StreamQ &q = g_queues[{dev, stream}];
+  q.heads = (uint32_t *)p;
+  q.spans = (uint32_t *)t;
+  q.span_words = kMaxBatch * kSpanRows0;
+  *out = &q;
+  return RT_OK;
+}
 
 int stream_queue(hipStream_t stream, uint32_t **out) {
   *out = nullptr;
   int dev = 0;
   HIP_TRY(hipGetDevice(&dev));
   std::lock_guard<std::mutex> lk(g_queue_mu);
-  auto it = g_queues.find({dev, stream});
-  if (it != g_queues.end()) {
-    *out = it->second;
-    return RT_OK;
-  }
-  void *p = nullptr;
-  HIP_TRY(hipMallocAsync(&p, kQueueBytes, stream));
-  const hipError_t e = hipMemsetAsync(p, 0, kQueueBytes, stream);
-  if (e != hipSuccess) {
-    HIP_NOTE(hipFreeAsync(p, stream));
-    return set_err(RT_E_DEVICE, std::string("work-queue init: ") + hipGetErrorString(e));
-  }
-  g_queues[{dev, stream}] = (uint32_t *)p;
-  *out = (uint32_t *)p;
+  StreamQ *q = nullptr;
+  if (const int rc = stream_state(dev, stream, &q)) return rc;
+  *out = q->heads;
+  return RT_OK;
+}
+
+int stream_spans(hipStream_t stream, size_t rows, uint32_t **out) {
+  *out = nullptr;
+  int dev = 0;
+  HIP_TRY(hipGetDevice(&dev));
+  std::lock_guard<std::mutex> lk(g_queue_mu);
+  StreamQ *q = nullptr;
+  if (const int rc = stream_state(dev, stream, &q)) return rc;
+  const size_t words = (size_t)kMaxBatch * rows;
+  if (words > q->span_words) {
+    void *t = nullptr;
+    HIP_TRY(hipMallocAsync(&t, words * sizeof(uint32_t), stream));
+    HIP_NOTE(hipFreeAsync(q->spans, stream));
+    q->spans = (uint32_t *)t;
+    q->span_words = words;
+  }
+  *out = q->spans;
   return RT_OK;
 }
 
@@ -1031,13 +1134,15 @@
 static_assert(g.ox == 1 && g.oy == 1 && g.tiles_x == 3 && g.tiles_y == 1, "rtq::grid");
 }
 
-bool takes_queue_grid(const FrameBatch &fb, int n) {
-  if (!g_queue_grid.load(std::memory_order_relaxed)) return false;
+bool whole_device_frames(const FrameBatch &fb, int n) {
   for (int i = 0; i < n; ++i)
     if (fb.f[i].nranks != 1 || (fb.f[i].flags & (kSysStoreFlags | kFlagNatural | kFlagHostFrame)) != 0 ||
         fb.f[i].W != fb.f[0].W || fb.f[i].rows_local != fb.f[0].rows_local || fb.f[i].flags != fb.f[0].flags)
       return false;
   return true;
+}
+bool takes_queue_grid(const FrameBatch &fb, int n) {
+  return g_queue_grid.load(std::memory_order_relaxed) && whole_device_frames(fb, n);
 }
 
 int make_queue(const FrameBatch &fb, int n, int group, int blocks, hipStream_t stream, PersistQ &q,
@@ -1068,6 +1173,46 @@
   grid = std::min<uint32_t>((uint32_t)blocks, (q.items + wpb - 1) / wpb);
   q.waves = grid * wpb;
   q.stamps = (g_persist_stamps && (int64_t)q.waves <= g_persist_stamps_cap) ? g_persist_stamps : nullptr;
+  return RT_OK;
+}
+
+bool cull_spans_env() {
+  static const bool on = !ab_off("RTAMD_CULL_SPANS");
+  return on;
+}
+std::atomic<bool> g_cull_spans{cull_spans_env()};
+
+int launch_cull_spans(rt_scene *s, const rtl::GNode *nodes, const FrameBatch &fb, int n, hipStream_t stream,
+                      const uint32_t **table) {
+  *table = nullptr;
+  if (!s || s->mesh.frontier.empty() || !nodes || !g_cull_spans.load(std::memory_order_relaxed)) return RT_OK;
+  if (!s->geo.frontier.p) {
+    hipStreamCaptureStatus cs = hipStreamCaptureStatusNone;
+    if (hipStreamIsCapturing(stream, &cs) != hipSuccess || cs != hipStreamCaptureStatusNone) {
+      (void)hipGetLastError();
+      return RT_OK;
+    }
+    if (const int rc = s->geo.frontier.upload(s->mesh.frontier.data(), s->mesh.frontier.size())) return rc;
+  }
+  SpanArgs a;
+  for (int i = 0; i < kMaxBatch; ++i) {
+    const FrameArgs &f = fb.f[i < n ? i : 0];
+    a.P[i] = f.P;
+    a.cx[i] = f.cull_x;
+    a.cy[i] = (uint32_t)f.P.reserved;
+  }
+  a.nodes = nodes;
+  a.frontier = s->geo.frontier.p;
+  a.n = (uint32_t)s->mesh.frontier.size();
+  a.W = fb.f[0].W;
+  a.H = fb.f[0].H;
+  a.rows = ((uint32_t)fb.f[0].H + 7u) / 8u;
+  uint32_t *t = nullptr;
+  if (const int rc = stream_spans(stream, a.rows, &t)) return rc;
+  a.table = t;
+  const unsigned block = a.n <= 64u ? 64u : (unsigned)kSpanBlock;
+  cull_spans_kernel<<<(unsigned)n, block, (2 * a.rows + 1) * sizeof(uint32_t), stream>>>(a);
+  *table = t;
   return RT_OK;
 }
 
@@ -1089,6 +1234,11 @@
   co.y0 = std::min(H, q.oy * q.gy * 8u);
   co.y1 = q.tiles_x ? std::min(H, (q.oy + q.per_frame / q.tiles_x) * q.gy * 8u) : co.y0;
   const bool whole = co.x0 == 0 && co.y0 == 0 && co.x1 == W && co.y1 == H;
+  const uint32_t *spans = nullptr;
+  if constexpr (kQueueOrigin<S, GENERAL>) {
+    if (grid != 0 && whole_device_frames(fb, n))
+      if (const int rc = launch_cull_spans(s, sc.d.nodes, fb, n, stream, &spans)) return rc;
+  }
   if (!whole && (fb.f[0].flags & RT_FLAG_CLEAR) && !(fb.f[0].flags & RT_FLAG_HITS_ONLY)) {
     for (int i = 0; i < kMaxBatch; ++i) {
       co.color[i] = i < n ? fb.f[i].color : nullptr;
@@ -1097,7 +1247,7 @@
     clear_outside_kernel<<<dim3((W + 63u) / 64u, (H + 7u) / 8u, (uint32_t)n), 64, 0, stream>>>(co);
   }
   if (grid == 0) return RT_OK;
-  render_persist_kernel<S, MAXD, GENERAL><<<grid, kPBlock, 0, stream>>>(sc, pl, fb, q);
+  render_persist_kernel<S, MAXD, GENERAL><<<grid, kPBlock, 0, stream>>>(sc, pl, fb, q, spans);
   return RT_OK;
 }
 
@@ -1235,93 +1385,42 @@
 
 bool cull_rect(const rt_render_params *p, int32_t W, int32_t H, const float box[6], const float *guard,
                int n_guard, int32_t out[4]) {
-  if (W <= 0 || H <= 0 || W > 32768 || H > 32768) return false;
-  const float *pi = p->proj_inv, *vi = p->view_inv;
-  double o[3], M[3][3];
-  for (int k = 0; k < 3; ++k) {
-    o[k] = (double)p->camera_pos[k];
-    if (!std::isfinite(o[k]) || !std::isfinite((double)box[k]) || !std::isfinite((double)box[3 + k])) return false;
-    if (!(box[k] <= box[3 + k])) return false;
-  }
+  rtc::Cam cam;
+  if (!rtc::cull_cam(p, W, H, cam)) return false;
   bool outside = false;
   for (int k = 0; k < 3; ++k) {
-    if (o[k] < (double)box[k] || o[k] > (double)box[3 + k]) outside = true;
-    if (o[k] == (double)box[k] || o[k] == (double)box[3 + k]) return false;
+    if (cam.o[k] < (double)box[k] || cam.o[k] > (double)box[3 + k]) outside = true;
     for (int g = 0; g < n_guard; ++g)
-      if (o[k] == (double)guard[6 * g + 2 * k] || o[k] == (double)guard[6 * g + 2 * k + 1]) return false;
+      if (cam.o[k] == (double)guard[6 * g + 2 * k] || cam.o[k] == (double)guard[6 * g + 2 * k + 1]) return false;
   }
   if (!outside) return false;
-  const double wc = (double)pi[15], wr = std::fabs((double)pi[3]) + std::fabs((double)pi[7]);
-  if (!std::isfinite(wc) || !std::isfinite(wr) || !(std::fabs(wc) > wr * (1.0 + 0x1p-20))) return false;
-  const double sgn = wc > 0 ? 1.0 : -1.0;
-  const int cols[3] = {0, 1, 3};
-  double scale = 0.0;
-  for (int r = 0; r < 3; ++r)
-    for (int c = 0; c < 3; ++c) {
-      double a = 0.0;
-      for (int j = 0; j < 3; ++j) a += (double)vi[j * 4 + r] * (double)pi[cols[c] * 4 + j];
-      if (!std::isfinite(a)) return false;
-      M[r][c] = a;
-      scale = std::max(scale, std::fabs(a));
-    }
-  double C[3][3];
-  for (int r = 0; r < 3; ++r)
-    for (int c = 0; c < 3; ++c) {
-      const int r1 = (r + 1) % 3, r2 = (r + 2) % 3, c1 = (c + 1) % 3, c2 = (c + 2) % 3;
-      C[r][c] = M[r1][c1] * M[r2][c2] - M[r1][c2] * M[r2][c1];
-    }
-  const double det = M[0][0] * C[0][0] + M[0][1] * C[0][1] + M[0][2] * C[0][2];
-  if (!std::isfinite(det) || !(std::fabs(det) > 1e-9 * scale * scale * scale)) return false;
-  const double l0 = std::sqrt(M[0][0] * M[0][0] + M[1][0] * M[1][0] + M[2][0] * M[2][0]) * 2.0 / W;
-  const double l1 = std::sqrt(M[0][1] * M[0][1] + M[1][1] * M[1][1] + M[2][1] * M[2][1]) * 2.0 / H;
-  const double l2 = std::sqrt(M[0][2] * M[0][2] + M[1][2] * M[1][2] + M[2][2] * M[2][2]) +
-                    std::sqrt(M[0][0] * M[0][0] + M[1][0] * M[1][0] + M[2][0] * M[2][0]) +
-                    std::sqrt(M[0][1] * M[0][1] + M[1][1] * M[1][1] + M[2][1] * M[2][1]);
-  if (!(l0 >= 0x1p-17 * l2) || !(l1 >= 0x1p-17 * l2)) return false;
-  double lo[2] = {std::numeric_limits<double>::infinity(), std::numeric_limits<double>::infinity()};
-  double hi[2] = {-lo[0], -lo[1]};
-  int behind = 0;
-  for (int i = 0; i < 8; ++i) {
-    double v[3], c[3];
-    for (int k = 0; k < 3; ++k) v[k] = (double)box[((i >> k) & 1) ? 3 + k : k] - o[k];
-    for (int r = 0; r < 3; ++r) c[r] = (C[0][r] * v[0] + C[1][r] * v[1] + C[2][r] * v[2]) / det;
-    const double z = sgn * c[2], zb = 1e-9 * (std::fabs(c[0]) + std::fabs(c[1]));
-    if (!std::isfinite(z) || !std::isfinite(zb)) return false;
-    if (z < -zb && z < 0.0) {
-      ++behind;
-      continue;
-    }
-    if (behind != 0 || !(z > zb) || !(z > 0.0)) return false;
-    for (int a = 0; a < 2; ++a) {
-      const double n = c[a] / c[2];
-      if (!std::isfinite(n)) return false;
-      lo[a] = std::min(lo[a], n);
-      hi[a] = std::max(hi[a], n);
-    }
-  }
-  if (behind == 8) {
-    out[0] = out[1] = out[2] = out[3] = 0;
-    return true;
-  }
-  if (behind != 0) return false;
-  const double dim[2] = {(double)W, (double)H};
-  int64_t p0[2], p1[2];
-  for (int a = 0; a < 2; ++a) {
-    const double f0 = std::floor((lo[a] + 1.0) * dim[a] * 0.5 - 0.5) - 2.0;
-    const double f1 = std::ceil((hi[a] + 1.0) * dim[a] * 0.5 - 0.5) + 2.0;
-    p0[a] = (int64_t)std::min(std::max(f0, 0.0), dim[a]);
-    p1[a] = (int64_t)std::min(std::max(f1, -1.0), dim[a] - 1.0);
-  }
-  const int64_t r0 = (int64_t)H - 1 - p1[1], r1 = (int64_t)H - 1 - p0[1];
-  if (p0[0] > p1[0] || r0 > r1) {
-    out[0] = out[1] = out[2] = out[3] = 0;
-    return true;
-  }
-  out[0] = (int32_t)(p0[0] >> 3);
-  out[1] = (int32_t)(p1[0] >> 3) + 1;
-  out[2] = (int32_t)(r0 >> 3);
-  out[3] = (int32_t)(r1 >> 3) + 1;
-  return true;
+  return rtc::cull_box(cam, W, H, box, box + 3, out);
+}
+
+void cull_spans(const rt_render_params *p, int32_t W, int32_t H, const float *boxes, int n, uint32_t cx, uint32_t cy,
+                uint32_t *out) {
+  const uint32_t rows = (uint32_t)(H + 7) / 8u;
+  std::vector<uint32_t> lo(rows, 0xFFFFu), hi(rows, 0u);
+  rtc::Cam cam;
+  bool whole = !rtc::cull_cam(p, W, H, cam);
+  for (int i = 0; i < n && !whole; ++i) {
+    const float *b = boxes + 6 * i;
+    const float blo[3] = {b[0], b[2], b[4]}, bhi[3] = {b[1], b[3], b[5]};
+    int32_t r[4];
+    double pix[8][2];
+    if (!rtc::cull_box(cam, W, H, blo, bhi, r, pix)) {
+      whole = true;
+      break;
+    }
+    for (int32_t y = r[2]; y < r[3] && (uint32_t)y < rows; ++y) {
+      uint32_t x0, x1;
+      rtc::row_span(pix, W, H, r, (uint32_t)y, x0, x1);
+      if (x0 >= x1) continue;
+      lo[y] = std::min(lo[y], x0);
+      hi[y] = std::max(hi[y], x1);
+    }
+  }
+  for (uint32_t y = 0; y < rows; ++y) out[y] = rtc::span_word(lo[y], hi[y], whole, cx, cy, y);
 }
 
 }
@@ -1438,7 +1537,8 @@
     }
     auto it = g_queues.find({dev, (hipStream_t)stream});
     if (it == g_queues.end()) return RT_OK;
-    p = it->second;
+    p = it->second.heads;
+    if (it->second.spans) HIP_NOTE(hipFreeAsync(it->second.spans, (hipStream_t)stream));
     g_queues.erase(it);
   }
   HIP_TRY(hipFreeAsync(p, (hipStream_t)stream));
@@ -1525,8 +1625,33 @@
   return p && box && out && cull_rect(p, W, H, box, nullptr, 0, out) ? 1 : 0;
 }
 
+int rtx_cull_spans(const rt_render_params *p, int32_t W, int32_t H, const float *boxes, int32_t n, uint32_t *out_rows) {
+  if (!p || !boxes || !out_rows || n < 1 || W <= 0 || H <= 0) return -1;
+  const float inf = std::numeric_limits<float>::infinity();
+  float u[6] = {inf, inf, inf, -inf, -inf, -inf};
+  for (int32_t i = 0; i < n; ++i)
+    for (int k = 0; k < 3; ++k) {
+      u[k] = std::min(u[k], boxes[6 * i + 2 * k]);
+      u[3 + k] = std::max(u[3 + k], boxes[6 * i + 2 * k + 1]);
+    }
+  uint32_t cx = kCullWhole, cy = kCullWhole;
+  int32_t r[4];
+  const bool rect = cull_rect(p, W, H, u, nullptr, 0, r);
+  if (rect) {
+    cx = (uint32_t)r[0] | ((uint32_t)r[1] << 16);
+    cy = (uint32_t)r[2] | ((uint32_t)r[3] << 16);
+  }
+  cull_spans(p, W, H, boxes, n, cx, cy, out_rows);
+  return rect ? 1 : 0;
+}
+
 int rtx_set_tile_cull(int on) {
   g_tile_cull.store(on < 0 ? tile_cull_env() : (on != 0));
+  return RT_OK;
+}
+
+int rtx_set_cull_spans(int on) {
+  g_cull_spans.store(on < 0 ? cull_spans_env() : (on != 0));
   return RT_OK;
 }
 
diff --git a/triangles-sdf-cpu-raytracing_amd/csrc/rt_host.cpp b/triangles-sdf-cpu-raytracing_amd/csrc/rt_host.cpp
--- a/triangles-sdf-cpu-raytracing_amd/csrc/rt_host.cpp
+++ b/triangles-sdf-cpu-raytracing_amd/csrc/rt_host.cpp
@@ -617,6 +617,30 @@
   return first;
 }
 
+std::vector<uint32_t> bvh_frontier(const std::vector<rtl::GNode> &nodes, uint32_t root_word, int depth, size_t cap) {
+  std::vector<uint32_t> cur;
+  if ((root_word & rtl::kLeafBit) || root_word >= nodes.size()) return cur;
+  auto slots = [&](uint32_t node, std::vector<uint32_t> &out) {
+    for (uint32_t c = 0; c < 8; ++c)
+      if (nodes[node].child[c] != rtl::kInvalidChild) out.push_back(node << 3 | c);
+  };
+  slots(root_word, cur);
+  for (int d = 1; d < depth; ++d) {
+    std::vector<uint32_t> next;
+    for (uint32_t e : cur) {
+      const uint32_t w = nodes[e >> 3].child[e & 7u];
+      if ((w & rtl::kLeafBit) || w >= nodes.size())
+        next.push_back(e);
+      else
+        slots(w, next);
+    }
+    if (next.size() > cap) break;
+    cur.swap(next);
+  }
+  if (cur.size() > cap) cur.clear();
+  return cur;
+}
+
 void refit_bvh8(BVHGpu &b, const float *vpos4, const uint32_t *idx) {
   auto leaf_box = [&](uint32_t word) {
     const uint32_t first = (word & ~rtl::kLeafBit) >> 3, nt = (word & 7u) + 1u;
diff --git a/triangles-sdf-cpu-raytracing_amd/csrc/rt_host.h b/triangles-sdf-cpu-raytracing_amd/csrc/rt_host.h
--- a/triangles-sdf-cpu-raytracing_amd/csrc/rt_host.h
+++ b/triangles-sdf-cpu-raytracing_amd/csrc/rt_host.h
@@ -116,6 +116,7 @@
 void bvh_layout(const float *vpos4, const uint32_t *idx, int64_t nidx, HostNodes H,
                 const std::vector<uint32_t> &cur, BVHGpu &out, unsigned want, bool host_tris);
 std::vector<uint32_t> bvh_level_first(const std::vector<rtl::GNode> &nodes);
+std::vector<uint32_t> bvh_frontier(const std::vector<rtl::GNode> &nodes, uint32_t root_word, int depth, size_t cap);
 void refit_bvh8(BVHGpu &b, const float *vpos4, const uint32_t *idx);
 bool build_bvh8_gpu(const float *vpos4, int64_t nverts, const uint32_t *idx, int64_t nidx, BVHGpu &out,
                     std::string &err, unsigned want = kBvhAll);
diff --git a/triangles-sdf-cpu-raytracing_amd/csrc/rt_scene.h b/triangles-sdf-cpu-raytracing_amd/csrc/rt_scene.h
--- a/triangles-sdf-cpu-raytracing_amd/csrc/rt_scene.h
+++ b/triangles-sdf-cpu-raytracing_amd/csrc/rt_scene.h
@@ -35,6 +35,7 @@
   int32_t depth = 0;
   uint32_t n_tris = 0;
   uint32_t root_nchild = 0;
+  std::vector<uint32_t> frontier;
 };
 
 struct GridDesc {
@@ -52,6 +53,7 @@
   rtmem::DevArray<float> vals;
   rtmem::DevArray<rtl::OctWord> child;
   rtmem::DevArray<rtl::OctVals> ovals;
+  rtmem::DevArray<uint32_t> frontier;
 };
 
 struct Dynamic {
diff --git a/triangles-sdf-cpu-raytracing_amd/csrc/rt_scene.hip b/triangles-sdf-cpu-raytracing_amd/csrc/rt_scene.hip
--- a/triangles-sdf-cpu-raytracing_amd/csrc/rt_scene.hip
+++ b/triangles-sdf-cpu-raytracing_amd/csrc/rt_scene.hip
@@ -9,6 +9,7 @@
 #include <vector>
 
 #include "../../include/rtamd.h"
+#include "rt_cull.h"
 #include "rt_dispatch.h"
 #include "rt_error.h"
 #include "rt_host.h"
@@ -195,6 +196,24 @@
   return RT_OK;
 }
 
+int rtx_bvh_frontier(const float *vpos4, int64_t nverts, const uint32_t *idx, int64_t nidx, int32_t depth,
+                     uint32_t *entries, float *boxes, int32_t *n) {
+  if (!vpos4 || !idx || !n || nverts <= 0 || nidx <= 0 || depth < 1) return set_err(RT_E_INVALID, "bad mesh");
+  rth::BVHGpu b;
+  if (int rc = build_bvh(vpos4, nverts, idx, nidx, b, 0u)) return rc;
+  const std::vector<uint32_t> f = rth::bvh_frontier(b.nodes, b.root_word, depth, 512);
+  if ((int64_t)*n < (int64_t)f.size()) {
+    *n = (int32_t)f.size();
+    return set_err(RT_E_INVALID, "buffer too small");
+  }
+  for (size_t i = 0; i < f.size(); ++i) {
+    if (entries) entries[i] = f[i];
+    if (boxes) std::memcpy(boxes + 6 * i, b.nodes[f[i] >> 3].box[f[i] & 7u], 24);
+  }
+  *n = (int32_t)f.size();
+  return RT_OK;
+}
+
 __global__ void tri_edge_bound_kernel(const rtl::GTri *__restrict__ tris, uint32_t n, uint32_t *out) {
   const uint32_t i = blockIdx.x * blockDim.x + threadIdx.x;
   float m = 0.0f;
@@ -262,6 +281,8 @@
   s->mesh.host_inner = b.host_inner;
   s->mesh.depth = b.max_depth;
   s->mesh.n_inner = (uint32_t)b.nodes.size();
+  static const int frontier_depth = (int)ab_int("RTAMD_CULL_DEPTH", rtc::kFrontierDepth, 1, 3);
+  s->mesh.frontier = rth::bvh_frontier(b.nodes, b.root_word, frontier_depth, rtc::kFrontierCap);
   if (b.dev_tris.p) {
     s->info.dev_bytes += (int64_t)b.dev_tris.bytes;
     s->geo.tris.adopt(b.dev_tris);
diff --git a/triangles-sdf-cpu-raytracing_amd/rtamd/_lib.py b/triangles-sdf-cpu-raytracing_amd/rtamd/_lib.py
--- a/triangles-sdf-cpu-raytracing_amd/rtamd/_lib.py
+++ b/triangles-sdf-cpu-raytracing_amd/rtamd/_lib.py
@@ -188,6 +188,10 @@
 _XSIGS = {
     "rtx_set_tile_cull": (C.c_int, [C.c_int]),
     "rtx_cull_rect": (C.c_int, [C.c_void_p, C.c_int32, C.c_int32, C.c_void_p, C.c_void_p]),
+    "rtx_set_cull_spans": (C.c_int, [C.c_int]),
+    "rtx_cull_spans": (C.c_int, [C.c_void_p, C.c_int32, C.c_int32, C.c_void_p, C.c_int32, C.c_void_p]),
+    "rtx_bvh_frontier": (C.c_int, [C.c_void_p, C.c_int64, C.c_void_p, C.c_int64, C.c_int32, C.c_void_p, C.c_void_p,
+                                   C.POINTER(C.c_int32)]),
     "rtx_set_queue_grid": (C.c_int, [C.c_int]),
     "rtx_queue_grid": (C.c_int, [C.c_void_p, C.c_void_p, C.c_int32, C.c_int32, C.c_int32, C.c_uint32, C.c_uint32,
                                  C.c_void_p]),
```

Measured after the change: 39000 Mrays/s. 0.89x the previous value.
